# chayanchatterjee/GW-Whisper

Measured on AMD Instinct MI355X. Metric: 1s-strain segments/sec (encoder fwd), higher is better.
Workload: dtype bf16; 1 GPU; whisper-tiny encoder fwd, batch 256 log-mel (80x3000) per GPU, 1500 tokens, random-init weights (BASELINE configs[1]); global_batch=256, parallelism=dp1, encoder=tiny, streams_per_gpu=1

## Files before the change

gw_whisper_amd/_lib.py:

```python

from __future__ import annotations

import ctypes as C
import os

_HERE = os.path.dirname(os.path.abspath(__file__))
LIB_PATH = os.environ.get("GWW_LIB") or os.path.join(_HERE, "libgww.so")

PREC_BF16 = 0
PREC_F32 = 1

EPI_BIAS, EPI_GELU, EPI_RESID = 0, 1, 2
EPI_DGELU = 5


class EncCfg(C.Structure):
    _fields_ = [("d_model", C.c_int), ("n_layers", C.c_int), ("n_heads", C.c_int),
                ("ffn", C.c_int), ("n_mels", C.c_int), ("t_in", C.c_int)]


class EncGlobals(C.Structure):
    _fields_ = [(n, C.c_void_p) for n in
                ("conv1_w", "conv1_b", "conv2_w", "conv2_b", "pos", "ln_w", "ln_b")]


class EncLayer(C.Structure):
    _fields_ = [(n, C.c_void_p) for n in
                ("ln1_w", "ln1_b", "q_w", "q_b", "k_w", "v_w", "v_b", "o_w", "o_b",
                 "ln2_w", "ln2_b", "fc1_w", "fc1_b", "fc2_w", "fc2_b")]


class DoraTarget(C.Structure):
    _fields_ = [("layer", C.c_int), ("proj", C.c_int), ("r", C.c_int), ("scaling", C.c_float),
                ("A", C.c_void_p), ("B", C.c_void_p), ("mag", C.c_void_p), ("nrm", C.c_void_p),
                ("dA", C.c_void_p), ("dB", C.c_void_p), ("dm", C.c_void_p)]


class EncLayerGrads(C.Structure):
    _fields_ = [(f[0], C.c_void_p) for f in EncLayer._fields_]


class EncGrads(C.Structure):
    _fields_ = [(n, C.c_void_p) for n in
                ("conv1_w", "conv1_b", "conv2_w", "conv2_b", "pos", "ln_w", "ln_b")] + \
               [("layers", C.POINTER(EncLayerGrads))]


class DoraMergeItem(C.Structure):
    _fields_ = [("w0", C.c_void_p), ("a", C.c_void_p), ("b", C.c_void_p), ("m", C.c_void_p), ("w_eff", C.c_void_p),
                ("norm_out", C.c_void_p), ("scaling", C.c_float), ("d_out", C.c_int), ("d_in", C.c_int), ("r", C.c_int)]


SIGNATURES = {
    "gww_version": (C.c_int, []),
    "gww_last_error": (C.c_char_p, []),
    "gww_frontend_create": (C.c_int, [C.POINTER(C.c_void_p)]),
    "gww_frontend_create_nmel": (C.c_int, [C.c_int, C.POINTER(C.c_void_p)]),
    "gww_frontend_destroy": (None, [C.c_void_p]),
    "gww_logmel_f32": (C.c_int, [C.c_void_p, C.c_void_p, C.c_int, C.c_int, C.c_long, C.c_void_p,
                                 C.c_void_p, C.c_void_p]),
    "gww_logmel_host_f32": (C.c_int, [C.c_void_p, C.c_int, C.c_int, C.c_long, C.c_void_p]),
    "gww_logmel_host_nmel_f32": (C.c_int, [C.c_void_p, C.c_int, C.c_int, C.c_long, C.c_int, C.c_void_p]),
    "gww_encoder_create": (C.c_int, [C.POINTER(EncCfg), C.POINTER(C.c_void_p)]),
    "gww_encoder_destroy": (None, [C.c_void_p]),
    "gww_encoder_set_weights": (C.c_int, [C.c_void_p, C.POINTER(EncGlobals), C.POINTER(EncLayer),
                                          C.c_int, C.c_void_p]),
    "gww_encoder_update_weights": (C.c_int, [C.c_void_p, C.POINTER(EncGlobals), C.POINTER(EncLayer), C.c_int,
                                             C.POINTER(C.c_uint), C.c_void_p]),
    "gww_encoder_workspace_bytes": (C.c_size_t, [C.c_void_p, C.c_int, C.c_int]),
    "gww_encoder_forward": (C.c_int, [C.c_void_p, C.c_void_p, C.c_int, C.c_int, C.c_void_p, C.c_size_t,
                                      C.c_void_p, C.c_void_p, C.c_void_p]),
    "gww_encoder_forward_outputs": (C.c_int, [C.c_void_p, C.c_void_p, C.c_int, C.c_int, C.c_void_p, C.c_size_t,
                                              C.c_void_p, C.c_void_p, C.c_void_p, C.c_void_p]),
    "gww_encoder_set_split": (C.c_int, [C.c_void_p, C.c_int]),
    "gww_encoder_set_stem_shortcut": (C.c_int, [C.c_void_p, C.c_int]),
    "gww_encoder_stem_shortcut_flags": (C.c_int, [C.c_void_p, C.c_int, C.c_int, C.c_void_p, C.POINTER(C.c_int)]),
    "gww_encoder_trace_enable": (C.c_int, [C.c_void_p, C.c_int]),
    "gww_encoder_trace_read": (C.c_int, [C.c_void_p, C.POINTER(C.c_float), C.POINTER(C.c_int)]),
    "gww_encoder_trace_classes": (C.c_int, []),
    "gww_encoder_trace_class_name": (C.c_char_p, [C.c_int]),
    "gww_train_saved_bytes": (C.c_size_t, [C.c_void_p, C.c_int]),
    "gww_train_workspace_bytes": (C.c_size_t, [C.c_void_p, C.c_int]),
    "gww_encoder_train_forward": (C.c_int, [C.c_void_p, C.c_void_p, C.c_int, C.c_void_p, C.c_size_t, C.c_void_p,
                                            C.c_size_t, C.c_void_p, C.c_int, C.c_void_p]),
    "gww_encoder_train_backward": (C.c_int, [C.c_void_p, C.c_int, C.c_void_p, C.c_size_t, C.c_void_p, C.c_size_t,
                                             C.c_void_p, C.POINTER(DoraTarget), C.c_int, C.c_void_p, C.c_void_p,
                                             C.c_int, C.c_void_p]),
    "gww_train_workspace_bytes_full": (C.c_size_t, [C.c_void_p, C.c_int]),
    "gww_train_workspace_bytes_adapters": (C.c_size_t, [C.c_void_p, C.c_int, C.c_int]),
    "gww_encoder_train_backward_full": (C.c_int, [C.c_void_p, C.c_int, C.c_void_p, C.c_size_t, C.c_void_p, C.c_size_t,
                                                  C.c_void_p, C.POINTER(DoraTarget), C.c_int, C.c_void_p, C.c_void_p,
                                                  C.c_int, C.POINTER(EncGrads), C.c_void_p]),
    "gww_train_saved_bytes_f32": (C.c_size_t, [C.c_void_p, C.c_int]),
    "gww_train_workspace_bytes_f32": (C.c_size_t, [C.c_void_p, C.c_int]),
    "gww_encoder_train_forward_f32": (C.c_int, [C.c_void_p, C.c_void_p, C.c_int, C.c_void_p, C.c_size_t, C.c_void_p,
                                                C.c_size_t, C.c_void_p, C.c_int, C.c_void_p]),
    "gww_encoder_train_backward_f32": (C.c_int, [C.c_void_p, C.c_int, C.c_void_p, C.c_size_t, C.c_void_p, C.c_size_t,
                                                 C.c_void_p, C.POINTER(DoraTarget), C.c_int, C.c_void_p, C.c_void_p,
                                                 C.c_int, C.c_void_p]),
    "gww_attention_lse_f32": (C.c_int, [C.c_void_p, C.c_void_p, C.c_void_p, C.c_int, C.c_int, C.c_int, C.c_void_p]),
    "gww_attention_bwd_f32_scratch_bytes": (C.c_size_t, [C.c_int, C.c_int, C.c_int]),
    "gww_attention_bwd_f32": (C.c_int, [C.c_void_p, C.c_void_p, C.c_void_p, C.c_void_p, C.c_void_p, C.c_void_p,
                                        C.c_int, C.c_int, C.c_int, C.c_void_p]),
    "gww_adapter_grads_f32_scratch_bytes": (C.c_size_t, [C.c_long, C.c_int, C.c_int, C.c_int]),
    "gww_adapter_grads_f32": (C.c_int, [C.c_void_p, C.c_long, C.c_void_p, C.c_void_p, C.c_long, C.c_void_p, C.c_float,
                                        C.c_float, C.c_void_p, C.c_void_p, C.c_void_p, C.c_void_p, C.c_void_p,
                                        C.c_void_p, C.c_void_p, C.c_long, C.c_int, C.c_int, C.c_int, C.c_void_p,
                                        C.c_size_t, C.c_void_p]),
    "gww_gemm_wgrad_workspace_bytes": (C.c_size_t, [C.c_long, C.c_int, C.c_int]),
    "gww_gemm_wgrad_bf16": (C.c_int, [C.c_void_p, C.c_long, C.c_void_p, C.c_long, C.c_long, C.c_int, C.c_int, C.c_float,
                                      C.c_void_p, C.c_void_p, C.c_void_p, C.c_size_t, C.c_void_p]),
    "gww_layernorm_param_grads_workspace_bytes": (C.c_size_t, [C.c_long, C.c_int]),
    "gww_layernorm_param_grads": (C.c_int, [C.c_void_p, C.c_void_p, C.c_int, C.c_long, C.c_int, C.c_void_p, C.c_void_p,
                                            C.c_void_p, C.c_size_t, C.c_void_p]),
    "gww_attention_bwd_bf16": (C.c_int, [C.c_void_p, C.c_void_p, C.c_void_p, C.c_void_p, C.c_void_p, C.c_void_p,
                                         C.c_int, C.c_int, C.c_int, C.c_void_p]),
    "gww_attention_bwd_log2q_bf16": (C.c_int, [C.c_void_p, C.c_void_p, C.c_void_p, C.c_void_p, C.c_void_p, C.c_void_p,
                                         C.c_int, C.c_int, C.c_int, C.c_void_p]),
    "gww_attention_log2q_bf16": (C.c_int, [C.c_void_p, C.c_void_p, C.c_void_p, C.c_int, C.c_int, C.c_int, C.c_void_p]),
    "gww_attention_lse_bf16": (C.c_int, [C.c_void_p, C.c_void_p, C.c_void_p, C.c_int, C.c_int, C.c_int, C.c_void_p]),
    "gww_layernorm_bwd": (C.c_int, [C.c_void_p, C.c_void_p, C.c_void_p, C.c_int, C.c_void_p, C.c_int, C.c_void_p,
                                    C.c_long, C.c_int, C.c_void_p]),
    "gww_gelu_bf16": (C.c_int, [C.c_void_p, C.c_void_p, C.c_void_p, C.c_long, C.c_void_p]),
    "gww_dora_grads": (C.c_int, [C.c_void_p, C.c_long, C.c_void_p, C.c_void_p, C.c_long, C.c_void_p, C.c_float,
                                 C.c_float, C.c_void_p, C.c_void_p, C.c_void_p, C.c_void_p, C.c_void_p, C.c_void_p,
                                 C.c_void_p, C.c_long, C.c_int, C.c_int, C.c_void_p]),
    "gww_adapter_grads_scratch_bytes": (C.c_size_t, [C.c_long, C.c_int, C.c_int, C.c_int]),
    "gww_adapter_grads": (C.c_int, [C.c_void_p, C.c_long, C.c_void_p, C.c_void_p, C.c_long, C.c_void_p, C.c_float,
                                    C.c_float, C.c_void_p, C.c_void_p, C.c_void_p, C.c_void_p, C.c_void_p, C.c_void_p,
                                    C.c_void_p, C.c_long, C.c_int, C.c_int, C.c_int, C.c_void_p, C.c_size_t,
                                    C.c_void_p]),
    "gww_dora_grads_multi": (C.c_int, [C.c_void_p, C.c_long, C.c_void_p, C.c_void_p, C.c_long, C.c_int,
                                       C.POINTER(C.c_long), C.POINTER(C.c_void_p), C.POINTER(C.c_float),
                                       C.POINTER(C.c_float), C.POINTER(C.c_void_p), C.POINTER(C.c_void_p),
                                       C.POINTER(C.c_void_p), C.POINTER(C.c_void_p), C.POINTER(C.c_void_p),
                                       C.POINTER(C.c_void_p), C.POINTER(C.c_void_p), C.c_long, C.c_int, C.c_void_p]),
    "gww_dora_merge_f32": (C.c_int, [C.c_void_p, C.c_void_p, C.c_void_p, C.c_void_p, C.c_float,
                                     C.c_int, C.c_int, C.c_int, C.c_void_p, C.c_void_p, C.c_void_p]),
    "gww_conv1_gelu_bf16": (C.c_int, [C.c_void_p, C.c_void_p, C.c_void_p, C.c_void_p, C.c_void_p, C.c_int, C.c_int, C.c_int,
                                      C.c_void_p]),
    "gww_dora_merge_batch_f32": (C.c_int, [C.POINTER(DoraMergeItem), C.c_int, C.c_void_p]),
    "gww_layernorm": (C.c_int, [C.c_void_p, C.c_void_p, C.c_void_p, C.c_void_p, C.c_int, C.c_long,
                                C.c_int, C.c_void_p]),
    "gww_gemm_bf16": (C.c_int, [C.c_void_p, C.c_void_p, C.c_void_p, C.c_void_p, C.c_void_p, C.c_long,
                                C.c_int, C.c_int, C.c_int, C.c_void_p]),
    "gww_gemm_bf16_v4_split": (C.c_int, [C.c_void_p, C.c_void_p, C.c_void_p, C.c_void_p, C.c_void_p, C.c_long,
                                         C.c_int, C.c_int, C.c_int, C.c_int, C.c_void_p]),
    "gww_gemm_astat_bf16": (C.c_int, [C.c_void_p, C.c_void_p, C.c_void_p, C.c_void_p, C.c_void_p, C.c_void_p,
                                      C.c_void_p, C.c_void_p, C.c_long, C.c_int, C.c_int, C.c_int, C.c_void_p]),
    "gww_ln_fold_weights": (C.c_int, [C.c_void_p, C.c_void_p, C.c_void_p, C.c_void_p, C.c_float, C.c_int, C.c_int,
                                      C.c_void_p, C.c_void_p, C.c_void_p, C.c_void_p]),
    "gww_gemm_fulln_bf16": (C.c_int, [C.c_void_p, C.c_void_p, C.c_void_p, C.c_void_p, C.c_long, C.c_int, C.c_int,
                                      C.c_int, C.c_void_p]),
    "gww_mlp_fused_bf16": (C.c_int, [C.c_void_p] * 8 + [C.c_long, C.c_int, C.c_int, C.c_void_p, C.c_void_p, C.c_void_p,
                                     C.c_int, C.c_void_p]),
    "gww_mlp_pack_bf16": (C.c_int, [C.c_void_p, C.c_void_p, C.c_void_p, C.c_void_p, C.c_int, C.c_int, C.c_int, C.c_void_p]),
    "gww_attn_out_mlp_fused_bf16": (C.c_int, [C.c_void_p] * 9 + [C.c_long, C.c_int, C.c_int, C.c_void_p, C.c_void_p, C.c_void_p,
                                              C.c_int, C.c_void_p]),
    "gww_attn_out_mlp_final_bf16": (C.c_int, [C.c_void_p] * 11 + [C.c_long, C.c_int, C.c_int, C.c_void_p]),
    "gww_mlp_pack_op_bf16": (C.c_int, [C.c_void_p] * 5 + [C.c_int, C.c_int, C.c_int, C.c_void_p]),
    "gww_lnqkv_fused_bf16": (C.c_int, [C.c_void_p, C.c_void_p, C.c_void_p, C.c_void_p, C.c_void_p, C.c_long, C.c_int, C.c_int,
                                       C.c_void_p]),
    "gww_stem_fill_f32": (C.c_int, [C.c_void_p] * 5 + [C.c_int, C.c_int, C.c_int, C.c_int, C.c_void_p]),
    "gww_lnqkv_fused_x0_bf16": (C.c_int, [C.c_void_p] * 5 + [C.c_int, C.c_int] + [C.c_void_p] * 4 + [C.c_long, C.c_int, C.c_int,
                                          C.c_void_p]),
    "gww_attn_out_mlp_fused_x0_bf16": (C.c_int, [C.c_void_p] * 5 + [C.c_int, C.c_int] + [C.c_void_p] * 6 + [C.c_long, C.c_int, C.c_int,
                                                 C.c_void_p, C.c_void_p, C.c_void_p, C.c_int, C.c_void_p]),
    "gww_qscan_energy_f32": (C.c_int, [C.c_void_p, C.c_int, C.c_int, C.c_void_p, C.c_void_p, C.POINTER(C.c_int), C.c_void_p,
                                       C.c_void_p, C.c_long, C.c_void_p, C.c_int, C.c_void_p]),
    "gww_qscan_interp_f32": (C.c_int, [C.c_void_p, C.c_long, C.c_void_p, C.c_void_p, C.c_int, C.c_void_p, C.c_int, C.c_int,
                                       C.c_int, C.c_void_p, C.c_void_p, C.c_void_p]),
    "gww_qadapter_tail_f32": (C.c_int, [C.c_void_p, C.c_int, C.c_int, C.c_int, C.c_void_p, C.c_void_p, C.c_void_p,
                                        C.c_void_p, C.c_void_p, C.c_long, C.c_int, C.c_int, C.c_void_p]),
    "gww_qadapter_cnn_packed_bytes": (C.c_size_t, [C.c_int, C.c_int, C.c_int]),
    "gww_qadapter_cnn_workspace_bytes": (C.c_size_t, [C.c_int, C.c_int, C.c_int, C.c_int, C.c_int]),
    "gww_qadapter_cnn_backward_workspace_bytes": (C.c_size_t, [C.c_int, C.c_int, C.c_int, C.c_int, C.c_int, C.c_int]),
    "gww_qadapter_cnn_backward_f32": (C.c_int, [C.c_void_p, C.c_void_p, C.c_int, C.c_int, C.c_int, C.c_void_p, C.c_void_p,
                                                C.c_void_p, C.c_int, C.c_int, C.c_int, C.c_void_p, C.c_size_t] + [C.c_void_p] * 9),
    "gww_qadapter_cnn_pack_f32": (C.c_int, [C.c_void_p] * 8 + [C.c_int, C.c_int, C.c_int, C.c_void_p, C.c_void_p]),
    "gww_qadapter_cnn_forward_f32": (C.c_int, [C.c_void_p, C.c_int, C.c_int, C.c_int, C.c_void_p, C.c_int, C.c_int, C.c_int,
                                              C.c_void_p, C.c_size_t, C.c_void_p, C.c_void_p]),
    "gww_welch_power_f32": (C.c_int, [C.c_void_p, C.c_long, C.c_long, C.c_int, C.c_float, C.c_void_p, C.c_void_p]),
    "gww_column_median_f32": (C.c_int, [C.c_void_p, C.c_long, C.c_int, C.c_void_p, C.c_void_p]),
    "gww_fir_f32": (C.c_int, [C.c_void_p, C.c_long, C.c_void_p, C.c_int, C.c_int, C.c_void_p, C.c_long, C.c_long, C.c_void_p]),
    "gww_fir_f64": (C.c_int, [C.c_void_p, C.c_long, C.c_void_p, C.c_int, C.c_int, C.c_void_p, C.c_long, C.c_long, C.c_void_p]),
    "gww_cluster_triggers_f64": (C.c_int, [C.c_void_p, C.c_void_p, C.c_long, C.c_float, C.c_double, C.c_void_p, C.c_void_p,
                                          C.c_void_p, C.c_int, C.c_void_p]),
    "gww_gemm_f32": (C.c_int, [C.c_void_p, C.c_void_p, C.c_void_p, C.c_void_p, C.c_void_p, C.c_long,
                               C.c_int, C.c_int, C.c_int, C.c_void_p]),
    "gww_attention_bf16": (C.c_int, [C.c_void_p, C.c_void_p, C.c_int, C.c_int, C.c_int, C.c_void_p]),
    "gww_attention_f32": (C.c_int, [C.c_void_p, C.c_void_p, C.c_int, C.c_int, C.c_int, C.c_void_p]),
    "gww_attention_probs_bf16": (C.c_int, [C.c_void_p, C.c_int, C.c_void_p, C.c_int, C.c_int, C.c_int, C.c_void_p]),
    "gww_attention_probs_f32": (C.c_int, [C.c_void_p, C.c_void_p, C.c_int, C.c_int, C.c_int, C.c_void_p]),
    "gww_cast_f32_bf16": (C.c_int, [C.c_void_p, C.c_void_p, C.c_long, C.c_void_p]),
    "gww_info_nce_forward_f32": (C.c_int, [C.c_void_p, C.c_void_p, C.c_int, C.c_int, C.c_float] + [C.c_void_p] * 6),
    "gww_info_nce_backward_f32": (C.c_int, [C.c_void_p] * 4 + [C.c_int, C.c_int, C.c_float] + [C.c_void_p] * 4),
    "gww_qadapter_tail_backward_workspace_bytes": (C.c_size_t, [C.c_int, C.c_int]),
    "gww_qadapter_tail_backward_f32": (C.c_int, [C.c_void_p, C.c_long, C.c_void_p, C.c_int, C.c_int, C.c_int, C.c_int, C.c_int,
                                                 C.c_void_p, C.c_void_p, C.c_void_p, C.c_void_p, C.c_void_p, C.c_size_t]
                                                + [C.c_void_p] * 5),
    "gww_assemble_batch_f32": (C.c_int, [C.c_void_p, C.c_long, C.c_void_p, C.c_long, C.c_long, C.c_void_p, C.c_void_p,
                                         C.c_void_p, C.c_int, C.c_void_p, C.c_void_p]),
    "gww_head_forward_f32": (C.c_int, [C.c_void_p] * 10 + [C.c_int, C.c_int, C.c_int, C.c_float, C.c_int, C.c_ulonglong,
                                       C.c_ulonglong] + [C.c_void_p] * 9),
    "gww_head_workspace_bytes": (C.c_size_t, [C.c_int, C.c_int]),
    "gww_head_backward_f32": (C.c_int, [C.c_void_p] * 10 + [C.c_int, C.c_int, C.c_int, C.c_float, C.c_int]
                              + [C.c_void_p] * 11),
    "gww_head_dropout_mask_f32": (C.c_int, [C.c_ulonglong, C.c_ulonglong, C.c_int, C.c_int, C.c_int, C.c_float, C.c_void_p,
                                            C.c_void_p]),
    "gww_eval_accumulate": (C.c_int, [C.c_void_p, C.c_void_p, C.c_void_p, C.c_int, C.c_int, C.c_void_p, C.c_void_p,
                                      C.c_void_p, C.c_void_p]),
    "gww_det_head_forward_f32": (C.c_int, [C.c_void_p] * 12 + [C.c_int, C.c_int, C.c_int, C.c_float] + [C.c_void_p] * 10),
    "gww_det_head_workspace_bytes": (C.c_size_t, [C.c_int, C.c_int]),
    "gww_det_head_backward_f32": (C.c_int, [C.c_void_p] * 12 + [C.c_int, C.c_int, C.c_int, C.c_void_p, C.c_size_t]
                                  + [C.c_void_p] * 12),
    "gww_det_head_scores_f32": (C.c_int, [C.c_void_p] * 11 + [C.c_int, C.c_int, C.c_int, C.c_int, C.c_void_p, C.c_long,
                                          C.c_void_p]),
    "gww_det_eval_accumulate": (C.c_int, [C.c_void_p, C.c_void_p, C.c_void_p, C.c_int, C.c_int] + [C.c_void_p] * 5),
    "gww_score_thresholds_workspace_bytes": (C.c_size_t, []),
    "gww_score_thresholds_f32": (C.c_int, [C.c_void_p, C.c_long, C.c_void_p, C.c_int, C.c_void_p, C.c_void_p, C.c_size_t,
                                           C.c_void_p]),
    "gww_detection_counts_f32": (C.c_int, [C.c_void_p, C.c_long, C.c_void_p, C.c_int, C.c_void_p, C.c_void_p]),
    "gww_roc_tile": (C.c_int, []),
    "gww_roc_sort_workspace_bytes": (C.c_size_t, [C.c_long]),
    "gww_roc_sort_f32": (C.c_int, [C.c_void_p, C.c_void_p, C.c_long] + [C.c_void_p] * 7 + [C.c_size_t, C.c_void_p]),
    "gww_roc_curve_workspace_bytes": (C.c_size_t, [C.c_long]),
    "gww_roc_curve_f64": (C.c_int, [C.c_void_p, C.c_void_p, C.c_void_p, C.c_long] + [C.c_void_p] * 7 + [C.c_size_t, C.c_void_p]),
    "gww_roc_bootstrap_workspace_bytes": (C.c_size_t, [C.c_long, C.c_long]),
    "gww_roc_bootstrap_tpr_f64": (C.c_int, [C.c_void_p] * 5 + [C.c_long, C.c_long, C.c_void_p, C.c_int, C.c_void_p, C.c_void_p,
# ... 41 lines not shown
```

gw_whisper_amd/csrc/common.h:

```cpp
#pragma once

#include <hip/hip_runtime.h>
#include <stdarg.h>
#include <stdint.h>
#include <stdio.h>
#include <string.h>

#include "../../include/gww.h"
#include <vector>

namespace gww {

extern thread_local char g_err[512];
int fail(int code, const char* fmt, ...);

#define GWW_HIP(expr)                                                                 \
  do {                                                                                \
    hipError_t _e = (expr);                                                           \
    if (_e != hipSuccess)                                                             \
      return ::gww::fail(GWW_ERR_HIP, "%s failed: %s (%s:%d)", #expr, hipGetErrorString(_e), \
                         __FILE__, __LINE__);                                         \
  } while (0)

#define GWW_LAUNCH_CHECK() GWW_HIP(hipGetLastError())

#define GWW_REQUIRE(cond, ...)                       \
  do {                                               \
    if (!(cond)) return ::gww::fail(GWW_ERR_ARG, __VA_ARGS__); \
  } while (0)

#define GWW_TRY(expr)          \
  do {                         \
    int _rc = (expr);          \
    if (_rc != GWW_OK) return _rc; \
  } while (0)

typedef __attribute__((ext_vector_type(8))) __bf16 bf16x8;
typedef __attribute__((ext_vector_type(4))) __bf16 bf16x4;
typedef __attribute__((ext_vector_type(4))) float f32x4;
typedef __attribute__((ext_vector_type(16))) float f32x16;
typedef __attribute__((ext_vector_type(4))) unsigned int u32x4;
typedef __attribute__((ext_vector_type(2))) unsigned int u32x2;

constexpr int kWave = 64;

__device__ __forceinline__ unsigned short f2bf(float f) {
  __bf16 h = (__bf16)f;
  return __builtin_bit_cast(unsigned short, h);
}
__device__ __forceinline__ float bf2f(unsigned short u) {
  return __builtin_bit_cast(float, ((unsigned int)u) << 16);
}
__device__ __forceinline__ unsigned int pack2bf(float lo, float hi) {
  typedef __bf16 bf16x2_t __attribute__((ext_vector_type(2)));
  typedef float f32x2_t __attribute__((ext_vector_type(2)));
  const f32x2_t v = {lo, hi};
  return __builtin_bit_cast(unsigned int, __builtin_convertvector(v, bf16x2_t));
}

__device__ __forceinline__ float wave_sum(float v) {
#pragma unroll
  for (int o = 32; o > 0; o >>= 1) v += __shfl_xor(v, o, 64);
  return v;
}
__device__ __forceinline__ float wave_max(float v) {
#pragma unroll
  for (int o = 32; o > 0; o >>= 1) v = fmaxf(v, __shfl_xor(v, o, 64));
  return v;
}

__device__ __forceinline__ double wave_sum_f64(double v) {
#pragma unroll
  for (int o = 32; o > 0; o >>= 1) v += __shfl_xor(v, o, 64);
  return v;
}
__device__ __forceinline__ double block_sum_f64(double s) {
  __shared__ double part[256];
  part[threadIdx.x] = s;
  __syncthreads();
  for (int o = 128; o > 0; o >>= 1) {
    if ((int)threadIdx.x < o) part[threadIdx.x] += part[threadIdx.x + o];
    __syncthreads();
  }
  return part[0];
}
__device__ __forceinline__ double block_sum_f64(const float* __restrict__ v, int n) {
  double s = 0.0;
  for (int i = threadIdx.x; i < n; i += 256) s += (double)v[i];
  return block_sum_f64(s);
}

__device__ __forceinline__ float gelu_erf(float x) {
  return 0.5f * x * (1.0f + erff(x * 0.70710678118654752440f));
}

__device__ __forceinline__ float gelu_fast(float x) {
  const float z = fabsf(x) * 0.70710678118654752440f;
  const float t = __builtin_amdgcn_rcpf(fmaf(0.3275911f, z, 1.0f));
  float p = fmaf(1.061405429f, t, -1.453152027f);
  p = fmaf(p, t, 1.421413741f);
  p = fmaf(p, t, -0.284496736f);
  p = fmaf(p, t, 0.254829592f);
  p *= t;
  const float e = __builtin_amdgcn_exp2f(-z * z * 1.44269504088896340736f);
  const float erf_abs = fmaf(-p, e, 1.0f);
  const float h = 0.5f * x;
  return fmaf(h, copysignf(erf_abs, x), h);
}

__device__ __forceinline__ float gelu_sig4(float x) {
  const float s = fminf(x * x, 64.0f);
  float q = fmaf(s, 0.0010148164f, -0.1067791331f);
  q = fmaf(s, q, -2.3011178f);
  const float e = __builtin_amdgcn_exp2f(x * q);
  return x * __builtin_amdgcn_rcpf(1.0f + e);
}
__device__ __forceinline__ float gelu_sig4_sigma(float x) {
  const float s = fminf(x * x, 64.0f);
  float q = fmaf(s, 0.0010148164f, -0.1067791331f);
  q = fmaf(s, q, -2.3011178f);
  const float e = __builtin_amdgcn_exp2f(x * q);
  return __builtin_amdgcn_rcpf(1.0f + e);
}

__device__ __forceinline__ float dgelu_fast(float z) {
  const float az = fabsf(z) * 0.70710678118654752440f;
  const float t = __builtin_amdgcn_rcpf(fmaf(0.3275911f, az, 1.0f));
  float p = fmaf(1.061405429f, t, -1.453152027f);
  p = fmaf(p, t, 1.421413741f);
  p = fmaf(p, t, -0.284496736f);
  p = fmaf(p, t, 0.254829592f);
  p *= t;
  const float e = __builtin_amdgcn_exp2f(-az * az * 1.44269504088896340736f);
  const float erf_abs = fmaf(-p, e, 1.0f);
  return fmaf(0.5f, copysignf(erf_abs, z), fmaf(z * 0.3989422804f, e, 0.5f));
}

static inline long cdiv(long a, long b) { return (a + b - 1) / b; }

struct Arena {
  size_t off = 0;
  size_t take(size_t bytes) { const size_t o = off; off += (bytes + 255) / 256 * 256; return o; }
  size_t total() const { return off; }
};

#ifdef GWW_LAB
long lab_int(const char* name, long dflt);
#else
constexpr long lab_int(const char*, long dflt) { return dflt; }
#endif

constexpr int kStemTc = 256, kStemTt = kStemTc / 2;

enum { PREP_PACK16, PREP_PACK32, PREP_COPY, PREP_LNFOLD, PREP_TRANSPOSE, PREP_DORA };
constexpr int kPrepMaxOps = 40;
constexpr int kPrepMaxRank = 1024;
struct PrepOp {
  const void *a, *b, *c, *d;
  void *o0, *o1, *o2;
  int kind, blocks, N, K;
  int C, taps;
  float scale;
  int pad_;
};
struct PrepArgs {
  int n;
  int first[kPrepMaxOps + 1];
  PrepOp op[kPrepMaxOps];
};
struct PrepBatch {
  std::vector<PrepArgs> args;
  hipStream_t s;
  explicit PrepBatch(hipStream_t st) : s(st) {}
  int add(const PrepOp& o);
  int flush();
  int pack(const float* w, void* out, int out_bf16, int N, int C, int taps, int Kpad, float scale);
  int copy(const float* in, float* out, int n, float scale);
  int ln_fold(const float* w, const float* g, const float* bl, const float* bias, float scale, int N, int K, void* wp,
              float* u, float* cb);
  int transpose(const void* in, void* out, int R, int Cn);
  int dora(const float* w0, const float* a, const float* b, const float* m, float scaling, int d_out, int d_in, int r,
           float* w_eff, float* norm_out);
};

enum : int {
  EPI_BIAS = 0,
  EPI_GELU = 1,
  EPI_RESID = 2,
  EPI_CONV2 = 3,
};

}

#include "launchers.h"
```

gw_whisper_amd/csrc/encoder.hip:

```cpp
#include "encoder_impl.h"

namespace gww {
#ifdef GWW_LAB
long lab_int(const char* name, long dflt) {
  const char* e = getenv(name);
  return e ? atol(e) : dflt;
}
#endif
}

using namespace gww;

static size_t carve_blob(gww_encoder* e, char* blob) {
  const size_t d = e->cfg.d_model, F = e->cfg.ffn, T = e->cfg.t_in / 2, Kc1 = conv1_kpad(e->cfg.n_mels);
  const uintptr_t base = (uintptr_t)blob;
  Arena a;
  auto put = [&](auto*& p, size_t bytes) { p = (decltype(+p))(base + a.take(bytes)); };
  put(e->c1w, d * Kc1 * 2);
  put(e->c2w, (d + 255) / 256 * 256 * 3 * d * 2);
  put(e->c1w32, d * Kc1 * 4);
  put(e->c2w32, d * 3 * d * 4);
  put(e->c1wT, d * Kc1 * 2);
  put(e->c2wT, d * 3 * d * 2);
  put(e->c1b, d * 4);
// ... 127 lines not shown
    GWW_HIP(hipMemcpyAsync(e->pos, g->pos, (size_t)T * d * 4, hipMemcpyDeviceToDevice, s));
    if (T > kStemTt) {
      GWW_HIP(hipMemcpyAsync(e->pos_c, g->pos, (size_t)(kStemTt - 2) * d * 4, hipMemcpyDeviceToDevice, s));
      GWW_HIP(hipMemsetAsync(e->pos_c + (size_t)(kStemTt - 2) * d, 0, (size_t)d * 4, s));
      GWW_HIP(hipMemcpyAsync(e->pos_c + (size_t)(kStemTt - 1) * d, g->pos + (size_t)(T - 1) * d, (size_t)d * 4,
                             hipMemcpyDeviceToDevice, s));
    }
    GWW_TRY(pb.copy(g->ln_w, e->lnw, d, 1.f));
    GWW_TRY(pb.copy(g->ln_b, e->lnb, d, 1.f));
  }
  for (int i = 0; i < n_layers; ++i) {
    const unsigned m = dirty ? dirty[i] : 15u;
    if (!m) continue;
    const gww_enc_layer& L = layers[i];
    LayerW& w = e->layers[i];
    const size_t dd = (size_t)d * d;
    if (m & 1u) {
      GWW_REQUIRE(L.ln1_w && L.ln1_b && L.q_w && L.q_b && L.k_w && L.v_w && L.v_b,
                  "gww_encoder_set_weights: NULL attention weight in layer %d", i);
      const float qs16 = attention_log2q_enabled() ? qs * 1.44269504088896340736f : qs;
      GWW_TRY(pb.pack(L.q_w, w.wqkv, 1, d, d, 1, d, qs16));
      GWW_TRY(pb.pack(L.q_w, w.wqkv32, 0, d, d, 1, d, qs));
      GWW_TRY(pack(L.k_w, w.wqkv + dd, w.wqkv32 + dd, d, d, 1, d, 1.f));
      GWW_TRY(pack(L.v_w, w.wqkv + 2 * dd, w.wqkv32 + 2 * dd, d, d, 1, d, 1.f));
      GWW_TRY(pb.copy(L.q_b, w.bqkv, d, qs));
      GWW_TRY(pb.copy(nullptr, w.bqkv + d, d, 0.f));
      GWW_TRY(pb.copy(L.v_b, w.bqkv + 2 * d, d, 1.f));
      GWW_TRY(pb.copy(L.q_b, w.bqkv16, d, qs16));
      GWW_TRY(pb.copy(nullptr, w.bqkv16 + d, d, 0.f));
      GWW_TRY(pb.copy(L.v_b, w.bqkv16 + 2 * d, d, 1.f));
      GWW_TRY(pb.copy(L.ln1_w, w.ln1w, d, 1.f));
      GWW_TRY(pb.copy(L.ln1_b, w.ln1b, d, 1.f));
      GWW_TRY(pb.ln_fold(L.q_w, L.ln1_w, L.ln1_b, L.q_b, qs16, d, d, w.wqkv_ln, w.uqkv, w.cbqkv));
      GWW_TRY(pb.ln_fold(L.k_w, L.ln1_w, L.ln1_b, nullptr, 1.f, d, d, w.wqkv_ln + dd, w.uqkv + d, w.cbqkv + d));
      GWW_TRY(pb.ln_fold(L.v_w, L.ln1_w, L.ln1_b, L.v_b, 1.f, d, d, w.wqkv_ln + 2 * dd, w.uqkv + 2 * d,
                             w.cbqkv + 2 * d));
      GWW_TRY(pt.transpose(w.wqkv, w.wqkvT, 3 * d, d));
    }
    if (m & 2u) {
      GWW_REQUIRE(L.o_w && L.o_b, "gww_encoder_set_weights: NULL out_proj weight in layer %d", i);
      GWW_TRY(pack(L.o_w, w.wo, w.wo32, d, d, 1, d, 1.f));
      GWW_TRY(pb.copy(L.o_b, w.bo, d, 1.f));
      GWW_TRY(pt.transpose(w.wo, w.woT, d, d));
    }
    if (m & 4u) {
      GWW_REQUIRE(L.ln2_w && L.ln2_b && L.fc1_w && L.fc1_b, "gww_encoder_set_weights: NULL fc1 weight in layer %d", i);
      GWW_TRY(pack(L.fc1_w, w.w1, w.w132, F, d, 1, d, 1.f));
      GWW_TRY(pb.copy(L.fc1_b, w.b1, F, 1.f));
      GWW_TRY(pb.copy(L.ln2_w, w.ln2w, d, 1.f));
      GWW_TRY(pb.copy(L.ln2_b, w.ln2b, d, 1.f));
      GWW_TRY(pb.ln_fold(L.fc1_w, L.ln2_w, L.ln2_b, L.fc1_b, 1.f, F, d, w.w1_ln, w.u1, w.cb1));
      GWW_TRY(pt.transpose(w.w1, w.w1T, F, d));
    }
    if (m & 8u) {
      GWW_REQUIRE(L.fc2_w && L.fc2_b, "gww_encoder_set_weights: NULL fc2 weight in layer %d", i);
      GWW_TRY(pack(L.fc2_w, w.w2, w.w232, d, F, 1, F, 1.f));
      GWW_TRY(pb.copy(L.fc2_b, w.b2, d, 1.f));
      GWW_TRY(pt.transpose(w.w2, w.w2T, d, F));
    }
  }
  GWW_TRY(pb.flush());
  GWW_TRY(pt.flush());
  if (mlp_fused_supported(d, F)) {
    for (int i = 0; i < n_layers; ++i) {
      const unsigned m = dirty ? dirty[i] : 15u, mn = i + 1 < n_layers ? (dirty ? dirty[i + 1] : 15u) : 0u;
      if (!(m & 14u) && !(mn & 1u)) continue;
      LayerW& w = e->layers[i];
      const void* wq_next = i + 1 < n_layers ? e->layers[i + 1].wqkv_ln : nullptr;
      const bool plain_stream = (generic_path_mask() & (GP_QKV | GP_OUT_PROJ)) != 0;
      if (plain_stream && ((m & 12u) || (mn & 1u))) GWW_TRY(launch_mlp_pack(w.w1_ln, w.w2, wq_next, w.wmlp, d, F, 3 * d, s));
      GWW_TRY(launch_mlp_pack(w.w1_ln, w.w2, wq_next, w.wmlp_op, d, F, 3 * d, s, w.wo));
    }
    if (!dirty || (dirty[0] & 1u))
      GWW_TRY(launch_mlp_pack(nullptr, nullptr, e->layers[0].wqkv_ln, e->layers[0].wqkv_st, d, 0, 3 * d, s));
  }
  return GWW_OK;
}

extern "C" int gww_encoder_set_weights(gww_encoder* e, const gww_enc_globals* g, const gww_enc_layer* layers,
                                       int n_layers, void* stream) {
  GWW_REQUIRE(e && g && layers, "gww_encoder_set_weights: NULL argument");
  GWW_REQUIRE(n_layers == e->cfg.n_layers, "gww_encoder_set_weights: got %d layers, handle has %d", n_layers,
              e->cfg.n_layers);
  GWW_TRY(pack_weights(e, g, layers, n_layers, nullptr, (hipStream_t)stream));
  e->ready = true;
  return GWW_OK;
}

extern "C" int gww_encoder_update_weights(gww_encoder* e, const gww_enc_globals* globals_or_null,
                                          const gww_enc_layer* layers, int n_layers, const unsigned* layer_dirty,
                                          void* stream) {
  GWW_REQUIRE(e && layers && layer_dirty, "gww_encoder_update_weights: NULL argument");
  GWW_REQUIRE(n_layers == e->cfg.n_layers, "gww_encoder_update_weights: got %d layers, handle has %d", n_layers,
              e->cfg.n_layers);
  if (!e->ready) return fail(GWW_ERR_STATE, "gww_encoder_update_weights: call gww_encoder_set_weights first");
  return pack_weights(e, globals_or_null, layers, n_layers, layer_dirty, (hipStream_t)stream);
}

namespace {
struct WsLayout {
  size_t melT, c1, x, x2, h, d2, qkv, ctx, f1, total;
};
WsLayout ws_layout(const gww_enc_cfg& c, int B, int precision) {
  const size_t es = precision == GWW_PREC_BF16 ? 2 : 4;
  const size_t d = c.d_model, F = c.ffn, Tin = c.t_in, T = c.t_in / 2, C = c.n_mels, Kc1 = conv1_kpad(c.n_mels);
  WsLayout w{};
  Arena a;
  const size_t Mp = padded_rows((size_t)B * T);
  w.melT = a.take(((size_t)B * (Tin + 2) * C + Kc1) * es);
  w.c1 = a.take((((size_t)B * (Tin + 2) + 255) / 256 * 256 + 520) * d * es);
  w.x = a.take(Mp * d * 4);
  w.x2 = a.take(Mp * d * 4);
  w.h = a.take(Mp * d * es);
  w.d2 = a.take(Mp * d * es);
  w.qkv = a.take(Mp * 3 * d * es);
  w.ctx = a.take(Mp * d * es);
  w.f1 = a.take(Mp * F * es);
  w.total = a.total();
  return w;
}

struct StemTailLayout {
  size_t c1s, xs, tr, dump, total;
};
StemTailLayout stem_tail_layout(int B, int d) {
  StemTailLayout t{};
  Arena a;
  t.c1s = a.take((((size_t)B * (kStemTc + 2) + 255) / 256 * 256 + 520) * d * 2);
  t.xs = a.take((size_t)B * kStemTt * d * 4);
  t.tr = a.take((size_t)B * d * 4);
  t.dump = a.take((size_t)d * 4);
  t.total = a.total();
  return t;
}

enum Conv1Kind { CONV1_DIRECT, CONV1_ASTAT, CONV1_GENERIC };
enum Conv2Kind { CONV2_V4, CONV2_FULLN, CONV2_GENERIC };
struct FwdWants {
  bool last_hidden, last_token, hidden_slab, attn_slab;
};
struct FwdPlan {
  Conv1Kind conv1;
  Conv2Kind conv2;
  bool shortcut;
  bool x0_layer0;
  bool astat;
  bool mlp_fused;
  bool fuse_qkv;
  bool lnqkv0;
  bool op;
  bool fuse_final;
  bool pooled;
  bool q_log2;
};
FwdPlan plan_forward(const gww_encoder* e, int batch, int precision, FwdWants want) {
  const gww_enc_cfg& c = e->cfg;
  const int m = generic_path_mask(), d = c.d_model, F = c.ffn, T = c.t_in / 2;
  const bool bf = precision == GWW_PREC_BF16;
  FwdPlan p{};
  p.conv1 = !bf || (m & GP_CONV1) ? CONV1_GENERIC
            : conv1_mel_supported(c.n_mels, d, conv1_kpad(c.n_mels)) ? CONV1_DIRECT : d % 128 == 0 ? CONV1_ASTAT : CONV1_GENERIC;
  p.conv2 = bf && d % 128 == 0 && d <= 3072 && !(m & GP_CONV2) ? CONV2_V4
            : bf && (d == 384 || d == 512) && !(m & GP_CONV2_FULLN) ? CONV2_FULLN : CONV2_GENERIC;
  const auto x2_bytes = [&] { const WsLayout w = ws_layout(c, batch, precision); return w.h - w.x2; };
  p.shortcut = p.conv1 == CONV1_DIRECT && p.conv2 == CONV2_V4 && e->stem_shortcut && batch > 0 && !(m & GP_STEM_SHORTCUT) &&
               stem_tail_supported(c.t_in, d) && stem_tail_layout(batch, d).total <= x2_bytes();
  p.astat = bf && (d == 384 || (d == 512 && (m & GP_ASTAT_512))) && F % 128 == 0 && !(m & GP_LAYER_GEMMS);
  p.mlp_fused = p.astat && mlp_fused_supported(d, F) && !(m & GP_MLP);
  p.fuse_qkv = p.mlp_fused && !(m & GP_QKV);
  p.lnqkv0 = p.fuse_qkv && !(m & GP_LNQKV0);
  p.op = p.fuse_qkv && !(m & GP_OUT_PROJ);
  p.fuse_final = p.op && want.last_hidden && !(m & GP_FINAL_LN);
  p.pooled = bf && !want.last_hidden && want.last_token && T >= 3 && !(m & GP_POOLED) && !want.hidden_slab && !want.attn_slab;
  p.x0_layer0 = p.shortcut && p.lnqkv0 && p.op && !want.hidden_slab && c.n_layers > 1;
  p.q_log2 = attention_log2q_enabled();
  return p;
}
}

constexpr int kSplitMin = 32;

static bool use_split(const gww_encoder* e, int batch) { return e->split && batch >= 2 * kSplitMin; }

extern "C" size_t gww_encoder_workspace_bytes(const gww_encoder* e, int batch, int precision) {
  if (!e || batch <= 0) return 0;
  if (use_split(e, batch)) {
    const int b0 = batch / 2;
    return ws_layout(e->cfg, b0, precision).total + ws_layout(e->cfg, batch - b0, precision).total;
  }
  return ws_layout(e->cfg, batch, precision).total;
}

extern "C" int gww_encoder_set_stem_shortcut(gww_encoder* e, int on) {
  GWW_REQUIRE(e != nullptr, "gww_encoder_set_stem_shortcut: NULL handle");
  e->stem_shortcut = on != 0;
  return GWW_OK;
}

extern "C" int gww_encoder_stem_shortcut_flags(const gww_encoder* e, int batch, int precision, const void* workspace,
                                               int* flags) {
  GWW_REQUIRE(e && workspace && flags, "gww_encoder_stem_shortcut_flags: NULL argument");
  GWW_REQUIRE(batch > 0 && (precision == GWW_PREC_BF16 || precision == GWW_PREC_F32),
              "gww_encoder_stem_shortcut_flags: bad batch %d / precision %d", batch, precision);
  flags[0] = flags[1] = -1;
  const bool split = use_split(e, batch);
  const int b[2] = {split ? batch / 2 : batch, split ? batch - batch / 2 : 0};
  size_t off = 0;
  for (int i = 0; i < 2 && b[i] > 0; ++i) {
    const WsLayout w = ws_layout(e->cfg, b[i], precision);
    if (plan_forward(e, b[i], precision, FwdWants{}).shortcut)
      GWW_HIP(hipMemcpy(&flags[i], (const char*)workspace + off + w.melT, sizeof(int), hipMemcpyDeviceToHost));
    off += w.total;
  }
  return GWW_OK;
}

extern "C" int gww_encoder_set_split(gww_encoder* e, int on) {
  GWW_REQUIRE(e != nullptr, "gww_encoder_set_split: NULL handle");
  if (on && !e->s2[0]) {
    for (int i = 0; i < 2; ++i) {
      GWW_HIP(hipStreamCreateWithFlags(&e->s2[i], hipStreamNonBlocking));
      GWW_HIP(hipEventCreateWithFlags(&e->ev_join[i], hipEventDisableTiming));
    }
    GWW_HIP(hipEventCreateWithFlags(&e->ev_fork, hipEventDisableTiming));
    GWW_HIP(hipEventCreateWithFlags(&e->ev_skew, hipEventDisableTiming));
  }
  e->split = on ? 1 : 0;
  return GWW_OK;
}

struct Tracer {
  gww_encoder* e;
  hipStream_t s;
  int begin(int cls) {
    if (!e->trace) return GWW_OK;
    TraceSpan sp{cls, nullptr, nullptr};
    for (hipEvent_t* ev : {&sp.a, &sp.b}) {
      if (!e->pool.empty()) { *ev = e->pool.back(); e->pool.pop_back(); }
      else GWW_HIP(hipEventCreate(ev));
    }
    GWW_HIP(hipEventRecord(sp.a, s));
    e->spans.push_back(sp);
    return GWW_OK;
  }
  int end() {
    if (!e->trace) return GWW_OK;
    GWW_HIP(hipEventRecord(e->spans.back().b, s));
    return GWW_OK;
  }
};
#define TR(cls, expr)        \
  do {                       \
    GWW_TRY(tr.begin(cls));  \
    GWW_TRY(expr);           \
    GWW_TRY(tr.end());       \
  } while (0)

struct Fwd {
  gww_encoder* e;
  FwdPlan p;
  Tracer tr;
  hipStream_t s;
  bool bf;
  int B, d, F, T, H, n_layers;
  long M;
  void *melT, *c1, *h, *d2, *qkv, *ctx, *f1;
  float *x, *x2;
  int* st_flag;
  void* c1s;
  float *xs, *st_tr, *st_dump;
  MfX0 x0;
  float *last_hidden, *last_token, *hidden_slab, *attn_slab;
  size_t hs_stride, as_stride;
  hipEvent_t skew_event;

  int gemm(const void* A, long lda, const void* W16, const float* W32, const float* bias, const float* resid, const float* pos,
           void* Cout, long Mr, int N, int K, int epi, int rpb) const {
    return bf ? launch_gemm_bf16(A, lda, W16, bias, resid, pos, Cout, Mr, N, K, epi, rpb, s, 1)
              : launch_gemm_f32((const float*)A, lda, W32, bias, resid, pos, (float*)Cout, Mr, N, K, epi, rpb, s);
  }
  int tap_hidden(int l, const float* src) const {
    if (hidden_slab)
      GWW_HIP(hipMemcpyAsync(hidden_slab + (size_t)l * hs_stride, src, (size_t)M * d * 4, hipMemcpyDeviceToDevice, s));
    return GWW_OK;
  }
  int tap_attn(int l) const {
    if (attn_slab) GWW_TRY(launch_attention_probs(qkv, bf, bf && p.q_log2, attn_slab + (size_t)l * as_stride, B, T, H, s));
    return GWW_OK;
  }
  int tap_final() const {
    float* dst = hidden_slab ? hidden_slab + (size_t)n_layers * hs_stride : nullptr;
    if (dst && dst != last_hidden)
      GWW_HIP(hipMemcpyAsync(dst, last_hidden, (size_t)M * d * 4, hipMemcpyDeviceToDevice, s));
    return GWW_OK;
  }
  int stem(const float* mel);
  int walk_astat();
  int walk_generic();
  int pooled_last_layer(const LayerW& L, const float* x, float* rows, void* hb);
  int final_layernorm(const float* xc, const void* pending);
};

int Fwd::stem(const float* mel) {
  const int Tin = e->cfg.t_in, C = e->cfg.n_mels, Kc1 = conv1_kpad(C);
  const size_t es = bf ? 2 : 4;
  auto conv1_direct = [&]() -> int {
    if (p.shortcut) {
      GWW_TRY(launch_stem_detect(mel, st_flag, (long)B * C, Tin, s));
      GWW_TRY(launch_conv1_mel(mel, e->c1w, e->c1b, c1s, B, kStemTc, d, s, Tin, st_flag, 1));
    }
    return launch_conv1_mel(mel, e->c1w, e->c1b, c1, B, Tin, d, s, 0, p.shortcut ? st_flag : nullptr, 0);
  };
  auto conv2_v4 = [&]() -> int {
    const int Np = (d + 255) / 256 * 256;
    if (p.shortcut) {
      GWW_TRY(launch_gemm_bf16_v4(c1s, 2L * d, e->c2w, e->c2b, nullptr, xs, (long)B * (kStemTt + 1), Np, 3 * d, EPI_CONV2, s, 0,
                                  e->pos_c, kStemTt + 1, d, st_dump, st_flag, 1, st_tr, kStemTt - 2));
      if (!p.x0_layer0) GWW_TRY(launch_stem_fill(xs, st_tr, e->pos, x, st_flag, B, T, d, s));
    }
    return launch_gemm_bf16_v4(c1, 2L * d, e->c2w, e->c2b, nullptr, x, (long)B * (T + 1), Np, 3 * d, EPI_CONV2, s, 0, e->pos,
                               T + 1, d, x + (((size_t)B * T + 255) / 256 * 256) * d, p.shortcut ? st_flag : nullptr, 0);
  };
  if (p.conv1 != CONV1_DIRECT) {
    TR(TR_MEL, launch_mel_to_tokens(mel, melT, bf ? 1 : 0, B, C, Tin, s));
    GWW_HIP(hipMemsetAsync((char*)melT + (size_t)B * (Tin + 2) * C * es, 0, Kc1 * es, s));
    GWW_HIP(hipMemsetAsync(c1, 0, (size_t)d * es, s));
  }
  if (p.conv1 == CONV1_DIRECT)
    TR(TR_CONV1, conv1_direct());
  else if (p.conv1 == CONV1_ASTAT)
    TR(TR_CONV1, launch_gemm_astat(melT, C, nullptr, nullptr, nullptr, nullptr, e->c1w, e->c1b, c1,
                                   (long)B * (Tin + 2), d, Kc1, EPI_CONV1, Tin + 2, s));
  else
    TR(TR_CONV1, gemm(melT, C, e->c1w, e->c1w32, e->c1b, nullptr, nullptr, c1, (long)B * (Tin + 2), d, Kc1,
                      EPI_CONV1, Tin + 2));
  if (p.conv2 == CONV2_V4)
    TR(TR_CONV2, conv2_v4());
  else if (p.conv2 == CONV2_FULLN)
    TR(TR_CONV2, launch_gemm_fulln(c1, 2L * d, e->c2w, e->c2b, e->pos, x, (long)B * (T + 1), d, 3 * d, EPI_CONV2, T + 1, s));
  else
    TR(TR_CONV2, gemm(c1, 2L * d, e->c2w, e->c2w32, e->c2b, nullptr, e->pos, x, (long)B * (T + 1), d, 3 * d, EPI_CONV2,
                      T + 1));
  return GWW_OK;
}

int Fwd::pooled_last_layer(const LayerW& L, const float* x, float* rows, void* hb) {
  TR(TR_ATTN, launch_attention_bf16(qkv, ctx, B, T, H, s, nullptr, true, p.q_log2));
  float* xl = rows;
  float* xm = rows + (size_t)B * d;
  float* xf = rows + 2 * (size_t)B * d;
  GWW_HIP(hipMemcpy2DAsync(xl, (size_t)d * 4, x + (size_t)(T - 1) * d, (size_t)T * d * 4, (size_t)d * 4, B,
                           hipMemcpyDeviceToDevice, s));
  TR(TR_OUT, launch_gemm_bf16((const unsigned short*)ctx + (size_t)(T - 1) * d, (long)T * d, L.wo, L.bo, xl, nullptr,
                              xm, B, d, d, EPI_RESID, 0, s, 0));
  TR(TR_LNROWS, launch_layernorm(xm, L.ln2w, L.ln2b, hb, 1, B, d, s));
  TR(TR_FC1, launch_gemm_bf16(hb, d, L.w1, L.b1, nullptr, nullptr, f1, B, F, d, EPI_GELU, 0, s, 0));
  TR(TR_FC2, launch_gemm_bf16(f1, F, L.w2, L.b2, xm, nullptr, xf, B, d, F, EPI_RESID, 0, s, 0));
  TR(TR_LNROWS, launch_layernorm_rows(xf, d, e->lnw, e->lnb, last_token, B, d, s, nullptr));
  return GWW_OK;
}

int Fwd::final_layernorm(const float* xc, const void* pending) {
  if (last_hidden) TR(TR_LN, launch_layernorm(xc, e->lnw, e->lnb, last_hidden, 0, M, d, s, pending));
  if (last_token)
    TR(TR_LNROWS, launch_layernorm_rows(xc + (long)(T - 1) * d, (long)T * d, e->lnw, e->lnb, last_token, B, d, s,
                                        pending ? (const char*)pending + (size_t)(T - 1) * d * 2 : nullptr));
  if (last_hidden) GWW_TRY(tap_final());
  return GWW_OK;
}

struct AstatState {
  float* xc;
  float* xn;
  const void* pending;
  bool qkv_ready;
  void swap() { std::swap(xc, xn); }
};

int Fwd::walk_astat() {
  AstatState st{x, x2, nullptr, false};
  void* const d1 = h;
  auto args = [&]() { MlpFusedArgs a; a.who = "gww_encoder_forward"; a.M = M; a.d = d; return a; };
  auto with_qkv = [&](MlpFusedArgs& a, const LayerW& W) { a.qkv_u = W.uqkv; a.qkv_cb = W.cbqkv; a.qkv_out = qkv; a.NQ = 3 * d; };
  for (int i = 0; i < n_layers; ++i) {
    const LayerW& L = e->layers[i];
    const bool last = i == n_layers - 1, from_x0 = i == 0 && p.x0_layer0;
    if (!st.qkv_ready) {
      if (i == 0 && p.lnqkv0) {
        MlpFusedArgs a = args();
        a.x = st.xc; a.Wt = L.wqkv_st;
        with_qkv(a, L);
        if (from_x0) a.x0 = &x0;
        TR(TR_QKV, launch_mlp_fused(a, s));
      } else {
        TR(TR_QKV, launch_gemm_astat(st.xc, d, st.pending, st.pending ? st.xn : nullptr, L.uqkv, L.cbqkv, L.wqkv_ln, nullptr, qkv,
                                     M, 3 * d, d, EPI_BIAS, 0, s));
        if (st.pending) st.swap();
        st.pending = nullptr;
      }
    }
    st.qkv_ready = false;
    GWW_TRY(tap_hidden(i, st.xc));
    if (i == 0 && skew_event) GWW_HIP(hipEventRecord(skew_event, s));
    if (p.pooled && last) return pooled_last_layer(L, st.xc, st.xn, d1);
    TR(TR_ATTN, launch_attention_bf16(qkv, ctx, B, T, H, s, nullptr, false, p.q_log2));
    GWW_TRY(tap_attn(i));
    if (!p.op)
      TR(TR_OUT, launch_gemm_astat(ctx, d, nullptr, nullptr, nullptr, nullptr, L.wo, L.bo, d1, M, d, d, EPI_BIAS, 0, s));
    MlpFusedArgs a = args();
    a.x = st.xc; a.x_new = from_x0 ? nullptr : st.xn; a.ln_u = L.u1; a.ln_cb = L.cb1; a.b2 = L.b2; a.F = F;
    if (p.op) { a.ctx = ctx; a.bo = L.bo; a.Wt = L.wmlp_op; }
    else { a.delta = d1; a.Wt = L.wmlp; }
    if (p.fuse_qkv && !last) {
      with_qkv(a, e->layers[i + 1]);
      if (from_x0) a.x0 = &x0;
      TR(TR_MLPQKV, launch_mlp_fused(a, s));
      st.qkv_ready = true;
    } else if (p.fuse_final) {
      a.lnf_w = e->lnw; a.lnf_b = e->lnb; a.y = last_hidden;
      TR(TR_MLPFIN, launch_mlp_fused(a, s));
      if (last_token)
        GWW_HIP(hipMemcpy2DAsync(last_token, (size_t)d * 4, last_hidden + (size_t)(T - 1) * d, (size_t)T * d * 4, (size_t)d * 4,
                                 B, hipMemcpyDeviceToDevice, s));
      return tap_final();
    } else if (p.mlp_fused) {
      a.C = d2; a.keep_x_new = true;
      TR(TR_MLP, launch_mlp_fused(a, s));
      st.swap();
      st.pending = d2;
    } else {
      TR(TR_FC1, launch_gemm_astat(st.xc, d, d1, st.xn, L.u1, L.cb1, L.w1_ln, nullptr, f1, M, F, d, EPI_GELU, 0, s));
      st.swap();
      TR(TR_FC2, launch_gemm_fulln(f1, F, L.w2, L.b2, nullptr, d2, M, d, F, EPI_BIAS, 0, s));
      st.pending = d2;
    }
  }
  return final_layernorm(st.xc, st.pending);
}

int Fwd::walk_generic() {
  for (int i = 0; i < n_layers; ++i) {
    const LayerW& L = e->layers[i];
    GWW_TRY(tap_hidden(i, x));
    TR(TR_LN, launch_layernorm(x, L.ln1w, L.ln1b, h, bf ? 1 : 0, M, d, s));
    TR(TR_QKV, gemm(h, d, L.wqkv, L.wqkv32, bf ? L.bqkv16 : L.bqkv, nullptr, nullptr, qkv, M, 3 * d, d, EPI_BIAS, 0));
    if (p.pooled && i == n_layers - 1) return pooled_last_layer(L, x, x2, h);
    if (bf) TR(TR_ATTN, launch_attention_bf16(qkv, ctx, B, T, H, s, nullptr, false, p.q_log2));
    else TR(TR_ATTN, launch_attention_f32((const float*)qkv, (float*)ctx, B, T, H, s));
    GWW_TRY(tap_attn(i));
    TR(TR_OUT, gemm(ctx, d, L.wo, L.wo32, L.bo, x, nullptr, x, M, d, d, EPI_RESID, 0));
    TR(TR_LN, launch_layernorm(x, L.ln2w, L.ln2b, h, bf ? 1 : 0, M, d, s));
    TR(TR_FC1, gemm(h, d, L.w1, L.w132, L.b1, nullptr, nullptr, f1, M, F, d, EPI_GELU, 0));
    TR(TR_FC2, gemm(f1, F, L.w2, L.w232, L.b2, x, nullptr, x, M, d, F, EPI_RESID, 0));
  }
  return final_layernorm(x, nullptr);
}
#undef TR

static int forward_impl(gww_encoder* e, const float* mel, int batch, int precision, void* workspace,
                        size_t workspace_bytes, float* last_hidden, float* last_token, void* stream,
                        hipEvent_t skew_event = nullptr, float* hidden_slab = nullptr, float* attn_slab = nullptr,
                        size_t hs_stride = 0, size_t as_stride = 0) {
  GWW_REQUIRE(e && mel, "gww_encoder_forward: NULL argument");
  if (!e->ready) return fail(GWW_ERR_STATE, "gww_encoder_forward: weights not set");
  GWW_REQUIRE(precision == GWW_PREC_BF16 || precision == GWW_PREC_F32, "gww_encoder_forward: bad precision %d",
              precision);
  GWW_REQUIRE(batch >= 0, "gww_encoder_forward: batch < 0");
  GWW_REQUIRE(last_hidden || last_token, "gww_encoder_forward: no output requested");
  if (batch == 0) return GWW_OK;
  GWW_REQUIRE((((uintptr_t)mel) & 15) == 0 && (((uintptr_t)workspace) & 255) == 0,
              "gww_encoder_forward: mel must be 16-byte and workspace 256-byte aligned");
  const WsLayout w = ws_layout(e->cfg, batch, precision);
  if (!workspace || workspace_bytes < w.total)
    return fail(GWW_ERR_WORKSPACE, "gww_encoder_forward: workspace %zu bytes < required %zu", workspace_bytes,
                w.total);
  const gww_enc_cfg& c = e->cfg;
  char* base = (char*)workspace;
  const StemTailLayout st = stem_tail_layout(batch, c.d_model);
  char* const st_base = base + w.x2;
  Fwd f{};
  f.e = e;
  f.p = plan_forward(e, batch, precision, {last_hidden != nullptr, last_token != nullptr, hidden_slab != nullptr, attn_slab != nullptr});
  f.s = (hipStream_t)stream;
  f.tr = Tracer{e, f.s};
  f.bf = precision == GWW_PREC_BF16;
  f.B = batch; f.d = c.d_model; f.F = c.ffn; f.T = c.t_in / 2; f.H = c.n_heads; f.n_layers = c.n_layers;
  f.M = (long)batch * f.T;
  f.melT = base + w.melT; f.c1 = base + w.c1; f.h = base + w.h; f.d2 = base + w.d2; f.qkv = base + w.qkv; f.ctx = base + w.ctx;
  f.f1 = base + w.f1; f.x = (float*)(base + w.x); f.x2 = (float*)(base + w.x2);
  f.st_flag = (int*)f.melT; f.c1s = st_base + st.c1s; f.xs = (float*)(st_base + st.xs); f.st_tr = (float*)(st_base + st.tr);
  f.st_dump = (float*)(st_base + st.dump);
  f.x0 = MfX0{f.xs, f.st_tr, e->pos, f.st_flag, f.T, kStemTt};
  f.last_hidden = last_hidden; f.last_token = last_token; f.hidden_slab = hidden_slab; f.attn_slab = attn_slab;
  f.hs_stride = hs_stride; f.as_stride = as_stride; f.skew_event = skew_event;
  GWW_TRY(f.stem(mel));
  return f.p.astat ? f.walk_astat() : f.walk_generic();
}

static int forward_split(gww_encoder* e, const float* mel, int batch, int precision, void* workspace,
                         size_t workspace_bytes, float* last_hidden, float* last_token, float* hidden_slab,
                         float* attn_slab, void* stream) {
  GWW_REQUIRE(e && mel, "gww_encoder_forward: NULL argument");
  const size_t T_ = (size_t)(e->cfg.t_in / 2);
  const size_t hs_stride = (size_t)(batch > 0 ? batch : 0) * T_ * e->cfg.d_model;
  const size_t as_stride = (size_t)(batch > 0 ? batch : 0) * e->cfg.n_heads * T_ * T_;
  if (batch <= 0 || !use_split(e, batch))
    return forward_impl(e, mel, batch, precision, workspace, workspace_bytes, last_hidden, last_token, stream, nullptr,
                        hidden_slab, attn_slab, hs_stride, as_stride);
  hipStream_t s = (hipStream_t)stream;
  const int d = e->cfg.d_model, T = e->cfg.t_in / 2;
  const int b[2] = {batch / 2, batch - batch / 2};
  const size_t w0 = ws_layout(e->cfg, b[0], precision).total, w1 = ws_layout(e->cfg, b[1], precision).total;
  if (!workspace || workspace_bytes < w0 + w1)
    return fail(GWW_ERR_WORKSPACE, "gww_encoder_forward: workspace %zu bytes < required %zu", workspace_bytes, w0 + w1);
  GWW_HIP(hipEventRecord(e->ev_fork, s));
  int off = 0;
  static const int skew = (int)lab_int("GWW_SPLIT_SKEW", 0);
  for (int i = 0; i < 2; ++i) {
    GWW_HIP(hipStreamWaitEvent(e->s2[i], e->ev_fork, 0));
    if (i == 1 && skew) GWW_HIP(hipStreamWaitEvent(e->s2[1], e->ev_skew, 0));
    const int rc = forward_impl(e, mel + (size_t)off * e->cfg.n_mels * e->cfg.t_in, b[i], precision,
                                (char*)workspace + (i ? w0 : 0), i ? w1 : w0,
                                last_hidden ? last_hidden + (size_t)off * T * d : nullptr,
                                last_token ? last_token + (size_t)off * d : nullptr, e->s2[i],
                                (i == 0 && skew) ? e->ev_skew : nullptr,
                                hidden_slab ? hidden_slab + (size_t)off * T * d : nullptr,
                                attn_slab ? attn_slab + (size_t)off * e->cfg.n_heads * T_ * T_ : nullptr, hs_stride, as_stride);
    if (rc != GWW_OK) return rc;
    GWW_HIP(hipEventRecord(e->ev_join[i], e->s2[i]));
    GWW_HIP(hipStreamWaitEvent(s, e->ev_join[i], 0));
    off += b[i];
  }
  return GWW_OK;
}

extern "C" int gww_encoder_forward(gww_encoder* e, const float* mel, int batch, int precision, void* workspace,
                                   size_t workspace_bytes, float* last_hidden, float* last_token,
                                   void* stream) {
  return forward_split(e, mel, batch, precision, workspace, workspace_bytes, last_hidden, last_token, nullptr, nullptr,
                       stream);
}

extern "C" int gww_encoder_forward_outputs(gww_encoder* e, const float* mel, int batch, int precision, void* workspace,
                                           size_t workspace_bytes, float* last_hidden, float* hidden_slab,
                                           float* attn_slab, void* stream) {
  GWW_REQUIRE(e && mel, "gww_encoder_forward_outputs: NULL argument");
  if (!last_hidden && hidden_slab && batch > 0)
    last_hidden = hidden_slab + (size_t)e->cfg.n_layers * batch * (e->cfg.t_in / 2) * e->cfg.d_model;
  GWW_REQUIRE(last_hidden != nullptr, "gww_encoder_forward_outputs: no last_hidden and no hidden_slab");
  return forward_split(e, mel, batch, precision, workspace, workspace_bytes, last_hidden, nullptr, hidden_slab, attn_slab,
                       stream);
}
```

gw_whisper_amd/csrc/encoder_impl.h:

```cpp
#pragma once

#include "common.h"
#include "epilogue.h"

#include <stdlib.h>
#include <algorithm>
#include <vector>

namespace gww {

struct LayerW {
  unsigned short *wqkv, *wo, *w1, *w2;
  float *wqkv32, *wo32, *w132, *w232;
  float *bqkv, *bo, *b1, *b2, *ln1w, *ln1b, *ln2w, *ln2b;
  float* bqkv16;
  unsigned short *wqkv_ln, *w1_ln;
  unsigned short* wmlp;
  unsigned short* wqkv_st;
  unsigned short* wmlp_op;
  float *uqkv, *cbqkv, *u1, *cb1;
  unsigned short *wqkvT, *woT, *w1T, *w2T;
};

constexpr int conv1_kpad(int n_mels) { return (3 * n_mels + 63) / 64 * 64; }

inline size_t align_up(size_t x, size_t a = 256) { return (x + a - 1) / a * a; }

inline size_t padded_rows(size_t M) { return (M + 255) / 256 * 256 + 512; }

struct SavedArena {
  size_t layer_stride, x_in, total;
  int n_layers;
  float* x_in_at(void* saved, int l) const {
    return (float*)((char*)saved + (l < n_layers ? (size_t)l * layer_stride + x_in : (size_t)n_layers * layer_stride));
  }
  const float* x_in_at(const void* saved, int l) const { return x_in_at(const_cast<void*>(saved), l); }
};

enum : int {
  GP_LAYER_GEMMS = 1,
  GP_CONV1 = 2,
  GP_CONV2 = 4,
  GP_MLP = 8,
  GP_QKV = 16,
  GP_POOLED = 32,
  GP_LNQKV0 = 64,
  GP_OUT_PROJ = 128,
  GP_FINAL_LN = 256,
  GP_ASTAT_512 = 512,
  GP_CONV2_FULLN = 1024,
  GP_STEM_SHORTCUT = 2048,
};
inline int generic_path_mask() {
  static const int mask = (int)lab_int("GWW_GENERIC_PATH", 0);
  return mask;
}

inline int check_targets(const char* who, const gww_dora_target* t, int n) {
  for (int i = 0; i < n; ++i) {
    GWW_REQUIRE(t[i].r >= 1 && t[i].r <= 64, "%s: target %d has rank %d: adapter gradients support ranks 1..64", who, i, t[i].r);
    GWW_REQUIRE(t[i].A && t[i].B && t[i].mag && t[i].nrm && t[i].dA && t[i].dB && t[i].dm, "%s: NULL pointer in target %d", who, i);
  }
  for (int i = 1; i < n; ++i)
    for (int j = 0; j < i; ++j)
      GWW_REQUIRE(t[i].layer != t[j].layer || t[i].proj != t[j].proj, "%s: duplicate target: %d and %d both name layer %d proj %d",
                  who, j, i, t[i].layer, t[i].proj);
  return GWW_OK;
}
inline int check_target_range(const char* who, const gww_dora_target* t, int n, int L) {
  for (int i = 0; i < n; ++i)
    GWW_REQUIRE(t[i].layer >= 0 && t[i].layer < L && t[i].proj >= 0 && t[i].proj <= 5, "%s: bad target %d", who, i);
  return GWW_OK;
}
struct TargetTable {
  std::vector<const gww_dora_target*> slot;
  TargetTable() = default;
  TargetTable(const gww_dora_target* t, int n, int L) : slot(n > 0 ? (size_t)L * 6 : 0, nullptr) {
    for (int i = 0; i < n; ++i) slot[(size_t)t[i].layer * 6 + t[i].proj] = &t[i];
  }
  const gww_dora_target* at(int layer, int proj) const { return slot.empty() ? nullptr : slot[(size_t)layer * 6 + proj]; }
};

}

enum : int { TR_MEL = 0, TR_CONV1, TR_CONV2, TR_QKV, TR_ATTN, TR_OUT, TR_FC1, TR_FC2, TR_LN, TR_MLP, TR_MLPQKV, TR_LNROWS, TR_MLPFIN, TR_COUNT };

struct TraceSpan { int cls; hipEvent_t a, b; };

struct gww_encoder {
  gww_enc_cfg cfg{};
  bool ready = false;
  bool trace = false;
  bool stem_shortcut = true;
  std::vector<TraceSpan> spans;
  std::vector<hipEvent_t> pool;
  int split = 0;
  hipStream_t s2[2] = {nullptr, nullptr};
  hipEvent_t ev_fork = nullptr, ev_skew = nullptr, ev_join[2] = {nullptr, nullptr};
  char* blob = nullptr;
  size_t blob_bytes = 0;
  unsigned short *c1w = nullptr, *c2w = nullptr;
  unsigned short *c1wT = nullptr, *c2wT = nullptr;
  float *c1w32 = nullptr, *c2w32 = nullptr;
  float *c1b = nullptr, *c2b = nullptr, *pos = nullptr, *lnw = nullptr, *lnb = nullptr;
  float* pos_c = nullptr;
  std::vector<gww::LayerW> layers;
};
```

gw_whisper_amd/csrc/launchers.h:

```cpp
#pragma once

namespace gww {

int launch_layernorm(const float* x, const float* w, const float* b, void* y, int out_bf16,
                     long M, int d, hipStream_t s, const void* delta_bf16 = nullptr);
int launch_layernorm_rows(const float* x, long row_stride, const float* w, const float* b, float* y,
                          long M, int d, hipStream_t s, const void* delta_bf16 = nullptr);
int launch_pack_weight(const float* w, void* out, int out_bf16, int N, int C, int taps, int Kpad,
                       float scale, hipStream_t s);

bool conv1_mel_supported(int n_mels, int d, int kpad);
int launch_conv1_mel(const float* mel, const void* W, const float* bias, void* c1, int B, int T, int d, hipStream_t s,
                     int t_stride = 0, const int* run_flag = nullptr, int run_if = 0);
bool stem_tail_supported(int t_in, int d);
int launch_stem_detect(const float* mel, int* flag, long rows, int t_in, hipStream_t s);
int launch_stem_fill(const float* xs, const float* tr, const float* pos, float* x, const int* flag, int B, int T, int d,
                     hipStream_t s, int Tt = kStemTt);
int launch_mel_to_tokens(const float* mel, void* out, int out_bf16, int B, int C, int T, hipStream_t s);

int launch_gemm_astat(const void* A, long lda, const void* delta, float* x_out, const float* ln_u,
                      const float* ln_cb, const void* W, const float* bias, void* C, long M, int N, int K,
                      int epi, int rows_per_batch, hipStream_t s, long c_panel_rows = 0);
int launch_gemm_bf16(const void* A, long lda, const void* W, const float* bias, const float* resid,
                     const float* pos, void* C, long M, int N, int K, int epi, int rows_per_batch,
                     hipStream_t s, int rows_padded_256 = 0);
int launch_gemm_bf16_v4(const void* A, long lda, const void* W, const float* bias, const float* resid, void* C, long M,
                        int N, int K, int epi, hipStream_t s, int force_split = 0, const float* pos = nullptr,
                        int rows_per_batch = 0, int n_real = 0, float* dump = nullptr, const int* run_flag = nullptr,
                        int run_if = 0, float* tmpl_r = nullptr, int tmpl_t = 0);
int launch_gemm_fulln(const void* A, long lda, const void* W, const float* bias, const float* pos, void* C,
                      long M, int N, int K, int epi, int rows_per_batch, hipStream_t s);
int launch_gemm_f32(const float* A, long lda, const float* W, const float* bias, const float* resid,
                    const float* pos, float* C, long M, int N, int K, int epi, int rows_per_batch,
                    hipStream_t s);

int launch_attention_bf16(const void* qkv, void* ctx, int B, int T, int H, hipStream_t s, float* lse = nullptr,
                          bool last_tile_only = false, bool q_log2 = false);
int launch_attention_w64_bf16(const void* qkv, void* ctx, int B, int T, int H, hipStream_t s, float* lse);
bool attention_log2q_enabled();
int launch_attention_f32(const float* qkv, float* ctx, int B, int T, int H, hipStream_t s);
int launch_attention_probs(const void* qkv, bool bf16, bool q_log2, float* probs, int B, int T, int H, hipStream_t s);
int launch_attention_bwd_bf16(const void* qkv, const void* ctx, const void* dctx, const float* lse, float* D,
                              void* dqkv, int B, int T, int H, hipStream_t s, bool q_log2);

int launch_mlp_pack(const void* w1_folded, const void* w2, const void* wqkv_folded, void* out, int d, int F, int NQ,
                    hipStream_t s, const void* wo = nullptr);
bool mlp_fused_supported(int d, int F);
struct MfX0 {
  const float *xs, *tr, *pos;
  const int* flag;
  int T, Tt;
};
struct MlpFusedArgs {
  const char* who = "mlp_fused";
  const float* x = nullptr;
  const void* delta = nullptr;
  const void* ctx = nullptr;
  const float* bo = nullptr;
  float* x_new = nullptr;
  bool keep_x_new = false;
  const float *ln_u = nullptr, *ln_cb = nullptr;
  const void* Wt = nullptr;
  const float* b2 = nullptr;
  void* C = nullptr;
  const float *qkv_u = nullptr, *qkv_cb = nullptr;
  void* qkv_out = nullptr;
  int NQ = 0;
  float* x_next = nullptr;
  const float *lnf_w = nullptr, *lnf_b = nullptr;
  float* y = nullptr;
  const MfX0* x0 = nullptr;
  long M = 0;
  int d = 0, F = 0;
};
int launch_mlp_fused(const MlpFusedArgs& a, hipStream_t s);

int launch_ln_bwd(const float* x, const float* gamma, const void* dy, int dy_f32, float* dx, int accumulate,
                  void* dx_bf16, long M, int d, hipStream_t s);
int launch_gelu_bf16(const void* z, const void* df, void* out, long n, hipStream_t s);
int launch_sub_f32_bf16(const float* a, const float* b, void* out, long n, hipStream_t s);
int launch_add_delta_f32(const float* x, const void* delta_bf16, float* out, long n, hipStream_t s);
int launch_stem_dz2(const void* dxb, const void* z2, void* out, int B, int T, int d, hipStream_t s);
int launch_stem_dz1(const void* col, const void* z1, void* out, int B, int T, int Tin, int d, hipStream_t s);
int launch_stem_dmel(const void* col1, float* dmel, int B, int Tin, int C, int Kp, hipStream_t s);
int launch_ln_param_grads(const float* x, const void* dy, int dy_f32, long M, int d, float* dgamma, float* dbeta,
                          void* workspace, size_t ws_bytes, hipStream_t s);
size_t ln_param_grads_workspace_bytes(long M, int d);
int launch_pos_grad(const float* dx0, float* dpos, int B, int T, int d, hipStream_t s);
int launch_dora_grads(const void* X, long ldx, const void* dY, const void* Y, long ldy, const float* bias_st,
                      float yscale, float scaling, const float* A, const float* Bm, const float* mag,
                      const float* nrm, float* dA, float* dB, float* dm, long M, int d, int r, hipStream_t s,
                      void* scratch = nullptr, size_t scratch_bytes = 0);
int launch_dora_grads_multi(const void* X, long ldx, const void* dY, const void* Y, long ldy, int np,
                            const long* col_off, const float* const* bias_st, const float* yscale,
                            const float* scaling, const float* const* A, const float* const* Bm,
                            const float* const* mag, const float* const* nrm, float* const* dA, float* const* dB,
                            float* const* dm, long M, int d, hipStream_t s, void* scratch, size_t scratch_bytes);
size_t dora_grads_scratch_bytes(int np, int d);
int launch_adapter_grads(const void* X, long ldx, const void* dY, const void* Y, long ldy, const float* bias_st,
                         float yscale, float scaling, const float* A, const float* Bm, const float* mag,
                         const float* nrm, float* dA, float* dB, float* dm, long M, int d_in, int d_out, int r,
                         hipStream_t s, void* scratch, size_t scratch_bytes);
size_t adapter_grads_scratch_bytes(long M, int d_in, int d_out, int r);
int launch_wgrad(const void* dY, long ldy, const void* X, long ldx, long M, int N, int K, float alpha, float* dW,
                 float* db, int conv_cin, void* workspace, size_t ws_bytes, hipStream_t s);
size_t wgrad_workspace_bytes(long M, int N, int K);

int launch_attention_lse_f32(const float* qkv, float* ctx, float* lse, int B, int T, int H, bool last_tile_only,
                             hipStream_t s);
int launch_attention_bwd_f32(const float* qkv, const float* ctx, const float* dctx, const float* lse, float* scratch,
                             float* dqkv, int B, int T, int H, hipStream_t s);
size_t attention_bwd_f32_scratch_words(int B, int T, int H);
int launch_gemm_f32_dx(const float* A, long lda, const float* W, float* C, long ldc, long M, int N, int K, hipStream_t s);
int launch_adapter_grads_f32(const float* X, long ldx, const float* dY, const float* Y, long ldy, const float* bias,
                             float yscale, float scaling, const float* A, const float* Bm, const float* mag,
                             const float* nrm, float* dA, float* dB, float* dm, long M, int d_in, int d_out, int r,
                             hipStream_t s, void* scratch, size_t scratch_bytes);
size_t adapter_grads_f32_scratch_bytes(long M, int d_in, int d_out, int r);
int launch_gelu_f32(const float* z, const float* g, float* out, long n, hipStream_t s);
int launch_sub_f32(const float* a, const float* b, float* out, long n, hipStream_t s);
int launch_stem_dz2_f32(const float* dx0, const float* z2, float* out, int B, int T, int d, hipStream_t s);
int launch_stem_dz1_f32(const float* col, const float* z1, float* out, int B, int T, int Tin, int d, hipStream_t s);
int launch_stem_dmel_f32(const float* col1, float* dmel, int B, int Tin, int C, int Kp, hipStream_t s);

}
```

gw_whisper_amd/csrc/mlp_fused.hip:

```cpp
#include "common.h"

#include <stdlib.h>

#include <type_traits>

namespace gww {

namespace {
constexpr int MF_D = 384;
constexpr int MF_KT = MF_D / 64;
constexpr int MF_OT = MF_D / 32;
constexpr int MF_WAVES = 4, MF_THREADS = 256, MF_BM = 128;
#ifndef GWW_MF_EXP
#define GWW_MF_EXP 0
#endif
#ifndef GWW_MF_ABL
#define GWW_MF_ABL 0
#endif
#ifndef GWW_MF_OLDDMA
#define GWW_MF_OLDDMA 0
#endif
#ifndef GWW_MF_AHEAD
#define GWW_MF_AHEAD 3
#endif
#ifndef GWW_MF_SCHED
#define GWW_MF_SCHED 1
#endif
#ifndef GWW_MF_VACC
#define GWW_MF_VACC 1
#endif
#ifndef GWW_MF_NTSTORE
#define GWW_MF_NTSTORE 1
#endif
#ifndef GWW_MF_NTLOAD
#define GWW_MF_NTLOAD 1
#endif
#if GWW_MF_NTLOAD
#define MF_NT " nt"
#else
#define MF_NT ""
#endif
#ifndef GWW_MF_PADNOP
#define GWW_MF_PADNOP 0
#endif
#if GWW_MF_PADNOP
#define MF_PADNOP "s_nop 1\n\t"
#else
#define MF_PADNOP ""
#endif
#ifndef GWW_MF_XLDS
#define GWW_MF_XLDS 0
#endif
#ifndef GWW_MF_XSTNT
#define GWW_MF_XSTNT 0
#endif
#ifndef GWW_MF_XNT
#define GWW_MF_XNT 0
#endif
#if GWW_MF_XNT
#define MF_XNT MF_NT
#else
#define MF_XNT ""
#endif
#ifndef GWW_MF_DMAGAP
#define GWW_MF_DMAGAP 1
#endif
#ifndef GWW_MF_TAIL2
#define GWW_MF_TAIL2 0
#endif
#ifndef GWW_MF_NORM
#define GWW_MF_NORM 1
#endif
#ifndef GWW_MF_XACC
#define GWW_MF_XACC 1
#endif
constexpr int MF_AHEAD = GWW_MF_AHEAD;
constexpr int MF_NST_MAX = MF_AHEAD + 1;
constexpr int MF_TILE = 128 * 64 * 2;
constexpr int MF_GL = 16 / MF_WAVES;
constexpr int MF_FMAX = 1536;
constexpr int MF_SLICE_STRIDE = 144, MF_SLICE_BYTES = 32 * MF_SLICE_STRIDE;
constexpr int MF_OFF_CB = MF_NST_MAX * MF_TILE;
constexpr int MF_OFF_U = MF_OFF_CB + MF_FMAX * 4;
constexpr int MF_OFF_B2 = MF_OFF_U + MF_FMAX * 4;
constexpr int MF_OFF_BO = MF_OFF_B2 + MF_D * 4;
constexpr int MF_OFF_QCB = MF_OFF_BO + MF_D * 4;
constexpr int MF_OFF_SLICE = MF_OFF_QCB + MF_FMAX * 4;
constexpr int MF_LDS = MF_OFF_SLICE + 2 * MF_WAVES * MF_SLICE_BYTES;
static_assert(MF_LDS <= 160 * 1024, "LDS budget");

template <int N>
using MF_FL = std::integral_constant<int, N>;

__device__ __forceinline__ float mf_sum8(float v) {
  v += __builtin_bit_cast(float, __builtin_amdgcn_update_dpp(0, __builtin_bit_cast(int, v), 0xB1, 0xF, 0xF, true));
  v += __builtin_bit_cast(float, __builtin_amdgcn_update_dpp(0, __builtin_bit_cast(int, v), 0x4E, 0xF, 0xF, true));
  v += __builtin_bit_cast(float, __builtin_amdgcn_update_dpp(0, __builtin_bit_cast(int, v), 0x141, 0xF, 0xF, true));
  return v;
}

template <int N>
__device__ __forceinline__ void mf_wait_vmcnt() {
  asm volatile("s_waitcnt vmcnt(%0)" ::"n"(N) : "memory");
}

__device__ __forceinline__ float gelu_sig(float x) {
  const float s = fminf(x * x, 64.0f);
  float q = fmaf(s, 0.0010148164f, -0.1067791331f);
  q = fmaf(s, q, -2.3011178f);
#if GWW_MF_EXP & 32
  const float e = (x * q) * 0.37f;
  return x * ((1.0f + e) * 0.91f);
#else
  const float e = __builtin_amdgcn_exp2f(x * q);
  return x * __builtin_amdgcn_rcpf(1.0f + e);
#endif
}

#ifdef GWW_STAMP
__device__ unsigned long long g_stamp_mlp[24];
#define MSTAMP_DECL unsigned long long _t0 = __builtin_amdgcn_s_memtime(); unsigned long long _acc[20] = {0}; \
  const unsigned long long _tb = _t0, _rb = __builtin_amdgcn_s_memrealtime();
#define MSTAMP(i)                                                  \
  do {                                                             \
    if (GWW_STAMP >= 2 && (i) != 0 && (i) != 3 && (i) != 4 && (i) != 5 && !((i) >= 100)) break; \
    __builtin_amdgcn_sched_barrier(0);                             \
    const unsigned long long _t1 = __builtin_amdgcn_s_memtime();   \
    _acc[(i) >= 100 ? (i) - 100 : (i)] += _t1 - _t0;               \
    _t0 = _t1;                                                     \
    __builtin_amdgcn_sched_barrier(0);                             \
  } while (0)
#define TSTAMP(i) do { if (GWW_STAMP == 3) MSTAMP(100 + (i)); } while (0)
#define MSTAMP_FLUSH                                                                 \
  if (lane == 0) {                                                                   \
    for (int _q = 0; _q < 20; ++_q) atomicAdd(&g_stamp_mlp[_q], _acc[_q]);           \
    atomicAdd(&g_stamp_mlp[21], __builtin_amdgcn_s_memrealtime() - _rb);             \
    atomicAdd(&g_stamp_mlp[22], __builtin_amdgcn_s_memtime() - _tb);                 \
    atomicAdd(&g_stamp_mlp[23], 1ull);                                                \
  }
#else
#define MSTAMP_DECL
#define MSTAMP(i)
#define TSTAMP(i)
#define MSTAMP_FLUSH
#endif
}

__device__ __forceinline__ const float* mf_x0_row(const MfX0& z, const float* X, long g, bool x0, bool& tail, int& seg) {
  tail = false; seg = 0;
  if (!x0) return X + g * MF_D;
  const unsigned b = (unsigned)g / (unsigned)z.T, j = (unsigned)g - b * (unsigned)z.T;
  seg = (int)b;
  tail = (int)j >= z.Tt - 2 && (int)j <= z.T - 2;
  if (tail) return z.pos + (long)j * MF_D;
  return z.xs + ((long)b * z.Tt + ((int)j == z.T - 1 ? z.Tt - 1 : (int)j)) * MF_D;
}

struct MfNoX0 {};
template <int MODE, bool OP, bool X0 = false>
__global__ __launch_bounds__(MF_THREADS, 1) void k_mlp_fused(const float* X, const unsigned short* delta, float* x_out,
                                                            const float* __restrict__ ln_u,
                                                            const float* __restrict__ ln_cb,
                                                            const unsigned short* __restrict__ Wt,
                                                            const float* __restrict__ b2,
                                                            unsigned short* __restrict__ C, long M, int F,
                                                            int stagger_ticks, const float* __restrict__ q_u,
                                                            const float* __restrict__ q_cb,
                                                            unsigned short* __restrict__ q_out, int NQ,
                                                            float* x_next, const float* __restrict__ bo, int keep_x_new,
                                                            const std::conditional_t<X0, MfX0, MfNoX0> z) {
  __shared__ __attribute__((aligned(16))) unsigned char lds[MF_LDS];
  constexpr bool QKV = MODE == 1 || MODE == 2, LNQ = MODE == 2, FIN = MODE == 3;
  static_assert(!X0 || (GWW_MF_NORM && GWW_MF_XACC && (MODE == 2 || (MODE == 1 && OP))), "X0: layer 0's two launches; stages in the u table");
  constexpr bool XACC = GWW_MF_XACC && GWW_MF_NORM && GWW_MF_SCHED && OP && (MODE == 1 || MODE == 3);
  constexpr int MF_NST = MF_AHEAD + 1;
  float* lds_cb = reinterpret_cast<float*>(lds + MF_OFF_CB);
  float* lds_u = reinterpret_cast<float*>(lds + MF_OFF_U);
  float* lds_b2 = reinterpret_cast<float*>(lds + MF_OFF_B2);
  float* lds_bo = reinterpret_cast<float*>(lds + MF_OFF_BO);
  float* lds_qcb = reinterpret_cast<float*>(lds + MF_OFF_QCB);
  constexpr int OP_TILES = OP ? 3 * MF_KT : 0;
  typedef __attribute__((address_space(3))) void* lds_ptr;

  const int tid = threadIdx.x, lane = tid & 63, wave = tid >> 6;
  const int r = lane & 31, hh = lane >> 5;
  const long m_base = (long)blockIdx.x * MF_BM + wave * 32;
  unsigned char* slice = lds + MF_OFF_SLICE + wave * MF_SLICE_BYTES;
  unsigned char* const slice0 = slice;
  const int crow = lane >> 3, cchunk = lane & 7;

  const int wave_u = __builtin_amdgcn_readfirstlane(wave);
  const unsigned lane_off = (unsigned)lane * 16u;
  const unsigned lds_base = (unsigned)(unsigned long long)(lds_ptr)lds;
  auto issue_piece_c = [&](int tile, int stage, auto j_c) {
    constexpr int J = decltype(j_c)::value;
    const unsigned dst = lds_base + (unsigned)(stage * MF_TILE + MF_GL * wave_u * 1024);
    if (GWW_MF_EXP & 8) tile &= 7;
    const unsigned short* src = Wt + ((long)tile * (MF_TILE / 2) + MF_GL * wave_u * 512);
    const unsigned lo = lane_off;
    asm volatile("s_mov_b32 m0, %2\n\ts_nop 0\n\tglobal_load_lds_dwordx4 %0, %1 offset:%3"
                 :
                 : "v"(lo), "s"(src), "s"(dst), "n"(J * 1024)
                 : "memory");
  };
  auto issue_piece = [&](int tile, int stage, int j) {
#if GWW_MF_OLDDMA
    const unsigned dst = lds_base + (unsigned)(stage * MF_TILE + (MF_GL * wave_u + j) * 1024);
    const unsigned short* src = Wt + ((long)tile * (MF_TILE / 2) + (MF_GL * wave_u + j) * 512);
    unsigned keep;
    asm volatile("s_mov_b32 %0, m0\n\ts_mov_b32 m0, %3\n\ts_nop 0\n\tglobal_load_lds_dwordx4 %1, %2\n\ts_mov_b32 m0, %0"
                 : "=&s"(keep) : "v"(lane_off), "s"(src), "s"(dst) : "memory");
#else
    if (j == 0) issue_piece_c(tile, stage, std::integral_constant<int, 0>{});
    else if (j == 1) issue_piece_c(tile, stage, std::integral_constant<int, 1>{});
    else if (j == 2) issue_piece_c(tile, stage, std::integral_constant<int, 2>{});
    else issue_piece_c(tile, stage, std::integral_constant<int, 3>{});
#endif
  };
  auto issue = [&](int tile, int stage) {
#pragma unroll
    for (int j = 0; j < MF_GL; ++j) issue_piece(tile, stage, j);
  };

  MSTAMP_DECL
  auto stage_tables = [&]() {
    for (int i = tid; i < F; i += MF_THREADS) {
      lds_cb[i] = GWW_MF_SCHED ? ln_cb[i] * 0.125f : ln_cb[i];
      if (!GWW_MF_NORM) lds_u[i] = ln_u[i];
    }
    if (!GWW_MF_NORM && FIN) __syncthreads();
    if (!LNQ)
      for (int i = tid; i < MF_D; i += MF_THREADS) lds_b2[i] = XACC ? b2[i] + bo[i] : b2[i];
    if (OP)
      for (int i = tid; i < MF_D; i += MF_THREADS) lds_bo[i] = bo[i];
    if (FIN)
      for (int i = tid; i < MF_D; i += MF_THREADS) { lds_u[i] = q_u[i]; lds_u[MF_D + i] = q_cb[i]; }
    if (QKV && GWW_MF_NORM)
      for (int i = tid; i < NQ; i += MF_THREADS) lds_qcb[i] = q_cb[i];
  };
  if constexpr (!XACC) stage_tables();
  if (stagger_ticks > 0 && blockIdx.x < 256) {
    const unsigned long long t0 = __builtin_amdgcn_s_memrealtime();
    const unsigned long long wait = (unsigned long long)((blockIdx.x >> 3) & 15) * stagger_ticks;
    while (__builtin_amdgcn_s_memrealtime() - t0 < wait) __builtin_amdgcn_s_sleep(8);
  }

#pragma unroll
  for (int p = 0; p < MF_AHEAD; ++p) issue(p, p);
  const long xrow_l = m_base + r < M ? m_base + r : M - 1;
  const unsigned xoff = (unsigned)xrow_l * (unsigned)(MF_D * 4) + 16u * (unsigned)hh;
  f32x4 xp[XACC ? MF_OT : 1][4];
  bool x0 = false;
  int x0_seg0 = 0;
  f32x4* const lds_x0 = reinterpret_cast<f32x4*>(lds + MF_OFF_U);
  const float* x0_stage[2] = {nullptr, nullptr};
  f32x4 x0_sg[2];
  bool x0_tail = false;
  int x0_seg = 0;
  if constexpr (X0) {
    x0 = __builtin_amdgcn_readfirstlane(*z.flag) != 0;
    const unsigned g0 = (unsigned)blockIdx.x * (unsigned)MF_BM;
    x0_seg0 = (int)(g0 / (unsigned)z.T);
    const int seg_last = (int)((unsigned)(M - 1) / (unsigned)z.T);
#pragma unroll
    for (int k = 0; k < 2; ++k) {
      const int q = tid + 256 * k < 4 * (MF_D / 4) ? tid + 256 * k : tid;
      const int sg = q / (2 * (MF_D / 4)), wh = (q / (MF_D / 4)) & 1, c = q % (MF_D / 4);
      const long b = x0_seg0 + sg < seg_last ? x0_seg0 + sg : seg_last;
      x0_stage[k] = (wh ? z.tr + b * MF_D : z.xs + (b * z.Tt + (z.Tt - 2)) * MF_D) + 4 * c;
    }
  }
  auto x0_publish = [&](f32x4 (&sg)[2]) {
    lds_x0[tid] = sg[0];
    if (tid + 256 < 4 * (MF_D / 4)) lds_x0[tid + 256] = sg[1];
    asm volatile("s_waitcnt lgkmcnt(0)" ::: "memory");
    __builtin_amdgcn_s_barrier();
    asm volatile("" ::: "memory");
  };
  if constexpr (XACC && X0) {
    const float* xsrc = mf_x0_row(z, X, xrow_l, x0, x0_tail, x0_seg) + 4 * hh;
#pragma unroll
    for (int t = 0; t < MF_OT; ++t)
#pragma unroll
      for (int cc = 0; cc < 4; ++cc)
        asm volatile("global_load_dwordx4 %0, %1, off offset:%2" MF_XNT : "=a"(xp[t][cc]) : "v"(xsrc), "n"((32 * t + 8 * cc) * 4) : "memory");
#pragma unroll
    for (int k = 0; k < 2; ++k) asm volatile("global_load_dwordx4 %0, %1, off" : "=v"(x0_sg[k]) : "v"(x0_stage[k]) : "memory");
  } else if constexpr (XACC) {
#pragma unroll
    for (int t = 0; t < MF_OT; ++t)
#pragma unroll
      for (int cc = 0; cc < 4; ++cc)
        if (GWW_MF_ABL & 32) asm volatile("v_accvgpr_write_b32 %0, 0" : "=a"(xp[t][cc][0]));
        else asm volatile("global_load_dwordx4 %0, %1, %2 offset:%3" MF_XNT : "=a"(xp[t][cc]) : "v"(xoff), "s"(X), "n"((32 * t + 8 * cc) * 4) : "memory");
  }
  bf16x8 af[MF_KT * 4];
  float row_rstd, row_mean;
  long grow[4];
#pragma unroll
  for (int i = 0; i < 4; ++i) {
    const long g = m_base + 8 * i + crow;
    grow[i] = g < M ? g : M - 1;
  }
  if constexpr (XACC) {
    const unsigned coff = (unsigned)xrow_l * (unsigned)(MF_D * 2) + 64u * (unsigned)hh;
#pragma unroll
    for (int S = 0; S < MF_KT; ++S)
#pragma unroll
      for (int j = 0; j < 4; ++j)
        asm volatile("global_load_dwordx4 %0, %1, %2 offset:%3" : "=v"(af[4 * S + j]) : "v"(coff), "s"(delta), "n"((64 * S + 8 * j) * 2) : "memory");
    if constexpr (X0) {
      if (x0) {
        asm volatile("s_waitcnt vmcnt(24)" : "+v"(x0_sg[0]), "+v"(x0_sg[1]) : : "memory");
#pragma unroll
        for (int t = 0; t < MF_OT; ++t) asm volatile("" : "+a"(xp[t][0]), "+a"(xp[t][1]), "+a"(xp[t][2]), "+a"(xp[t][3]));
        x0_publish(x0_sg);
        if (x0_tail) {
          const f32x4* const st = lds_x0 + (x0_seg - x0_seg0) * (2 * (MF_D / 4)) + hh;
#pragma unroll
          for (int t = 0; t < MF_OT; ++t)
#pragma unroll
            for (int cc = 0; cc < 4; ++cc) {
              const f32x4 xt = st[8 * t + 2 * cc], rt = st[MF_D / 4 + 8 * t + 2 * cc];
#pragma unroll
              for (int k = 0; k < 4; ++k) xp[t][cc][k] = __builtin_fmaf(xt[k], rt[k], xp[t][cc][k]);
            }
        }
      }
    }
    stage_tables();
    asm volatile("s_waitcnt vmcnt(0)" ::: "memory");
#pragma unroll
    for (int i = 0; i < MF_KT * 4; ++i) asm volatile("" : "+v"(af[i]));
    row_rstd = 1.f; row_mean = 0.f;
  } else if constexpr (OP) {
    const unsigned short* crow_p[4];
#pragma unroll
    for (int i = 0; i < 4; ++i) crow_p[i] = delta + grow[i] * MF_D + 8 * cchunk;
    u32x4 cv[MF_KT][4];
#pragma unroll
    for (int S = 0; S < MF_KT; ++S)
#pragma unroll
      for (int i = 0; i < 4; ++i) {
        if (GWW_MF_ABL & 64) { cv[S][i] = u32x4{0x3f803f80u, 0x3f803f80u, 0x3f803f80u, 0x3f803f80u}; continue; }
        asm volatile("global_load_dwordx4 %0, %1, off offset:%2" MF_NT : "=v"(cv[S][i]) : "v"(crow_p[i]), "n"(64 * S * 2) : "memory");
      }
#pragma unroll
    for (int S = 0; S < MF_KT; ++S) {
#pragma unroll
      for (int i = 0; i < 4; ++i) {
        if (!(GWW_MF_ABL & 64)) asm volatile("s_waitcnt vmcnt(%1)" : "+v"(cv[S][i]) : "n"(23 - (4 * S + i)));
        *reinterpret_cast<u32x4*>(slice + (8 * i + crow) * MF_SLICE_STRIDE + cchunk * 16) = cv[S][i];
      }
#pragma unroll
      for (int j = 0; j < 4; ++j) {
        u32x4 u = *reinterpret_cast<const u32x4*>(slice + r * MF_SLICE_STRIDE + (4 * hh + j) * 16);
        asm volatile("" : "+v"(u)::"memory");
        af[4 * S + j] = __builtin_bit_cast(bf16x8, u);
      }
    }
    row_rstd = 1.f; row_mean = 0.f;
  } else
  {
    float s1[4] = {0.f, 0.f, 0.f, 0.f}, s2[4] = {0.f, 0.f, 0.f, 0.f}, cshift[4];
    const float* xrow[4];
    const unsigned short* drow[4];
#pragma unroll
    for (int i = 0; i < 4; ++i) {
      xrow[i] = X + grow[i] * MF_D + 4 * cchunk;
      drow[i] = LNQ ? nullptr : delta + grow[i] * MF_D + 4 * cchunk;
    }
    bool tl[4] = {false, false, false, false};
    const f32x4* st_row[4] = {lds_x0, lds_x0, lds_x0, lds_x0};
    if constexpr (X0) {
#pragma unroll
      for (int i = 0; i < 4; ++i) {
        int seg;
        xrow[i] = mf_x0_row(z, X, grow[i], x0, tl[i], seg) + 4 * cchunk;
        st_row[i] = lds_x0 + (seg - x0_seg0) * (2 * (MF_D / 4)) + cchunk;
      }
#pragma unroll
      for (int k = 0; k < 2; ++k) asm volatile("global_load_dwordx4 %0, %1, off" : "=v"(x0_sg[k]) : "v"(x0_stage[k]) : "memory");
    }
#pragma unroll
    for (int S3 = 0; S3 < MF_KT; S3 += 3) {
      f32x4 xv[3][2][4];
      u32x2 dv[3][2][4];
#pragma unroll
      for (int S = 0; S < 3; ++S)
#pragma unroll
        for (int h2 = 0; h2 < 2; ++h2)
#pragma unroll
          for (int i = 0; i < 4; ++i) {
            if constexpr (X0)
              asm volatile("global_load_dwordx4 %0, %1, off offset:%2"
                           : "=v"(xv[S][h2][i]) : "v"(xrow[i]), "n"((64 * (S3 + S) + 32 * h2) * 4) : "memory");
            else
            asm volatile("global_load_dwordx4 %0, %1, off offset:%2" MF_NT
                         : "=v"(xv[S][h2][i]) : "v"(xrow[i]), "n"((64 * (S3 + S) + 32 * h2) * 4) : "memory");
            if (!LNQ)
              asm volatile("global_load_dwordx2 %0, %1, off offset:%2" MF_NT
                           : "=v"(dv[S][h2][i]) : "v"(drow[i]), "n"((64 * (S3 + S) + 32 * h2) * 2) : "memory");
          }
      if constexpr (X0) {
        if (S3 == 0 && x0) {
          asm volatile("s_waitcnt vmcnt(24)" : "+v"(x0_sg[0]), "+v"(x0_sg[1]) : : "memory");
          x0_publish(x0_sg);
        }
      }
#pragma unroll
      for (int Sl = 0; Sl < 3; ++Sl) {
        const int S = S3 + Sl;
#pragma unroll
        for (int h2 = 0; h2 < 2; ++h2)
#pragma unroll
          for (int i = 0; i < 4; ++i) {
            f32x4 v;
            if (LNQ) {
              asm volatile("s_waitcnt vmcnt(%1)" : "+v"(xv[Sl][h2][i]) : "n"(23 - (8 * Sl + 4 * h2 + i)));
              v = xv[Sl][h2][i];
              if constexpr (X0) {
                if (tl[i]) {
                  const f32x4 xt = st_row[i][16 * S + 8 * h2], rt = st_row[i][MF_D / 4 + 16 * S + 8 * h2];
#pragma unroll
                  for (int k = 0; k < 4; ++k) v[k] = __builtin_fmaf(xt[k], rt[k], v[k]);
                }
              }
            } else {
              asm volatile("s_waitcnt vmcnt(%2)" : "+v"(xv[Sl][h2][i]), "+v"(dv[Sl][h2][i]) : "n"(46 - (8 * Sl + 4 * h2 + i)));
              v = xv[Sl][h2][i];
              v[0] += bf2f((unsigned short)(dv[Sl][h2][i][0] & 0xffff));
              v[1] += bf2f((unsigned short)(dv[Sl][h2][i][0] >> 16));
              v[2] += bf2f((unsigned short)(dv[Sl][h2][i][1] & 0xffff));
              v[3] += bf2f((unsigned short)(dv[Sl][h2][i][1] >> 16));
              *reinterpret_cast<f32x4*>(x_out + grow[i] * MF_D + 64 * S + 32 * h2 + 4 * cchunk) = v;
              asm volatile("" ::: "memory");
            }
            if (S == 0 && h2 == 0) {
              float t = (v[0] + v[1]) + (v[2] + v[3]);
              t = mf_sum8(t);
              cshift[i] = t * (1.0f / 32.0f);
            }
            v[0] -= cshift[i]; v[1] -= cshift[i]; v[2] -= cshift[i]; v[3] -= cshift[i];
            s1[i] += (v[0] + v[1]) + (v[2] + v[3]);
            s2[i] += (v[0] * v[0] + v[1] * v[1]) + (v[2] * v[2] + v[3] * v[3]);
            u32x2 o = {pack2bf(v[0], v[1]), pack2bf(v[2], v[3])};
// ... 241 lines not shown
        }
        if (GWW_MF_SCHED && RIDE_T >= 0) {
          if (u < 3) asm volatile("" : "+v"(cur[u + 1]));
          else if (sub < 3) asm volatile("" : "+v"(nxt[0]));
        }
        if (!(GWW_MF_EXP & 4)) {
          int off;
          if (sub == 3) off = first_off(next_kind, u);
          else off = KIND == 0 ? (u & 1) * 8192 + off1[2 * (sub + 1) + (u >> 1)] : u * 4096 + off2[sub + 1];
          nxt[u] = *reinterpret_cast<const bf16x8*>(Wn + off);
        }
        if (GWW_MF_SCHED && RIDE_T >= 0) {
          if (PRE >= 0 && 4 * sub + u < 8) preload_bias(2 * PRE + ((4 * sub + u) >> 2), pre_chunk, (4 * sub + u) & 3);
          gelu_slice(RIDE_T, 16 * IDX3 + 4 * sub + u);
          if (DMA_IN_GAPS && !(GWW_MF_EXP & 1)) {
            const int piece = 4 * sub + u - (9 - 4 * IDX3);
            if (piece >= 0 && piece < 4) issue_piece(dma_tile, dma_stage, piece);
          }
          MF_FENCE();
        }
      }
      if (GWW_MF_SCHED) continue;
      __builtin_amdgcn_sched_group_barrier(0x008, 1, 0);
      __builtin_amdgcn_sched_group_barrier(0x100, 2, 0);
      __builtin_amdgcn_sched_group_barrier(0x002, 8, 0);
      __builtin_amdgcn_sched_group_barrier(0x008, 1, 0);
      __builtin_amdgcn_sched_group_barrier(0x100, 1, 0);
      __builtin_amdgcn_sched_group_barrier(0x002, 8, 0);
      __builtin_amdgcn_sched_group_barrier(0x008, 1, 0);
      __builtin_amdgcn_sched_group_barrier(0x100, 1, 0);
      __builtin_amdgcn_sched_group_barrier(0x002, 8, 0);
      __builtin_amdgcn_sched_group_barrier(0x008, 1, 0);
      __builtin_amdgcn_sched_group_barrier(0x100, 1, 0);
      __builtin_amdgcn_sched_group_barrier(0x002, 8, 0);
      __builtin_amdgcn_sched_barrier(0);
    }
    stage = stage_next;
    ++it;
    MSTAMP(8 + (KIND == 0 ? IDX3 : 3 + IDX3) + 6 * PAR);
  };
  using I0 = std::integral_constant<int, 0>;
  using I1 = std::integral_constant<int, 1>;
  using I2 = std::integral_constant<int, 2>;
  using I3 = std::integral_constant<int, 3>;
  using IM = std::integral_constant<int, -1>;

  auto seam = [&](const float* seam_src, float* seam_dst, const float* seam_bias, auto&& after_request) {
      unsigned roff[4];
#pragma unroll
      for (int i = 0; i < 4; ++i) roff[i] = (unsigned)grow[i] * (unsigned)(MF_D * 4) + 16u * (unsigned)cchunk;

      float s1[4] = {0.f, 0.f, 0.f, 0.f}, s2[4] = {0.f, 0.f, 0.f, 0.f}, cshift[4];
      f32x4 xn4[3][2][4], xa4[3][2][4];
      auto request = [&](int np0) {
#pragma unroll
        for (int q = 0; q < 3; ++q)
#pragma unroll
          for (int h2 = 0; h2 < 2; ++h2)
#pragma unroll
            for (int i = 0; i < 4; ++i) {
              if (GWW_MF_ABL & 32) { xn4[q][h2][i] = f32x4{0.5f, -0.25f, 1.f, 0.f}; xa4[q][h2][i] = f32x4{0.5f, -0.25f, 1.f, 0.f}; continue; }
              if (np0 == 0)
                asm volatile("global_load_dwordx4 %0, %1, %2 offset:%3" MF_NT
                             : "=v"(xn4[q][h2][i]) : "v"(roff[i]), "s"(seam_src), "n"((64 * q + 32 * h2) * 4) : "memory");
              else
                asm volatile("global_load_dwordx4 %0, %1, %2 offset:%3" MF_NT
                             : "=a"(xa4[q][h2][i]) : "v"(roff[i]), "s"(seam_src), "n"((64 * (3 + q) + 32 * h2) * 4) : "memory");
            }
      };
      auto store_chunk = [&](int np) {
#pragma unroll
        for (int h2 = 0; h2 < 2; ++h2)
#pragma unroll
          for (int i = 0; i < 4; ++i) {
            if (GWW_MF_ABL & 16) asm volatile("" :: "v"(xn4[np % 3][h2][i]));
            else asm volatile("global_store_dwordx4 %0, %1, %2 offset:%3\n\ts_nop 1"
                              : : "v"(roff[i]), "v"(xn4[np % 3][h2][i]), "s"(seam_dst), "n"((64 * np + 32 * h2) * 4) : "memory");
          }
      };
#pragma unroll
      for (int np = 0; np < MF_KT; ++np) {
        unsigned char* const slice = slice0 + (np & 1) * (MF_WAVES * MF_SLICE_BYTES);
        if (np == 0) {
          request(0);
          after_request();
        }
#pragma unroll
        for (int tt = 0; tt < 2; ++tt) {
          const int t = 2 * np + tt;
#pragma unroll
          for (int cc = 0; cc < 4; ++cc) {
            const int nl = 32 * t + 8 * cc + 4 * hh;
            const float4 bv = *reinterpret_cast<const float4*>(seam_bias + nl);
            u32x2 o = {pack2bf(oacc[t][4 * cc] + bv.x, oacc[t][4 * cc + 1] + bv.y),
                       pack2bf(oacc[t][4 * cc + 2] + bv.z, oacc[t][4 * cc + 3] + bv.w)};
            *reinterpret_cast<u32x2*>(slice + r * MF_SLICE_STRIDE + (32 * tt + 8 * cc + 4 * hh) * 2) = o;
          }
        }
#pragma unroll
        for (int h2 = 0; h2 < 2; ++h2)
#pragma unroll
          for (int i = 0; i < 4; ++i) {
            const int ST_SINCE = 8 * (np % 3) + (np >= 3 ? 8 : 0);
            f32x4 v;
            if (np < 3) {
              if (!(GWW_MF_ABL & 32)) asm volatile("s_waitcnt vmcnt(%1)" : "+v"(xn4[np % 3][h2][i]) : "n"(ST_SINCE + 23 - (8 * (np % 3) + 4 * h2 + i)));
              v = xn4[np % 3][h2][i];
            } else {
              if (!(GWW_MF_ABL & 32)) asm volatile("s_waitcnt vmcnt(%1)" : "+a"(xa4[np % 3][h2][i]) : "n"(ST_SINCE + 23 - (8 * (np % 3) + 4 * h2 + i)));
              v = xa4[np % 3][h2][i];
            }
            const u32x2 dv = *reinterpret_cast<const u32x2*>(slice + (8 * i + crow) * MF_SLICE_STRIDE + h2 * 64 + cchunk * 8);
            v[0] += bf2f((unsigned short)(dv[0] & 0xffff));
            v[1] += bf2f((unsigned short)(dv[0] >> 16));
            v[2] += bf2f((unsigned short)(dv[1] & 0xffff));
            v[3] += bf2f((unsigned short)(dv[1] >> 16));
            xn4[np % 3][h2][i] = v;
            if (np == 0 && h2 == 0) {
              float t = (v[0] + v[1]) + (v[2] + v[3]);
              t = mf_sum8(t);
              cshift[i] = t * (1.0f / 32.0f);
            }
            v[0] -= cshift[i]; v[1] -= cshift[i]; v[2] -= cshift[i]; v[3] -= cshift[i];
            s1[i] += (v[0] + v[1]) + (v[2] + v[3]);
            s2[i] += (v[0] * v[0] + v[1] * v[1]) + (v[2] * v[2] + v[3] * v[3]);
            u32x2 o = {pack2bf(v[0], v[1]), pack2bf(v[2], v[3])};
            *reinterpret_cast<u32x2*>(slice + (8 * i + crow) * MF_SLICE_STRIDE + h2 * 64 + cchunk * 8) = o;
          }
#pragma unroll
        for (int j = 0; j < 4; ++j) {
          u32x4 u = *reinterpret_cast<const u32x4*>(slice + r * MF_SLICE_STRIDE + (4 * hh + j) * 16);
          asm volatile("" : "+v"(u)::"memory");
          af[4 * np + j] = __builtin_bit_cast(bf16x8, u);
        }
        if (np == 2) request(3);
        store_chunk(np);
      }
      float* stat = reinterpret_cast<float*>(slice0);
#pragma unroll
      for (int i = 0; i < 4; ++i) {
        float a = s1[i], b = s2[i];
        a = mf_sum8(a); b = mf_sum8(b);
        const float mean = a * (1.0f / MF_D);
        const float var = fmaxf(b * (1.0f / MF_D) - mean * mean, 0.f);
        if (cchunk == 0) {
          stat[8 * i + crow] = rsqrtf(var + 1e-5f);
          stat[32 + 8 * i + crow] = mean;
        }
      }
      row_rstd = stat[r];
      row_mean = stat[32 + r];
      asm volatile("" : "+v"(row_rstd), "+v"(row_mean)::"memory");
      };
  auto seam_x = [&](const float* sb, float* dst) {
    if constexpr (XACC) {
    float s1 = 0.f, s2 = 0.f, csh = 0.f;
#pragma unroll
    for (int t = 0; t < MF_OT; ++t)
#pragma unroll
      for (int cc = 0; cc < 4; ++cc) {
        const float4 bv = *reinterpret_cast<const float4*>(sb + 32 * t + 8 * cc + 4 * hh);
        f32x4 v = {oacc[t][4 * cc] + bv.x, oacc[t][4 * cc + 1] + bv.y, oacc[t][4 * cc + 2] + bv.z, oacc[t][4 * cc + 3] + bv.w};
        if (dst && !(GWW_MF_ABL & 16)) {
          if (GWW_MF_XLDS) {
            *reinterpret_cast<f32x4*>(slice0 + (t & 1) * (MF_WAVES * MF_SLICE_BYTES) + r * MF_SLICE_STRIDE + (8 * cc + 4 * hh) * 4) = v;
          } else {
            f32x4* const sp = reinterpret_cast<f32x4*>(reinterpret_cast<char*>(dst) + xoff + (32 * t + 8 * cc) * 4);
            if (GWW_MF_XSTNT) __builtin_nontemporal_store(v, sp);
            else *sp = v;
          }
        }
        if (GWW_MF_XLDS && dst && !(GWW_MF_ABL & 16) && cc == 3) {
#pragma unroll
          for (int i = 0; i < 4; ++i) {
            const f32x4 u = *reinterpret_cast<const f32x4*>(slice0 + (t & 1) * (MF_WAVES * MF_SLICE_BYTES) + (8 * i + crow) * MF_SLICE_STRIDE + cchunk * 16);
            *reinterpret_cast<f32x4*>(reinterpret_cast<char*>(dst) + (unsigned)grow[i] * (unsigned)(MF_D * 4) + 16u * (unsigned)cchunk + t * 128) = u;
          }
        }
        if (t == 0 && cc == 0) {
          const auto sw = __builtin_amdgcn_permlane32_swap(__float_as_uint(v[0]), __float_as_uint(v[0]), false, false);
          csh = hh ? __uint_as_float(sw[0]) : v[0];
        }
        v[0] -= csh; v[1] -= csh; v[2] -= csh; v[3] -= csh;
        s1 += (v[0] + v[1]) + (v[2] + v[3]);
        s2 += (v[0] * v[0] + v[1] * v[1]) + (v[2] * v[2] + v[3] * v[3]);
      }
    {
      const auto a = __builtin_amdgcn_permlane32_swap(__float_as_uint(s1), __float_as_uint(s1), false, false);
      const auto b = __builtin_amdgcn_permlane32_swap(__float_as_uint(s2), __float_as_uint(s2), false, false);
      s1 = __uint_as_float(a[0]) + __uint_as_float(a[1]);
      s2 = __uint_as_float(b[0]) + __uint_as_float(b[1]);
    }
    const float mean_s = s1 * (1.0f / MF_D);
    row_rstd = rsqrtf(fmaxf(s2 * (1.0f / MF_D) - mean_s * mean_s, 0.f) + 1e-5f);
    row_mean = csh + mean_s;
    const float nm = -mean_s * row_rstd;
    asm volatile("" : "+a"(oacc[0]), "+a"(oacc[1]), "+a"(oacc[2]), "+a"(oacc[3]), "+a"(oacc[4]), "+a"(oacc[5]), "+a"(oacc[6]),
                      "+a"(oacc[7]), "+a"(oacc[8]), "+a"(oacc[9]), "+a"(oacc[10]), "+a"(oacc[11]));
#pragma unroll
    for (int S = 0; S < MF_KT; ++S)
#pragma unroll
      for (int cc = 0; cc < 4; ++cc) {
        const float4 be = *reinterpret_cast<const float4*>(sb + 64 * S + 8 * cc + 4 * hh);
        const float4 bo_ = *reinterpret_cast<const float4*>(sb + 64 * S + 32 + 8 * cc + 4 * hh);
        const f32x16& E = oacc[2 * S];
        const f32x16& O = oacc[2 * S + 1];
        const unsigned e0 = pack2bf(fmaf(E[4 * cc] + be.x - csh, row_rstd, nm), fmaf(E[4 * cc + 1] + be.y - csh, row_rstd, nm));
        const unsigned e1 = pack2bf(fmaf(E[4 * cc + 2] + be.z - csh, row_rstd, nm), fmaf(E[4 * cc + 3] + be.w - csh, row_rstd, nm));
        const unsigned o0 = pack2bf(fmaf(O[4 * cc] + bo_.x - csh, row_rstd, nm), fmaf(O[4 * cc + 1] + bo_.y - csh, row_rstd, nm));
        const unsigned o1 = pack2bf(fmaf(O[4 * cc + 2] + bo_.z - csh, row_rstd, nm), fmaf(O[4 * cc + 3] + bo_.w - csh, row_rstd, nm));
        const auto w0 = __builtin_amdgcn_permlane32_swap(e0, o0, false, false);
        const auto w1 = __builtin_amdgcn_permlane32_swap(e1, o1, false, false);
        const u32x4 f = {w0[0], w1[0], w0[1], w1[1]};
        af[4 * S + cc] = __builtin_bit_cast(bf16x8, f);
      }
      }
  };
  if constexpr (OP) {
    static_assert(12 % MF_NST == 0, "OP mode relies on a ring whose depth divides the 12-tile body (4 or 6 stages)");
#pragma unroll
    for (int nt = 0; nt < 3; ++nt) {
#pragma unroll
      for (int kt = 0; kt < MF_KT; ++kt) {
        const int itile = nt * MF_KT + kt;
        if (!(GWW_MF_ABL & 128)) mf_wait_vmcnt<MF_GL * (MF_AHEAD - 2)>();
        __builtin_amdgcn_s_barrier();
        const int st = itile % MF_NST, st_next = (itile + 1) % MF_NST, dma_st = (itile + MF_AHEAD) % MF_NST;
        const int dma_tile = itile + MF_AHEAD < total ? itile + MF_AHEAD : total - 1;
        const bool last = itile == OP_TILES - 1;
#pragma unroll
        for (int sub = 0; sub < 4; ++sub) {
          const int q = 4 * kt + sub;
          bf16x8(&cur)[4] = wf[q & 1];
          bf16x8(&nxt)[4] = wf[(q + 1) & 1];
          const unsigned char* Wn = lds + (sub == 3 ? st_next : st) * MF_TILE;
          if (!(GWW_MF_ABL & 128)) issue_piece(dma_tile, dma_st, sub);
#pragma unroll
          for (int u = 0; u < 4; ++u) {
            asm volatile(MF_PADNOP "v_mfma_f32_32x32x16_bf16 %0, %1, %2, %0" : "+a"(oacc[4 * nt + u]) : "v"(cur[u]), "v"(af[4 * kt + sub]));
            const int off = (last && sub == 3) ? (u & 1) * 8192 + off1[u >> 1] : u * 4096 + offq[(sub + 1) & 3];
            nxt[u] = *reinterpret_cast<const bf16x8*>(Wn + off);
          }
        }
      }
    }
    it = OP_TILES;
    stage = OP_TILES % MF_NST;
    TSTAMP(14);
    asm volatile("s_nop 15\n\ts_nop 15"
                 : "+a"(oacc[0]), "+a"(oacc[1]), "+a"(oacc[2]), "+a"(oacc[3]), "+a"(oacc[4]), "+a"(oacc[5]), "+a"(oacc[6]),
                   "+a"(oacc[7]), "+a"(oacc[8]), "+a"(oacc[9]), "+a"(oacc[10]), "+a"(oacc[11]));
    if constexpr (XACC) {
      seam_x(lds_bo, (keep_x_new && !(GWW_MF_ABL & 256)) ? x_out : nullptr);
    } else {
    seam(X, x_out, lds_bo, [] {});
#if GWW_MF_NORM
    normalise_af();
#endif
#pragma unroll
    for (int t = 0; t < MF_OT; ++t)
#pragma unroll
      for (int j = 0; j < 16; ++j) oacc[t][j] = 0.f;
    }
    TSTAMP(15);
  }
  if constexpr (!LNQ) {
  if (GWW_MF_SCHED) {
#pragma unroll
    for (int t = 0; t < 4; ++t)
#pragma unroll
      for (int q = 0; q < 4; ++q) preload_bias(t, t >> 1, q);
  }
  using IW = std::conditional_t<OP && !XACC && !(GWW_MF_ABL & 32), I2, I1>;
  run_tile(MF_FL<0>{}, I0{}, I0{}, I0{}, IM{}, 0, 0, IM{}, 0, IW{});
  run_tile(MF_FL<1>{}, I0{}, I0{}, I1{}, IM{}, 0, 0, IM{}, 0, IW{});
  run_tile(MF_FL<2>{}, I0{}, I0{}, I2{}, IM{}, 0, 0, IM{}, 0, I1{});
  TSTAMP(12);
  if (GWW_MF_SCHED) asm volatile("s_nop 15\n\ts_nop 15" : "+v"(sacc[0]), "+v"(sacc[1]), "+v"(sacc[2]), "+v"(sacc[3]));
  act_piece(0, 0, 0); act_piece(0, 0, 1); act_piece(0, 0, 2); act_piece(0, 0, 3);
  TSTAMP(13);
  int b = 0;
  for (; b + 2 < nck; b += 2) {
    run_tile(MF_FL<3>{}, I0{}, I1{}, I0{}, I1{}, b >> 1, 0, IM{}, 0, I0{});
    run_tile(MF_FL<4>{}, I0{}, I1{}, I1{}, I1{}, b >> 1, 0, IM{}, 0, I0{});
    run_tile(MF_FL<5>{}, I0{}, I1{}, I2{}, I1{}, b >> 1, 1, IM{}, 0, I0{});
    run_tile(MF_FL<6>{}, I1{}, I0{}, I0{}, I2{}, b >> 1, 1, I0{}, b + 2, I0{});
    run_tile(MF_FL<7>{}, I1{}, I0{}, I1{}, I2{}, b >> 1, 1, IM{}, 0, I0{});
    run_tile(MF_FL<8>{}, I1{}, I0{}, I2{}, I2{}, b >> 1, 0, IM{}, 0, I0{});
    run_tile(MF_FL<9>{}, I0{}, I0{}, I0{}, I3{}, b >> 1, 0, IM{}, 0, I0{});
    run_tile(MF_FL<10>{}, I0{}, I0{}, I1{}, I3{}, b >> 1, 0, IM{}, 0, I0{});
    run_tile(MF_FL<11>{}, I0{}, I0{}, I2{}, I3{}, b >> 1, 1, IM{}, 0, I0{});
    run_tile(MF_FL<12>{}, I1{}, I1{}, I0{}, I0{}, (b >> 1) + 1, 1, I1{}, b + 3, I0{});
    run_tile(MF_FL<13>{}, I1{}, I1{}, I1{}, I0{}, (b >> 1) + 1, 1, IM{}, 0, I0{});
    run_tile(MF_FL<14>{}, I1{}, I1{}, I2{}, I0{}, (b >> 1) + 1, 0, IM{}, 0, I0{});
  }
  run_tile(MF_FL<3>{}, I0{}, I1{}, I0{}, I1{}, b >> 1, 0, IM{}, 0, I1{});
  run_tile(MF_FL<4>{}, I0{}, I1{}, I1{}, I1{}, b >> 1, 0, IM{}, 0, I1{});
  run_tile(MF_FL<5>{}, I0{}, I1{}, I2{}, I1{}, b >> 1, 1, IM{}, 0, I1{});
  run_tile(MF_FL<6>{}, I1{}, I0{}, I0{}, I2{}, b >> 1, 1, IM{}, 0, I1{});
  run_tile(MF_FL<7>{}, I1{}, I0{}, I1{}, I2{}, b >> 1, 1, IM{}, 0, I1{});
  run_tile(MF_FL<8>{}, I1{}, I0{}, I2{}, I2{}, b >> 1, 1, IM{}, 0, I1{});
  if (GWW_MF_SCHED) asm volatile("s_nop 15\n\ts_nop 15" : "+v"(sacc[0]), "+v"(sacc[1]), "+v"(sacc[2]), "+v"(sacc[3]));
  act_piece(0, b >> 1, 12); act_piece(0, b >> 1, 13); act_piece(0, b >> 1, 14); act_piece(0, b >> 1, 15);
  run_tile(MF_FL<9>{}, I1{}, I1{}, I0{}, IM{}, 0, 1, IM{}, 0, I1{});
  run_tile(MF_FL<10>{}, I1{}, I1{}, I1{}, IM{}, 0, 1, IM{}, 0, I1{});
  run_tile(MF_FL<11>{}, I1{}, I1{}, I2{}, IM{}, 0, QKV ? (GWW_MF_TAIL2 ? 0 : 2) : 1, IM{}, 0, I1{});

  MSTAMP(4);
  if (GWW_MF_SCHED)
    asm volatile("s_nop 15\n\ts_nop 15"
                 : "+a"(oacc[0]), "+a"(oacc[1]), "+a"(oacc[2]), "+a"(oacc[3]), "+a"(oacc[4]), "+a"(oacc[5]), "+a"(oacc[6]),
                   "+a"(oacc[7]), "+a"(oacc[8]), "+a"(oacc[9]), "+a"(oacc[10]), "+a"(oacc[11]));
  }
  if constexpr (FIN && XACC) {
    mf_wait_vmcnt<0>();
    float* y_out = reinterpret_cast<float*>(C);
    float s1 = 0.f, s2 = 0.f, csh = 0.f;
#pragma unroll
    for (int t = 0; t < MF_OT; ++t)
#pragma unroll
      for (int cc = 0; cc < 4; ++cc) {
        const float4 bv = *reinterpret_cast<const float4*>(lds_b2 + 32 * t + 8 * cc + 4 * hh);
        f32x4 v = {oacc[t][4 * cc] + bv.x, oacc[t][4 * cc + 1] + bv.y, oacc[t][4 * cc + 2] + bv.z, oacc[t][4 * cc + 3] + bv.w};
        if (t == 0 && cc == 0) {
          const auto sw = __builtin_amdgcn_permlane32_swap(__float_as_uint(v[0]), __float_as_uint(v[0]), false, false);
          csh = hh ? __uint_as_float(sw[0]) : v[0];
        }
        v[0] -= csh; v[1] -= csh; v[2] -= csh; v[3] -= csh;
        s1 += (v[0] + v[1]) + (v[2] + v[3]);
        s2 += (v[0] * v[0] + v[1] * v[1]) + (v[2] * v[2] + v[3] * v[3]);
      }
    {
      const auto a = __builtin_amdgcn_permlane32_swap(__float_as_uint(s1), __float_as_uint(s1), false, false);
      const auto b = __builtin_amdgcn_permlane32_swap(__float_as_uint(s2), __float_as_uint(s2), false, false);
      s1 = __uint_as_float(a[0]) + __uint_as_float(a[1]);
      s2 = __uint_as_float(b[0]) + __uint_as_float(b[1]);
    }
    const float mean_s = s1 * (1.0f / MF_D);
    const float rstd = rsqrtf(fmaxf(s2 * (1.0f / MF_D) - mean_s * mean_s, 0.f) + 1e-5f);
    const float mean = csh + mean_s;
    asm volatile("" : "+a"(oacc[0]), "+a"(oacc[1]), "+a"(oacc[2]), "+a"(oacc[3]), "+a"(oacc[4]), "+a"(oacc[5]), "+a"(oacc[6]),
                      "+a"(oacc[7]), "+a"(oacc[8]), "+a"(oacc[9]), "+a"(oacc[10]), "+a"(oacc[11]));
#pragma unroll
    for (int t = 0; t < MF_OT; ++t)
#pragma unroll
      for (int cc = 0; cc < 4; ++cc) {
        const int col = 32 * t + 8 * cc + 4 * hh;
        const float4 bv = *reinterpret_cast<const float4*>(lds_b2 + col);
        const float4 g4 = *reinterpret_cast<const float4*>(lds_u + col);
        const float4 b4 = *reinterpret_cast<const float4*>(lds_u + MF_D + col);
        const f32x4 y = {fmaf((oacc[t][4 * cc] + bv.x - mean) * rstd, g4.x, b4.x), fmaf((oacc[t][4 * cc + 1] + bv.y - mean) * rstd, g4.y, b4.y),
                         fmaf((oacc[t][4 * cc + 2] + bv.z - mean) * rstd, g4.z, b4.z), fmaf((oacc[t][4 * cc + 3] + bv.w - mean) * rstd, g4.w, b4.w)};
        if (GWW_MF_XLDS) {
          *reinterpret_cast<f32x4*>(slice0 + (t & 1) * (MF_WAVES * MF_SLICE_BYTES) + r * MF_SLICE_STRIDE + (8 * cc + 4 * hh) * 4) = y;
          if (cc == 3) {
#pragma unroll
            for (int i = 0; i < 4; ++i) {
              const f32x4 u = *reinterpret_cast<const f32x4*>(slice0 + (t & 1) * (MF_WAVES * MF_SLICE_BYTES) + (8 * i + crow) * MF_SLICE_STRIDE + cchunk * 16);
              *reinterpret_cast<f32x4*>(reinterpret_cast<char*>(y_out) + (unsigned)grow[i] * (unsigned)(MF_D * 4) + 16u * (unsigned)cchunk + t * 128) = u;
            }
          }
        } else if (GWW_MF_XSTNT) __builtin_nontemporal_store(y, reinterpret_cast<f32x4*>(reinterpret_cast<char*>(y_out) + xoff + (32 * t + 8 * cc) * 4));
        else *reinterpret_cast<f32x4*>(reinterpret_cast<char*>(y_out) + xoff + (32 * t + 8 * cc) * 4) = y;
      }
  } else if constexpr (FIN) {
    mf_wait_vmcnt<0>();
    float* y_out = reinterpret_cast<float*>(C);
    unsigned roff[4];
#pragma unroll
    for (int i = 0; i < 4; ++i) roff[i] = (unsigned)grow[i] * (unsigned)(MF_D * 4) + 16u * (unsigned)cchunk;
    f32x4 xh[MF_KT][2][4];
    float s1[4] = {0.f, 0.f, 0.f, 0.f}, s2[4] = {0.f, 0.f, 0.f, 0.f}, cshift[4];
    auto request = [&](int np0) {
#pragma unroll
      for (int q = 0; q < 3; ++q)
#pragma unroll
        for (int h2 = 0; h2 < 2; ++h2)
#pragma unroll
          for (int i = 0; i < 4; ++i) {
            if (np0 == 0)
              asm volatile("global_load_dwordx4 %0, %1, %2 offset:%3" MF_NT
                           : "=v"(xh[q][h2][i]) : "v"(roff[i]), "s"(x_out), "n"((64 * q + 32 * h2) * 4) : "memory");
            else
              asm volatile("global_load_dwordx4 %0, %1, %2 offset:%3" MF_NT
                           : "=a"(xh[3 + q][h2][i]) : "v"(roff[i]), "s"(x_out), "n"((64 * (3 + q) + 32 * h2) * 4) : "memory");
          }
    };
    request(0);
#pragma unroll
    for (int np = 0; np < MF_KT; ++np) {
#pragma unroll
      for (int tt = 0; tt < 2; ++tt) {
        const int t = 2 * np + tt;
#pragma unroll
        for (int cc = 0; cc < 4; ++cc) {
          const int nl = 32 * t + 8 * cc + 4 * hh;
          const float4 bv = *reinterpret_cast<const float4*>(lds_b2 + nl);
          u32x2 o = {pack2bf(oacc[t][4 * cc] + bv.x, oacc[t][4 * cc + 1] + bv.y),
                     pack2bf(oacc[t][4 * cc + 2] + bv.z, oacc[t][4 * cc + 3] + bv.w)};
          *reinterpret_cast<u32x2*>(slice + r * MF_SLICE_STRIDE + (32 * tt + 8 * cc + 4 * hh) * 2) = o;
        }
      }
      if (np == 2) request(3);
#pragma unroll
      for (int h2 = 0; h2 < 2; ++h2)
#pragma unroll
        for (int i = 0; i < 4; ++i) {
          if (np < 2) asm volatile("s_waitcnt vmcnt(%1)" : "+v"(xh[np][h2][i]) : "n"(23 - (8 * np + 4 * h2 + i)));
          else if (np == 2) asm volatile("s_waitcnt vmcnt(%1)" : "+v"(xh[np][h2][i]) : "n"(24 + 23 - (16 + 4 * h2 + i)));
          else asm volatile("s_waitcnt vmcnt(%1)" : "+a"(xh[np][h2][i]) : "n"(23 - (8 * (np - 3) + 4 * h2 + i)));
          f32x4 v = xh[np][h2][i];
          const u32x2 dv = *reinterpret_cast<const u32x2*>(slice + (8 * i + crow) * MF_SLICE_STRIDE + h2 * 64 + cchunk * 8);
          v[0] += bf2f((unsigned short)(dv[0] & 0xffff));
          v[1] += bf2f((unsigned short)(dv[0] >> 16));
          v[2] += bf2f((unsigned short)(dv[1] & 0xffff));
          v[3] += bf2f((unsigned short)(dv[1] >> 16));
          if (np == 0 && h2 == 0) {
            float t = (v[0] + v[1]) + (v[2] + v[3]);
            t = mf_sum8(t);
            cshift[i] = t * (1.0f / 32.0f);
          }
          v[0] -= cshift[i]; v[1] -= cshift[i]; v[2] -= cshift[i]; v[3] -= cshift[i];
          s1[i] += (v[0] + v[1]) + (v[2] + v[3]);
          s2[i] += (v[0] * v[0] + v[1] * v[1]) + (v[2] * v[2] + v[3] * v[3]);
          xh[np][h2][i] = v;
        }
    }
    float rstd[4], mean_s[4];
#pragma unroll
    for (int i = 0; i < 4; ++i) {
      float a = s1[i], b = s2[i];
      a = mf_sum8(a); b = mf_sum8(b);
      mean_s[i] = a * (1.0f / MF_D);
      rstd[i] = rsqrtf(fmaxf(b * (1.0f / MF_D) - mean_s[i] * mean_s[i], 0.f) + 1e-5f);
    }
#pragma unroll
    for (int np = 0; np < MF_KT; ++np)
#pragma unroll
      for (int h2 = 0; h2 < 2; ++h2) {
        const int col = 64 * np + 32 * h2 + 4 * cchunk;
        const float4 g4 = *reinterpret_cast<const float4*>(lds_u + col);
        const float4 b4 = *reinterpret_cast<const float4*>(lds_u + MF_D + col);
#pragma unroll
        for (int i = 0; i < 4; ++i) {
          const f32x4 v = xh[np][h2][i];
          const f32x4 y = {fmaf((v[0] - mean_s[i]) * rstd[i], g4.x, b4.x), fmaf((v[1] - mean_s[i]) * rstd[i], g4.y, b4.y),
                           fmaf((v[2] - mean_s[i]) * rstd[i], g4.z, b4.z), fmaf((v[3] - mean_s[i]) * rstd[i], g4.w, b4.w)};
          *reinterpret_cast<f32x4*>(reinterpret_cast<char*>(y_out) + roff[i] + (64 * np + 32 * h2) * 4) = y;
        }
      }
  } else if constexpr (!QKV) {
    mf_wait_vmcnt<0>();
#pragma unroll
    for (int np = 0; np < MF_OT / 2; ++np) {
#pragma unroll
      for (int tt = 0; tt < 2; ++tt) {
        const int t = 2 * np + tt;
#pragma unroll
        for (int cc = 0; cc < 4; ++cc) {
          const int nl = 32 * t + 8 * cc + 4 * hh;
          const float4 bv = *reinterpret_cast<const float4*>(lds_b2 + nl);
          u32x2 o = {pack2bf(oacc[t][4 * cc] + bv.x, oacc[t][4 * cc + 1] + bv.y),
                     pack2bf(oacc[t][4 * cc + 2] + bv.z, oacc[t][4 * cc + 3] + bv.w)};
          *reinterpret_cast<u32x2*>(slice + r * MF_SLICE_STRIDE + (32 * tt + 8 * cc + 4 * hh) * 2) = o;
        }
      }
#pragma unroll
      for (int i = 0; i < 4; ++i) {
        const u32x4 u = *reinterpret_cast<const u32x4*>(slice + (8 * i + crow) * MF_SLICE_STRIDE + cchunk * 16);
        const long orow = m_base + 8 * i + crow;
        *reinterpret_cast<u32x4*>(C + orow * MF_D + np * 64 + 8 * cchunk) = u;
      }
    }
  } else {
    if constexpr (XACC) {
      seam_x(lds_b2, x_next);
    } else if constexpr (!LNQ) {
      seam(x_out, x_next, lds_b2, [] {});
#if GWW_MF_NORM
    normalise_af();
#else
      for (int i = tid; i < NQ; i += MF_THREADS) { lds_qcb[i] = q_cb[i]; lds_u[i] = q_u[i]; }
      mf_wait_vmcnt<0>();
#endif
    } else {
      mf_wait_vmcnt<0>();
    }
    __builtin_amdgcn_s_barrier();

    MSTAMP(5);
#if GWW_MF_TAIL2
    {
    const int nchunks = NQ / 64;
    u32x4 tq[4];
#pragma unroll
    for (int i = 0; i < 4; ++i) tq[i] = u32x4{0u, 0u, 0u, 0u};
    auto q_preload = [&](int t, int chunk, int q) {
      const float4 bv = *reinterpret_cast<const float4*>(lds_qcb + 64 * chunk + 32 * (t & 1) + 8 * q + 4 * hh);
      sacc[t][4 * q] = bv.x; sacc[t][4 * q + 1] = bv.y; sacc[t][4 * q + 2] = bv.z; sacc[t][4 * q + 3] = bv.w;
    };
    auto q_ride = [&](auto q_c, auto g_c, int chunk, auto mode_c) {
      constexpr int Q = decltype(q_c)::value, G = decltype(g_c)::value, RM = decltype(mode_c)::value;
      if constexpr (RM == 1 && G >= 4 && G < 12) {
        constexpr int tt = (G - 4) >> 2, cc = (G - 4) & 3;
        const f32x16& a = sacc[2 * Q + tt];
        u32x2 o = {pack2bf(a[4 * cc], a[4 * cc + 1]), pack2bf(a[4 * cc + 2], a[4 * cc + 3])};
        *reinterpret_cast<u32x2*>(slice + r * MF_SLICE_STRIDE + (32 * tt + 8 * cc + 4 * hh) * 2) = o;
      }
      if constexpr (RM >= 1 && G >= 12 && G < 20) {
        if (chunk + 1 < nchunks) q_preload(2 * Q + ((G - 12) >> 2), chunk + 1, (G - 12) & 3);
      }
      if constexpr (RM == 1 && G >= 22 && G < 26) {
        tq[G - 22] = *reinterpret_cast<const u32x4*>(slice + (8 * (G - 22) + crow) * MF_SLICE_STRIDE + cchunk * 16);
        asm volatile("" : "+v"(tq[G - 22]));
      }
      if constexpr (RM == 1 && G >= 37 && G < 41) {
        const long orow = m_base + 8 * (G - 37) + crow;
        if (!(GWW_MF_ABL & 1))
          __builtin_nontemporal_store(tq[G - 37], reinterpret_cast<u32x4*>(q_out + orow * NQ + (chunk - 1) * 64 + 8 * cchunk));
      }
    };
    auto run_qtile = [&](auto flat_c, auto par_c, auto idx3_c, auto mode_c, int chunk, auto extra_c, auto nowait_c) {
      constexpr int FLAT = decltype(flat_c)::value, PAR = decltype(par_c)::value, IDX3 = decltype(idx3_c)::value;
      constexpr int RM = decltype(mode_c)::value, EXTRA = decltype(extra_c)::value;
      constexpr bool NOWAIT = decltype(nowait_c)::value != 0;
      constexpr int ST = (12 % MF_NST == 0) ? ((FLAT + OP_TILES) % MF_NST) : -1;
      if (ST >= 0) stage = ST;
      if (!(GWW_MF_ABL & 4)) {
        if (!NOWAIT) mf_wait_vmcnt<MF_GL*(MF_AHEAD - 2) + ((GWW_MF_ABL & 3) ? 0 : EXTRA)>();
      }
      if (!(GWW_MF_ABL & 8)) __builtin_amdgcn_s_barrier();
      TSTAMP(6);
      const int dma_tile = it + MF_AHEAD < total ? it + MF_AHEAD : total - 1;
      const int dma_stage = stage + MF_AHEAD >= MF_NST ? stage + MF_AHEAD - MF_NST : stage + MF_AHEAD;
      const int stage_next = stage + 1 == MF_NST ? 0 : stage + 1;
#pragma unroll
      for (int sub = 0; sub < 4; ++sub) {
        bf16x8(&cur)[4] = wf[sub & 1];
        bf16x8(&nxt)[4] = wf[(sub + 1) & 1];
        const unsigned char* Wn = lds + (sub == 3 ? stage_next : stage) * MF_TILE;
        __builtin_amdgcn_sched_barrier(0);
#pragma unroll
        for (int u = 0; u < 4; ++u) {
          const int tl = u & 1, ks = 2 * sub + (u >> 1);
          asm volatile("s_nop 1\n\tv_mfma_f32_32x32x16_bf16 %0, %1, %2, %0" : "+v"(sacc[2 * PAR + tl]) : "v"(cur[u]), "v"(af[8 * IDX3 + ks]));
          if (u < 3) asm volatile("" : "+v"(cur[u + 1]));
          else if (sub < 3) asm volatile("" : "+v"(nxt[0]));
          {
            const int off = sub == 3 ? first_off(0, u) : (u & 1) * 8192 + off1[2 * (sub + 1) + (u >> 1)];
            nxt[u] = *reinterpret_cast<const bf16x8*>(Wn + off);
          }
          if constexpr (RM != 0) {
            if (sub == 0 && u == 0) q_ride(MF_FL<1 - PAR>{}, MF_FL<16 * IDX3 + 0>{}, chunk, mode_c);
            else if (sub == 0 && u == 1) q_ride(MF_FL<1 - PAR>{}, MF_FL<16 * IDX3 + 1>{}, chunk, mode_c);
            else if (sub == 0 && u == 2) q_ride(MF_FL<1 - PAR>{}, MF_FL<16 * IDX3 + 2>{}, chunk, mode_c);
            else if (sub == 0 && u == 3) q_ride(MF_FL<1 - PAR>{}, MF_FL<16 * IDX3 + 3>{}, chunk, mode_c);
            else if (sub == 1 && u == 0) q_ride(MF_FL<1 - PAR>{}, MF_FL<16 * IDX3 + 4>{}, chunk, mode_c);
            else if (sub == 1 && u == 1) q_ride(MF_FL<1 - PAR>{}, MF_FL<16 * IDX3 + 5>{}, chunk, mode_c);
            else if (sub == 1 && u == 2) q_ride(MF_FL<1 - PAR>{}, MF_FL<16 * IDX3 + 6>{}, chunk, mode_c);
            else if (sub == 1 && u == 3) q_ride(MF_FL<1 - PAR>{}, MF_FL<16 * IDX3 + 7>{}, chunk, mode_c);
            else if (sub == 2 && u == 0) q_ride(MF_FL<1 - PAR>{}, MF_FL<16 * IDX3 + 8>{}, chunk, mode_c);
            else if (sub == 2 && u == 1) q_ride(MF_FL<1 - PAR>{}, MF_FL<16 * IDX3 + 9>{}, chunk, mode_c);
            else if (sub == 2 && u == 2) q_ride(MF_FL<1 - PAR>{}, MF_FL<16 * IDX3 + 10>{}, chunk, mode_c);
            else if (sub == 2 && u == 3) q_ride(MF_FL<1 - PAR>{}, MF_FL<16 * IDX3 + 11>{}, chunk, mode_c);
            else if (sub == 3 && u == 0) q_ride(MF_FL<1 - PAR>{}, MF_FL<16 * IDX3 + 12>{}, chunk, mode_c);
            else if (sub == 3 && u == 1) q_ride(MF_FL<1 - PAR>{}, MF_FL<16 * IDX3 + 13>{}, chunk, mode_c);
            else if (sub == 3 && u == 2) q_ride(MF_FL<1 - PAR>{}, MF_FL<16 * IDX3 + 14>{}, chunk, mode_c);
            else q_ride(MF_FL<1 - PAR>{}, MF_FL<16 * IDX3 + 15>{}, chunk, mode_c);
          }
          if (!(GWW_MF_ABL & 4)) {
            const int piece = 4 * sub + u - (9 - 4 * IDX3);
            if (piece >= 0 && piece < 4) issue_piece(dma_tile, dma_stage, piece);
          }
        }
        __builtin_amdgcn_sched_barrier(0);
      }
      stage = stage_next;
      ++it;
      TSTAMP(7);
    };
    using NW = std::conditional_t<LNQ || (GWW_MF_ABL & 32), I0, I1>;
    if (LNQ) {
#pragma unroll
      for (int u = 0; u < 4; ++u) wf[0][u] = *reinterpret_cast<const bf16x8*>(lds + stage * MF_TILE + first_off(0, u));
    }
#pragma unroll
    for (int t = 0; t < 2; ++t)
#pragma unroll
      for (int q = 0; q < 4; ++q) q_preload(t, 0, q);
    run_qtile(MF_FL<0>{}, I0{}, I0{}, I2{}, 0, I0{}, NW{});
    run_qtile(MF_FL<1>{}, I0{}, I1{}, I2{}, 0, I0{}, NW{});
    run_qtile(MF_FL<2>{}, I0{}, I2{}, I2{}, 0, I0{}, I0{});
    run_qtile(MF_FL<3>{}, I1{}, I0{}, I1{}, 1, I0{}, I0{});
    run_qtile(MF_FL<4>{}, I1{}, I1{}, I1{}, 1, I0{}, I0{});
    run_qtile(MF_FL<5>{}, I1{}, I2{}, I1{}, 1, I0{}, I0{});
    using I4 = std::integral_constant<int, 4>;
    for (int c = 2; c < nchunks; c += 4) {
      run_qtile(MF_FL<6>{}, I0{}, I0{}, I1{}, c, I4{}, I0{});
      run_qtile(MF_FL<7>{}, I0{}, I1{}, I1{}, c, I4{}, I0{});
      run_qtile(MF_FL<8>{}, I0{}, I2{}, I1{}, c, I0{}, I0{});
      run_qtile(MF_FL<9>{}, I1{}, I0{}, I1{}, c + 1, I4{}, I0{});
      run_qtile(MF_FL<10>{}, I1{}, I1{}, I1{}, c + 1, I4{}, I0{});
      run_qtile(MF_FL<11>{}, I1{}, I2{}, I1{}, c + 1, I0{}, I0{});
      run_qtile(MF_FL<12>{}, I0{}, I0{}, I1{}, c + 2, I4{}, I0{});
      run_qtile(MF_FL<13>{}, I0{}, I1{}, I1{}, c + 2, I4{}, I0{});
      run_qtile(MF_FL<14>{}, I0{}, I2{}, I1{}, c + 2, I0{}, I0{});
      run_qtile(MF_FL<15>{}, I1{}, I0{}, I1{}, c + 3, I4{}, I0{});
      run_qtile(MF_FL<16>{}, I1{}, I1{}, I1{}, c + 3, I4{}, I0{});
      run_qtile(MF_FL<17>{}, I1{}, I2{}, I1{}, c + 3, I0{}, I0{});
    }
    asm volatile("s_nop 15\n\ts_nop 15" : "+v"(sacc[2]), "+v"(sacc[3]));
    if (!(GWW_MF_ABL & 2)) {
#pragma unroll
      for (int tt = 0; tt < 2; ++tt)
#pragma unroll
        for (int cc = 0; cc < 4; ++cc) {
          const f32x16& a = sacc[2 + tt];
          u32x2 o = {pack2bf(a[4 * cc], a[4 * cc + 1]), pack2bf(a[4 * cc + 2], a[4 * cc + 3])};
          *reinterpret_cast<u32x2*>(slice + r * MF_SLICE_STRIDE + (32 * tt + 8 * cc + 4 * hh) * 2) = o;
        }
#pragma unroll
      for (int i = 0; i < 4; ++i) {
        const u32x4 u = *reinterpret_cast<const u32x4*>(slice + (8 * i + crow) * MF_SLICE_STRIDE + cchunk * 16);
        const long orow = m_base + 8 * i + crow;
        if (GWW_MF_ABL & 1) { asm volatile("" :: "v"(u)); continue; }
        __builtin_nontemporal_store(u, reinterpret_cast<u32x4*>(q_out + orow * NQ + (nchunks - 1) * 64 + 8 * cchunk));
      }
    }
    mf_wait_vmcnt<(GWW_MF_ABL & 3) ? 0 : 8>();
// ... 50 lines not shown
            } else {
              acc[u] = __builtin_amdgcn_mfma_f32_32x32x16_bf16(cur[u], af[4 * kt + sub], acc[u], 0, 0, 0);
            }
#endif
            nxt[u] = *reinterpret_cast<const bf16x8*>(Wn + u * 4096);
          }
#if !GWW_MF_SCHED
          __builtin_amdgcn_sched_group_barrier(0x008, 1, 0);
          __builtin_amdgcn_sched_group_barrier(0x100, 1, 0);
          __builtin_amdgcn_sched_group_barrier(0x002, 2, 0);
          __builtin_amdgcn_sched_group_barrier(0x008, 1, 0);
          __builtin_amdgcn_sched_group_barrier(0x100, 1, 0);
          __builtin_amdgcn_sched_group_barrier(0x002, 2, 0);
          __builtin_amdgcn_sched_group_barrier(0x008, 1, 0);
          __builtin_amdgcn_sched_group_barrier(0x100, 1, 0);
          __builtin_amdgcn_sched_group_barrier(0x002, 2, 0);
          __builtin_amdgcn_sched_group_barrier(0x008, 1, 0);
          __builtin_amdgcn_sched_group_barrier(0x100, 1, 0);
          __builtin_amdgcn_sched_group_barrier(0x002, 2, 0);
#endif
          __builtin_amdgcn_sched_barrier(0);
        }
        stage = stage_next;
        TSTAMP(7);
      }
#if GWW_MF_SCHED
      asm volatile("s_nop 15\n\ts_nop 15" : "+v"(acc[0]), "+v"(acc[1]), "+v"(acc[2]), "+v"(acc[3]));
#endif
#pragma unroll
      for (int half = 0; half < 2; ++half) {
        if (GWW_MF_ABL & 2) break;
#pragma unroll
        for (int tt = 0; tt < 2; ++tt) {
          const int t = 2 * half + tt;
#pragma unroll
          for (int cc = 0; cc < 4; ++cc) {
            const int nl = 128 * nt + 32 * t + 8 * cc + 4 * hh;
#if GWW_MF_SCHED
            const float v0 = acc[t][4 * cc], v1 = acc[t][4 * cc + 1], v2 = acc[t][4 * cc + 2], v3 = acc[t][4 * cc + 3];
            (void)nl;
#elif GWW_MF_NORM
            const float4 bv = *reinterpret_cast<const float4*>(lds_qcb + nl);
            const float v0 = acc[t][4 * cc] + bv.x, v1 = acc[t][4 * cc + 1] + bv.y;
            const float v2 = acc[t][4 * cc + 2] + bv.z, v3 = acc[t][4 * cc + 3] + bv.w;
#else
            const float4 bv = *reinterpret_cast<const float4*>(lds_qcb + nl);
            const float4 uv = *reinterpret_cast<const float4*>(lds_u + nl);
            const float v0 = fmaf(row_rstd, fmaf(-row_mean, uv.x, acc[t][4 * cc]), bv.x);
            const float v1 = fmaf(row_rstd, fmaf(-row_mean, uv.y, acc[t][4 * cc + 1]), bv.y);
            const float v2 = fmaf(row_rstd, fmaf(-row_mean, uv.z, acc[t][4 * cc + 2]), bv.z);
            const float v3 = fmaf(row_rstd, fmaf(-row_mean, uv.w, acc[t][4 * cc + 3]), bv.w);
#endif
            u32x2 o = {pack2bf(v0, v1), pack2bf(v2, v3)};
            *reinterpret_cast<u32x2*>(slice + r * MF_SLICE_STRIDE + (32 * tt + 8 * cc + 4 * hh) * 2) = o;
          }
        }
#pragma unroll
        for (int i = 0; i < 4; ++i) {
          const u32x4 u = *reinterpret_cast<const u32x4*>(slice + (8 * i + crow) * MF_SLICE_STRIDE + cchunk * 16);
          const long orow = m_base + 8 * i + crow;
          if (GWW_MF_ABL & 1) { asm volatile("" :: "v"(u)); continue; }
#if GWW_MF_NTSTORE
          __builtin_nontemporal_store(u, reinterpret_cast<u32x4*>(q_out + orow * NQ + nt * 128 + 64 * half + 8 * cchunk));
#else
          *reinterpret_cast<u32x4*>(q_out + orow * NQ + nt * 128 + 64 * half + 8 * cchunk) = u;
#endif
        }
      }
    }
    mf_wait_vmcnt<(GWW_MF_ABL & 3) ? 0 : 8>();
#endif
  }
  MSTAMP(3);
  MSTAMP_FLUSH
}

__device__ __forceinline__ u32x4 mf_scale_bf16x8(u32x4 v, float f) {
#pragma unroll
  for (int j = 0; j < 4; ++j) {
    const float lo = __uint_as_float(v[j] << 16) * f, hi = __uint_as_float(v[j] & 0xffff0000u) * f;
    v[j] = (__float_as_uint(lo) >> 16) | (__float_as_uint(hi) & 0xffff0000u);
  }
  return v;
}

__global__ __launch_bounds__(256) void k_mlp_pack(const unsigned short* __restrict__ w1,
                                                  const unsigned short* __restrict__ w2,
                                                  const unsigned short* __restrict__ wq,
                                                  unsigned short* __restrict__ out, int F, long n_chunks16,
                                                  const unsigned short* __restrict__ wo) {
  const int nck = F / 64, mlp_tiles = 6 * nck, op_tiles = wo ? 3 * MF_KT : 0;
  for (long g = (long)blockIdx.x * 256 + threadIdx.x; g < n_chunks16; g += (long)gridDim.x * 256) {
    const int tile_all = (int)(g >> 10), within = (int)(g & 1023);
    const int row = within >> 3, chunk = (within & 7) ^ ((row >> 1) & 7);
    const int tile = tile_all - op_tiles;
    u32x4 v;
    if (tile < 0) {
      const int nt = tile_all / MF_KT, kt = tile_all - nt * MF_KT;
      v = *reinterpret_cast<const u32x4*>(wo + (long)(128 * nt + row) * MF_D + 64 * kt + 8 * chunk);
    } else if (tile >= mlp_tiles) {
#if GWW_MF_TAIL2
      const int it2 = tile - mlp_tiles, cq = it2 / 3, k3 = it2 - 3 * cq;
      const int row2 = within >> 4, ch = (within & 15) ^ (row2 & 15);
      v = *reinterpret_cast<const u32x4*>(wq + (long)(64 * cq + row2) * MF_D + 128 * k3 + 8 * ch);
#else
      const int it2 = tile - mlp_tiles, nt = it2 / MF_KT, kt = it2 - nt * MF_KT;
      v = *reinterpret_cast<const u32x4*>(wq + (long)(128 * nt + row) * MF_D + 64 * kt + 8 * chunk);
#endif
    } else {
      int kind, cp, idx3;
      if (tile < 3) { kind = 0; cp = 0; idx3 = tile; }
      else {
        const int k = tile - 3, blk = k / 6, w = k - 6 * blk;
        if (blk == nck - 1) { kind = 1; cp = blk; idx3 = w; }
        else if (w < 3) { kind = 0; cp = blk + 1; idx3 = w; }
        else { kind = 1; cp = blk; idx3 = w - 3; }
      }
      if (kind == 0) {
        const int row2 = within >> 4, ch = (within & 15) ^ (row2 & 15);
        v = *reinterpret_cast<const u32x4*>(w1 + (long)(64 * cp + row2) * MF_D + 128 * idx3 + 8 * ch);
        if (GWW_MF_SCHED) v = mf_scale_bf16x8(v, 0.125f);
      } else {
        const unsigned short* src = w2 + (long)(128 * idx3 + row) * F + 64 * cp;
        unsigned short e[8];
#pragma unroll
        for (int j = 0; j < 8; ++j) {
          const int p = 8 * chunk + j;
          e[j] = src[(p & ~12) | ((p & 4) << 1) | ((p & 8) >> 1)];
        }
        v = u32x4{(unsigned)e[0] | ((unsigned)e[1] << 16), (unsigned)e[2] | ((unsigned)e[3] << 16),
                  (unsigned)e[4] | ((unsigned)e[5] << 16), (unsigned)e[6] | ((unsigned)e[7] << 16)};
        if (GWW_MF_SCHED) v = mf_scale_bf16x8(v, 8.0f);
      }
    }
    reinterpret_cast<u32x4*>(out)[g] = v;
  }
}

int launch_mlp_pack(const void* w1_folded, const void* w2, const void* wqkv_folded, void* out, int d, int F, int NQ,
                    hipStream_t s, const void* wo) {
  GWW_REQUIRE(d == MF_D && F % 128 == 0 && F >= 0 && (F > 0 || wqkv_folded),
              "mlp_pack: d must be 384 and ffn a multiple of 128 (0: only the q / k / v panel, for LayerNorm 1 + q / k / v alone)");
  GWW_REQUIRE(!wqkv_folded || (NQ > 0 && NQ % 128 == 0), "mlp_pack: the q / k / v panel needs NQ %% 128 == 0");
  GWW_REQUIRE(!wo || F > 0, "mlp_pack: an out_proj panel goes in front of an MLP stream");
  const long n16 = ((wo ? (long)MF_D * MF_D : 0) + 2L * MF_D * F + (wqkv_folded ? (long)NQ * MF_D : 0)) / 8;
  hipLaunchKernelGGL(k_mlp_pack, dim3((unsigned)cdiv(n16, 256)), dim3(256), 0, s, (const unsigned short*)w1_folded,
                     (const unsigned short*)w2, (const unsigned short*)wqkv_folded, (unsigned short*)out, F, n16,
                     (const unsigned short*)wo);
  GWW_LAUNCH_CHECK();
  return GWW_OK;
}

bool mlp_fused_supported(int d, int F) { return d == MF_D && F > 0 && F % 128 == 0 && F <= MF_FMAX; }

int launch_mlp_fused(const MlpFusedArgs& a, hipStream_t s) {
  const char* who = a.who;
  const void* const A = a.ctx ? a.ctx : a.delta;
  const bool op = a.ctx != nullptr, lnq = !A, fin = a.y != nullptr, qkv = a.qkv_out != nullptr, x0 = a.x0 != nullptr;
  GWW_REQUIRE(!(a.ctx && a.delta) && op == (a.bo != nullptr), "%s: a pending delta, or ctx with the out_proj bias", who);
  GWW_REQUIRE(!fin || (op && !qkv && !a.C && a.lnf_w && a.lnf_b), "%s: the final LayerNorm takes ctx, bo, lnf_w, lnf_b and no other output", who);
  GWW_REQUIRE(!lnq || (!a.x_new && !a.ln_u && !a.ln_cb && !a.b2 && !a.C && a.F == 0), "%s: LayerNorm 1 + q / k / v alone takes no block operand", who);
  GWW_REQUIRE(fin || qkv || (!lnq && a.C), "%s: no output", who);
  GWW_REQUIRE(!x0 || (!a.x_new && !a.keep_x_new && (lnq || (op && qkv))), "%s: x0 runs LN1 + q / k / v alone or ctx + block + q / k / v, without x_new", who);
  GWW_REQUIRE(a.Wt && (x0 || a.x) && (lnq || (a.ln_u && a.ln_cb && a.b2 && (x0 || a.x_new))) && (!a.keep_x_new || a.x_new), "%s: NULL operand", who);
  GWW_REQUIRE(a.d == MF_D && (lnq || mlp_fused_supported(a.d, a.F)),
              "%s: built for d_model = 384 and ffn a multiple of 128, <= 1536 (got %d, %d)", who, a.d, a.F);
  GWW_REQUIRE(!qkv || (a.qkv_u && a.qkv_cb && a.NQ > 0 && a.NQ % 128 == 0 && a.NQ <= MF_FMAX),
              "%s: the q / k / v projection needs u, cb and NQ %% 128 == 0, NQ <= 1536", who);
  GWW_REQUIRE(x0 || lnq || ((const void*)a.x_new != (const void*)a.x && (const void*)a.y != (const void*)a.x_new),
              "%s: x_new must alias neither x nor y", who);
  GWW_REQUIRE((lnq && !x0) || a.M * (long)(MF_D * 4) < (1L << 32), "%s: M = %ld rows exceed the 32-bit row offsets of the seams", who, a.M);
  GWW_REQUIRE((((x0 ? 0 : (uintptr_t)a.x) | ((uintptr_t)A) | ((uintptr_t)a.x_new) | ((uintptr_t)a.Wt) | ((uintptr_t)a.C) |
                ((uintptr_t)a.qkv_out) | ((uintptr_t)a.y)) & 15) == 0, "%s: operands must be 16-byte aligned", who);
  if (a.M == 0) return GWW_OK;
  if (x0) {
    const MfX0& z = *a.x0;
    GWW_REQUIRE(z.xs && z.tr && z.pos && z.flag && a.x, "%s: NULL operand", who);
    GWW_REQUIRE(z.T >= MF_BM && z.Tt >= 3 && z.Tt < z.T && a.M % z.T == 0, "%s: bad shape M=%ld T=%d Tt=%d", who, a.M, z.T, z.Tt);
    GWW_REQUIRE(((((uintptr_t)z.xs) | ((uintptr_t)z.tr) | ((uintptr_t)z.pos) | ((uintptr_t)a.x)) & 15) == 0 && (((uintptr_t)z.flag) & 3) == 0,
                "%s: operands must be 16-byte aligned", who);
  }
  float* const x_next = !qkv || lnq ? nullptr : a.x_next ? a.x_next : const_cast<float*>(a.x);
  GWW_REQUIRE(!x_next || ((((uintptr_t)x_next) & 15) == 0 && x_next != a.x_new), "%s: x_next must not alias x_new", who);
  const long panels = cdiv(a.M, MF_BM);
  static const int stagger_env = (int)lab_int("GWW_MLP_STAGGER", 0);
  const int stagger = !lnq && !fin && !x0 && panels >= 512 ? stagger_env : 0;
  auto launch = [&](auto kernel, auto z) {
    hipLaunchKernelGGL(kernel, dim3((unsigned)panels), dim3(MF_THREADS), 0, s, a.x, (const unsigned short*)A, a.x_new, a.ln_u, a.ln_cb,
                       (const unsigned short*)a.Wt, a.b2, fin ? reinterpret_cast<unsigned short*>(a.y) : (unsigned short*)a.C, a.M, a.F,
                       stagger, fin ? a.lnf_w : qkv ? a.qkv_u : nullptr, fin ? a.lnf_b : qkv ? a.qkv_cb : nullptr,
                       (unsigned short*)a.qkv_out, qkv ? a.NQ : 0, x_next, a.bo, a.keep_x_new ? 1 : 0, z);
  };
  switch ((lnq ? 2 : fin ? 3 : qkv ? 1 : 0) | (op ? 4 : 0) | (x0 ? 8 : 0)) {
    case 5: launch(k_mlp_fused<1, true>, MfNoX0{}); break;
    case 1: launch(k_mlp_fused<1, false>, MfNoX0{}); break;
    case 4: launch(k_mlp_fused<0, true>, MfNoX0{}); break;
    case 0: launch(k_mlp_fused<0, false>, MfNoX0{}); break;
    case 7: launch(k_mlp_fused<3, true>, MfNoX0{}); break;
    case 2: launch(k_mlp_fused<2, false>, MfNoX0{}); break;
    case 10: launch(k_mlp_fused<2, false, true>, *a.x0); break;
    case 13: launch(k_mlp_fused<1, true, true>, *a.x0); break;
    default: return fail(GWW_ERR_ARG, "%s: no such instantiation of k_mlp_fused", who);
  }
  GWW_LAUNCH_CHECK();
  return GWW_OK;
}

}

using namespace gww;

#ifdef GWW_STAMP
extern "C" int gww_debug_stamps_mlp(unsigned long long* out8, int reset) {
  GWW_HIP(hipMemcpyFromSymbol(out8, HIP_SYMBOL(gww::g_stamp_mlp), sizeof(unsigned long long) * 24));
  if (reset) {
    unsigned long long z[24] = {0};
    GWW_HIP(hipMemcpyToSymbol(HIP_SYMBOL(gww::g_stamp_mlp), z, sizeof(z)));
  }
  return GWW_OK;
}
#endif

extern "C" int gww_mlp_pack_bf16(const void* w1_folded, const void* w2, const void* wqkv_folded_or_null, void* out, int d,
                                 int F, int NQ, void* stream) {
  GWW_REQUIRE(out && ((w1_folded && w2) || (F == 0 && wqkv_folded_or_null)), "gww_mlp_pack_bf16: NULL argument");
  return launch_mlp_pack(w1_folded, w2, wqkv_folded_or_null, out, d, F, NQ, (hipStream_t)stream, nullptr);
}

extern "C" int gww_mlp_pack_op_bf16(const void* wo, const void* w1_folded, const void* w2, const void* wqkv_folded_or_null,
                                    void* out, int d, int F, int NQ, void* stream) {
  GWW_REQUIRE(wo && w1_folded && w2 && out, "gww_mlp_pack_op_bf16: NULL argument");
  return launch_mlp_pack(w1_folded, w2, wqkv_folded_or_null, out, d, F, NQ, (hipStream_t)stream, wo);
}

static MlpFusedArgs mf_block_args(const char* who, const float* x, float* x_new, const float* ln_u, const float* ln_cb, const void* Wt,
                                  const float* b2, long M, int d, int F) {
  MlpFusedArgs a;
  a.who = who; a.x = x; a.x_new = x_new; a.keep_x_new = x_new != nullptr; a.ln_u = ln_u; a.ln_cb = ln_cb; a.Wt = Wt; a.b2 = b2;
  a.M = M; a.d = d; a.F = F;
  return a;
}
static void mf_qkv_args(MlpFusedArgs& a, const float* qkv_u, const float* qkv_cb, void* qkv_out, int NQ) {
  a.qkv_u = qkv_u; a.qkv_cb = qkv_cb; a.qkv_out = qkv_out; a.NQ = NQ;
}

extern "C" int gww_attn_out_mlp_fused_bf16(float* x, const void* ctx, const float* bo, float* x_out, const float* ln_u,
                                           const float* ln_cb, const void* Wt, const float* b2, void* C, long M, int d,
                                           int F, const float* qkv_u, const float* qkv_cb, void* qkv_out, int NQ,
                                           void* stream) {
  GWW_REQUIRE(ctx && bo, "gww_attn_out_mlp_fused_bf16: NULL ctx or out_proj bias");
  MlpFusedArgs a = mf_block_args("gww_attn_out_mlp_fused_bf16", x, x_out, ln_u, ln_cb, Wt, b2, M, d, F);
  a.ctx = ctx; a.bo = bo; a.C = C;
  mf_qkv_args(a, qkv_u, qkv_cb, qkv_out, NQ);
  return launch_mlp_fused(a, (hipStream_t)stream);
}

extern "C" int gww_attn_out_mlp_final_bf16(const float* x, const void* ctx, const float* bo, float* x_mid, const float* ln_u,
                                          const float* ln_cb, const void* Wt, const float* b2, const float* lnf_w,
                                          const float* lnf_b, float* y, long M, int d, int F, void* stream) {
  MlpFusedArgs a = mf_block_args("gww_attn_out_mlp_final_bf16", x, x_mid, ln_u, ln_cb, Wt, b2, M, d, F);
  a.ctx = ctx; a.bo = bo; a.lnf_w = lnf_w; a.lnf_b = lnf_b; a.y = y;
  return launch_mlp_fused(a, (hipStream_t)stream);
}

extern "C" int gww_lnqkv_fused_bf16(const float* x, const float* qkv_u, const float* qkv_cb, const void* Wt, void* qkv_out,
                                    long M, int d, int NQ, void* stream) {
  MlpFusedArgs a;
  a.who = "gww_lnqkv_fused_bf16"; a.x = x; a.Wt = Wt; a.M = M; a.d = d;
  mf_qkv_args(a, qkv_u, qkv_cb, qkv_out, NQ);
  return launch_mlp_fused(a, (hipStream_t)stream);
}

extern "C" int gww_mlp_fused_bf16(float* x, const void* delta, float* x_out, const float* ln_u,
                                  const float* ln_cb, const void* Wt, const float* b2, void* C, long M, int d,
                                  int F, const float* qkv_u, const float* qkv_cb, void* qkv_out, int NQ,
                                  void* stream) {
  GWW_REQUIRE(delta, "gww_mlp_fused_bf16: NULL operand");
  MlpFusedArgs a = mf_block_args("gww_mlp_fused_bf16", x, x_out, ln_u, ln_cb, Wt, b2, M, d, F);
  a.delta = delta; a.C = C;
  mf_qkv_args(a, qkv_u, qkv_cb, qkv_out, NQ);
  return launch_mlp_fused(a, (hipStream_t)stream);
}

extern "C" int gww_lnqkv_fused_x0_bf16(const float* xs, const float* tr, const float* pos, const int* flag, const float* x, int T,
                                       int Tt, const float* qkv_u, const float* qkv_cb, const void* Wt, void* qkv_out, long M,
                                       int d, int NQ, void* stream) {
  const MfX0 z{xs, tr, pos, flag, T, Tt};
  MlpFusedArgs a;
  a.who = "gww_lnqkv_fused_x0_bf16"; a.x = x; a.x0 = &z; a.Wt = Wt; a.M = M; a.d = d;
  mf_qkv_args(a, qkv_u, qkv_cb, qkv_out, NQ);
  return launch_mlp_fused(a, (hipStream_t)stream);
}

extern "C" int gww_attn_out_mlp_fused_x0_bf16(const float* xs, const float* tr, const float* pos, const int* flag, float* x, int T,
                                              int Tt, const void* ctx, const float* bo, const float* ln_u, const float* ln_cb,
                                              const void* Wt, const float* b2, long M, int d, int F, const float* qkv_u,
                                              const float* qkv_cb, void* qkv_out, int NQ, void* stream) {
  GWW_REQUIRE(ctx, "gww_attn_out_mlp_fused_x0_bf16: NULL operand");
  const MfX0 z{xs, tr, pos, flag, T, Tt};
  MlpFusedArgs a = mf_block_args("gww_attn_out_mlp_fused_x0_bf16", x, nullptr, ln_u, ln_cb, Wt, b2, M, d, F);
  a.ctx = ctx; a.bo = bo; a.x0 = &z;
  mf_qkv_args(a, qkv_u, qkv_cb, qkv_out, NQ);
  return launch_mlp_fused(a, (hipStream_t)stream);
}
```

gw_whisper_amd/encoder.py:

```python

from __future__ import annotations

import ctypes as C
import operator
import sys
import weakref
from dataclasses import dataclass

import torch
import torch.nn as nn

from . import _lib, synth
from ._lib import check, lib


@dataclass
class WhisperConfig:
    d_model: int = 384
    encoder_layers: int = 4
    encoder_attention_heads: int = 6
    encoder_ffn_dim: int = 1536
    num_mel_bins: int = 80
    max_source_positions: int = 1500
    dropout: float = 0.0
# ... 227 lines not shown
        enc = WhisperEncoder(config, **kw)
        enc.load_state_dict({k: torch.from_numpy(v) for k, v in sd.items()})
        return enc

    def __del__(self):
        try:
            h = self.__dict__.get("_handle")
            self.__dict__["_handle"] = None
            if h is not None and not sys.is_finalizing():
                lib().gww_encoder_destroy(h)
        except Exception:
            pass

    def _ensure_handle(self):
        if self._handle is None:
            c = self.config
            cfg = _lib.EncCfg(c.d_model, c.encoder_layers, c.encoder_attention_heads, c.encoder_ffn_dim,
                              c.num_mel_bins, 2 * c.max_source_positions)
            h = C.c_void_p()
            check(lib().gww_encoder_create(C.byref(cfg), C.byref(h)), "gww_encoder_create")
            self._handle = h
        return self._handle

    def _param_cache(self) -> _ParamCache:
        c = self.__dict__.get("_pcache")
        if c is None or not c.valid():
            c = self.__dict__["_pcache"] = _ParamCache(self)
        return c

    def _group_keys(self, c=None):
        c = self._param_cache() if c is None else c
        key = lambda ps: tuple((p.data_ptr(), p._version) for p in ps)
        return key(c.globals), [tuple(key(ps) for ps in g) for g in c.layers]

    def _sync_weights(self, c=None):
        c = self._param_cache() if c is None else c
        stream = torch.cuda.current_stream()
        ev = self.__dict__.get("_packed_event")
        if ev is not None and ev[0] != stream.cuda_stream:
            stream.wait_event(ev[1])
        gkey, lkeys = self._group_keys(c)
        old = self._packed_key
        if old == (gkey, lkeys):
            return
        full = old is None
        masks = [15 if full else sum((1 << b) for b in range(4) if old[1][i][b] != lkeys[i][b])
                 for i in range(len(lkeys))]
        keep = []

        def ptr(t):
            t = t.detach().to(torch.float32).contiguous()
            keep.append(t)
            return t.data_ptr()

        wrapped = [x for mods, m in zip(c.modules, masks) for x, r in zip(mods, _LAYER)
                   if m & r[3] and hasattr(x, "effective_weights")]
        merged = {}
        if wrapped:
            merged = {id(x): w for x, w in zip(wrapped, type(wrapped[0]).effective_weights(wrapped))}
        eff = lambda lin: merged[id(lin)] if id(lin) in merged else _effective_weight(lin)

        g = None
        if full or old[0] != gkey:
            g = _lib.EncGlobals(**{f: ptr(getattr(self.get_submodule(path), attr)) for f, path, attr in _fields(_GLOBALS)})
        n = len(lkeys)
        arr = (_lib.EncLayer * n)()
        for lay, mods, m in zip(arr, c.modules, masks):
            for mod, (_, w_field, b_field, bit, _) in zip(mods, _LAYER):
                if m & bit:
                    setattr(lay, w_field, ptr(eff(mod)))
                    if b_field:
                        setattr(lay, b_field, ptr(_bias(mod)))
        if full:
            check(lib().gww_encoder_set_weights(self._ensure_handle(), C.byref(g), arr, n, stream.cuda_stream),
                  "gww_encoder_set_weights")
        else:
            dirty = (C.c_uint * n)(*masks)
            check(lib().gww_encoder_update_weights(self._ensure_handle(), C.byref(g) if g is not None else None, arr, n,
                                                   dirty, stream.cuda_stream), "gww_encoder_update_weights")
        self._packed_key = (gkey, lkeys)
        ev = torch.cuda.Event()
        ev.record(stream)
        self.__dict__["_packed_event"] = (stream.cuda_stream, ev)

    def _workspace(self, batch: int, prec: int, device) -> torch.Tensor:
        need = lib().gww_encoder_workspace_bytes(self._ensure_handle(), batch, prec)
        if self._ws is None or self._ws.numel() < need or self._ws.device != device:
            self._ws = None
            self._ws = torch.empty((need,), dtype=torch.uint8, device=device)
        return self._ws

    @property
    def _prec(self) -> int:
        return {"bf16": _lib.PREC_BF16, "fp32": _lib.PREC_F32}[self.precision]

    def _enter(self, x) -> _ParamCache:
        c = self._param_cache()
        if not x.is_cuda:
            raise _lib.GwwError("WhisperEncoder.forward needs GPU tensors: gw_whisper_amd has no CPU fallback "
                                f"(got input on {x.device})")
        t_in = 2 * self.config.max_source_positions
        if x.dim() != 3 or x.shape[1] != self.config.num_mel_bins or x.shape[-1] != t_in:
            raise ValueError(f"Whisper expects the mel input features to be of length {t_in}, but found "
                             f"{x.shape[-1]}. Make sure to pad the input mel features to {t_in}.")
        if c.named[0][1].device != x.device:
            raise _lib.GwwError("encoder parameters and input are on different devices")
        return c

    def forward_raw(self, input_features: torch.Tensor, want_hidden: bool = True, want_last: bool = False, cache=None):
        c = self._enter(input_features) if cache is None else cache
        x, prec = input_features.to(torch.float32).contiguous(), self._prec
        cfg = self.config
        B = x.shape[0]
        with torch.cuda.device(x.device):
            self._sync_weights(c)
            ws = self._workspace(B, prec, x.device)
            hidden = torch.empty((B, cfg.max_source_positions, cfg.d_model), dtype=torch.float32,
                                 device=x.device) if want_hidden else None
            last = torch.empty((B, cfg.d_model), dtype=torch.float32, device=x.device) if want_last else None
            check(lib().gww_encoder_forward(self._handle, x.data_ptr(), B, prec, ws.data_ptr(), ws.numel(),
                                            hidden.data_ptr() if want_hidden else None,
                                            last.data_ptr() if want_last else None,
                                            torch.cuda.current_stream().cuda_stream), "gww_encoder_forward")
        return hidden, last

    def forward_outputs_raw(self, input_features: torch.Tensor, want_hidden_states: bool, want_attentions: bool,
                            cache=None):
        c = self._enter(input_features) if cache is None else cache
        x, prec = input_features.to(torch.float32).contiguous(), self._prec
        cfg = self.config
        B, T, d, L, H = x.shape[0], cfg.max_source_positions, cfg.d_model, cfg.encoder_layers, cfg.encoder_attention_heads
        f32 = dict(dtype=torch.float32, device=x.device)
        with torch.cuda.device(x.device):
            self._sync_weights(c)
            ws = self._workspace(B, prec, x.device)
            hs = torch.empty((L + 1, B, T, d), **f32) if want_hidden_states else None
            last = hs[L] if want_hidden_states else torch.empty((B, T, d), **f32)
            at = torch.empty((L, B, H, T, T), **f32) if want_attentions else None
            check(lib().gww_encoder_forward_outputs(self._handle, x.data_ptr(), B, prec, ws.data_ptr(), ws.numel(),
                                                    last.data_ptr(), hs.data_ptr() if hs is not None else None,
                                                    at.data_ptr() if at is not None else None,
                                                    torch.cuda.current_stream().cuda_stream), "gww_encoder_forward_outputs")
        hidden_states = tuple(hs[:L].unbind(0)) + (last,) if hs is not None else None
        attentions = tuple(at.unbind(0)) if at is not None else None
        return last, hidden_states, attentions

    def set_split(self, on: bool = True):
        check(lib().gww_encoder_set_split(self._ensure_handle(), int(on)), "gww_encoder_set_split")
        self._ws = None

    def set_stem_shortcut(self, on: bool = True):
        check(lib().gww_encoder_set_stem_shortcut(self._ensure_handle(), int(on)), "gww_encoder_set_stem_shortcut")

    def stem_shortcut_flags(self, batch: int) -> tuple:
        if self._ws is None:
            raise _lib.GwwError("stem_shortcut_flags: no forward has run yet")
        flags = (C.c_int * 2)()
        with torch.cuda.device(self._ws.device):
            torch.cuda.synchronize()
            check(lib().gww_encoder_stem_shortcut_flags(self._ensure_handle(), int(batch), self._prec, self._ws.data_ptr(), flags),
                  "gww_encoder_stem_shortcut_flags")
        return int(flags[0]), int(flags[1])

    def trace_enable(self, on: bool = True):
        check(lib().gww_encoder_trace_enable(self._ensure_handle(), int(on)), "gww_encoder_trace_enable")

    def trace_read(self) -> dict:
        n = lib().gww_encoder_trace_classes()
        ms = (C.c_float * n)()
        cnt = (C.c_int * n)()
        check(lib().gww_encoder_trace_read(self._ensure_handle(), ms, cnt), "gww_encoder_trace_read")
        return {lib().gww_encoder_trace_class_name(i).decode(): (float(ms[i]), int(cnt[i])) for i in range(n)}

    def forward(self, input_features, attention_mask=None, output_hidden_states=None, output_attentions=None,
                return_dict=None, **kwargs):
        c = self.config
        want_h = c.output_hidden_states if output_hidden_states is None else bool(output_hidden_states)
        want_a = c.output_attentions if output_attentions is None else bool(output_attentions)
        as_dict = c.return_dict if return_dict is None else bool(return_dict)
        cache = self._enter(input_features)
        if self._wants_grad(input_features, cache):
            if want_h or want_a:
                raise _lib.GwwError("WhisperEncoder: output_hidden_states / output_attentions are inference only (no "
                                    "gradient flows through them): run under torch.no_grad() or freeze the adapters")
            from .training import encoder_train_forward
            out = BaseModelOutput(last_hidden_state=encoder_train_forward(self, input_features, cache=cache))
        elif want_h or want_a:
            last, hs, at = self.forward_outputs_raw(input_features, want_h, want_a, cache=cache)
            out = BaseModelOutput(last_hidden_state=last, hidden_states=hs, attentions=at)
        else:
            hidden, _ = self.forward_raw(input_features, want_hidden=True, want_last=False, cache=cache)
            out = BaseModelOutput(last_hidden_state=hidden)
        return out if as_dict else out.to_tuple()

    def _wants_grad(self, input_features, c=None) -> bool:
        if not torch.is_grad_enabled():
            return False
        c = self._param_cache() if c is None else c
        input_grad = torch.is_tensor(input_features) and input_features.requires_grad
        base_trainable = [n for n, p in c.base if p.requires_grad]
        if not base_trainable and not any(p.requires_grad for p in c.adapters):
            return input_grad
        if self.full_finetune:
            if c.adapters:
                raise _lib.GwwError("WhisperEncoder: full fine-tuning is enabled and DoRA / LoRA adapters are attached: "
                                    "the two do not combine")
            return True
        if base_trainable:
            raise _lib.GwwError(
                "WhisperEncoder: autograd is on and base parameters require grad (e.g. " + base_trainable[0] + "): only "
                "the frozen-base + DoRA training step (and the input gradient) is implemented -- freeze the encoder "
                "(get_peft_model does) or run under torch.no_grad()")
        return self._has_trainable_adapters(c) or input_grad

    def _has_trainable_adapters(self, c=None) -> bool:
        return any(p.requires_grad for p in (self._param_cache() if c is None else c).lora_A)

    def last_token(self, input_features) -> torch.Tensor:
        cache = self._enter(input_features)
        if self._wants_grad(input_features, cache):
            from .training import encoder_train_forward
            return encoder_train_forward(self, input_features, pooled=True, cache=cache)
        return self.forward_raw(input_features, want_hidden=False, want_last=True, cache=cache)[1]
```

include/gww.h:

```cpp
#ifndef GWW_H
#define GWW_H

#include <stddef.h>
#include <stdint.h>

#ifdef __cplusplus
extern "C" {
#endif

#define GWW_VERSION 107

#define GWW_OK 0
#define GWW_ERR_ARG (-1)
#define GWW_ERR_HIP (-2)
#define GWW_ERR_WORKSPACE (-3)
#define GWW_ERR_STATE (-4)

#define GWW_PREC_BF16 0
#define GWW_PREC_F32 1

int gww_version(void);
const char* gww_last_error(void);

typedef struct gww_frontend gww_frontend;
int gww_frontend_create(gww_frontend** out);
int gww_frontend_create_nmel(int n_mels, gww_frontend** out);
void gww_frontend_destroy(gww_frontend* fe);
int gww_logmel_f32(gww_frontend* fe, const float* wave, int n_seg, int n_samples,
                   long wave_stride, float* out, float* seg_max, void* stream);
int gww_logmel_host_f32(const float* wave, int n_seg, int n_samples, long wave_stride, float* out);
int gww_logmel_host_nmel_f32(const float* wave, int n_seg, int n_samples, long wave_stride, int n_mels, float* out);

typedef struct {
  int d_model;
  int n_layers;
  int n_heads;
  int ffn;
  int n_mels;
  int t_in;
} gww_enc_cfg;

typedef struct {
  const float* conv1_w; const float* conv1_b;
  const float* conv2_w; const float* conv2_b;
  const float* pos;
  const float* ln_w; const float* ln_b;
} gww_enc_globals;

typedef struct {
  const float* ln1_w; const float* ln1_b;
  const float* q_w; const float* q_b;
  const float* k_w;
  const float* v_w; const float* v_b;
  const float* o_w; const float* o_b;
  const float* ln2_w; const float* ln2_b;
  const float* fc1_w; const float* fc1_b;
  const float* fc2_w; const float* fc2_b;
} gww_enc_layer;

typedef struct gww_encoder gww_encoder;

int gww_encoder_create(const gww_enc_cfg* cfg, gww_encoder** out);
void gww_encoder_destroy(gww_encoder* enc);
int gww_encoder_set_weights(gww_encoder* enc, const gww_enc_globals* g,
                            const gww_enc_layer* layers, int n_layers, void* stream);
int gww_encoder_update_weights(gww_encoder* enc, const gww_enc_globals* globals_or_null,
                               const gww_enc_layer* layers, int n_layers, const unsigned* layer_dirty,
                               void* stream);
size_t gww_encoder_workspace_bytes(const gww_encoder* enc, int batch, int precision);
int gww_encoder_forward(gww_encoder* enc, const float* mel, int batch, int precision,
                        void* workspace, size_t workspace_bytes,
                        float* last_hidden, float* last_token, void* stream);
int gww_encoder_forward_outputs(gww_encoder* enc, const float* mel, int batch, int precision,
                                void* workspace, size_t workspace_bytes, float* last_hidden,
                                float* hidden_slab, float* attn_slab, void* stream);

int gww_encoder_set_split(gww_encoder* enc, int on);

int gww_encoder_set_stem_shortcut(gww_encoder* enc, int on);
int gww_encoder_stem_shortcut_flags(const gww_encoder* enc, int batch, int precision, const void* workspace, int* flags);

int gww_encoder_trace_enable(gww_encoder* enc, int on);
int gww_encoder_trace_read(gww_encoder* enc, float* ms, int* counts);
int gww_encoder_trace_classes(void);
const char* gww_encoder_trace_class_name(int i);

int gww_dora_merge_f32(const float* w0, const float* a, const float* b, const float* m,
                       float scaling, int d_out, int d_in, int r,
                       float* w_eff, float* norm_out, void* stream);

int gww_conv1_gelu_bf16(const float* mel, const float* conv1_w, const float* conv1_b, void* w_scratch_bf16,
                        void* c1_out, int B, int T, int d, void* stream);

typedef struct {
  const float* w0;
  const float* a;
  const float* b;
  const float* m;
  float* w_eff;
  float* norm_out;
  float scaling;
  int d_out, d_in, r;
} gww_dora_merge_item;
int gww_dora_merge_batch_f32(const gww_dora_merge_item* items, int n, void* stream);

typedef struct {
  int layer;
  int proj;
  int r;
  float scaling;
  const float* A;
  const float* B;
  const float* mag;
  const float* nrm;
  float* dA;
  float* dB;
  float* dm;
} gww_dora_target;

size_t gww_train_saved_bytes(const gww_encoder* enc, int batch);
size_t gww_train_workspace_bytes(const gww_encoder* enc, int batch);
size_t gww_train_workspace_bytes_adapters(const gww_encoder* enc, int batch, int max_r);
int gww_encoder_train_forward(gww_encoder* enc, const float* mel, int batch, void* workspace,
                              size_t workspace_bytes, void* saved, size_t saved_bytes,
                              float* last_hidden, int pooled, void* stream);
int gww_encoder_train_backward(gww_encoder* enc, int batch, void* workspace, size_t workspace_bytes,
                               const void* saved, size_t saved_bytes, const float* d_last_hidden,
                               const gww_dora_target* targets, int n_targets, float* d_x0, float* d_mel,
                               int pooled, void* stream);

typedef struct {
  float* ln1_w; float* ln1_b;
  float* q_w; float* q_b;
  float* k_w;
  float* v_w; float* v_b;
  float* o_w; float* o_b;
  float* ln2_w; float* ln2_b;
  float* fc1_w; float* fc1_b;
  float* fc2_w; float* fc2_b;
} gww_enc_layer_grads;
typedef struct {
  float* conv1_w; float* conv1_b;
  float* conv2_w; float* conv2_b;
  float* pos;
  float* ln_w; float* ln_b;
  const gww_enc_layer_grads* layers;
} gww_enc_grads;
size_t gww_train_workspace_bytes_full(const gww_encoder* enc, int batch);
int gww_encoder_train_backward_full(gww_encoder* enc, int batch, void* workspace, size_t workspace_bytes,
                                    const void* saved, size_t saved_bytes, const float* d_last_hidden,
                                    const gww_dora_target* targets, int n_targets, float* d_x0, float* d_mel,
                                    int pooled, const gww_enc_grads* grads, void* stream);
size_t gww_train_saved_bytes_f32(const gww_encoder* enc, int batch);
size_t gww_train_workspace_bytes_f32(const gww_encoder* enc, int batch);
int gww_encoder_train_forward_f32(gww_encoder* enc, const float* mel, int batch, void* workspace,
                                  size_t workspace_bytes, void* saved, size_t saved_bytes,
                                  float* last_hidden, int pooled, void* stream);
int gww_encoder_train_backward_f32(gww_encoder* enc, int batch, void* workspace, size_t workspace_bytes,
                                   const void* saved, size_t saved_bytes, const float* d_last_hidden,
                                   const gww_dora_target* targets, int n_targets, float* d_x0, float* d_mel,
                                   int pooled, void* stream);

size_t gww_gemm_wgrad_workspace_bytes(long M, int N, int K);
int gww_gemm_wgrad_bf16(const void* dY, long ldy, const void* X, long ldx, long M, int N, int K, float alpha,
                        float* dW, float* db_or_null, void* workspace, size_t ws_bytes, void* stream);
size_t gww_layernorm_param_grads_workspace_bytes(long M, int d);
int gww_layernorm_param_grads(const float* x, const void* dy, int dy_is_f32, long M, int d, float* dgamma,
                              float* dbeta, void* workspace, size_t ws_bytes, void* stream);

int gww_layernorm(const float* x, const float* w, const float* b, void* y, int out_bf16,
                  long M, int d, void* stream);
int gww_gemm_bf16(const void* A, const void* W, const float* bias, const float* resid, void* C,
                  long M, int N, int K, int epilogue, void* stream);
int gww_gemm_bf16_v4_split(const void* A, const void* W, const float* bias, const float* resid, void* C,
                           long M, int N, int K, int epilogue, int n_split, void* stream);
int gww_gemm_astat_bf16(const void* A, const void* delta, float* x_out, const float* ln_u,
                        const float* ln_cb, const void* W, const float* bias, void* C, long M, int N,
                        int K, int epilogue, void* stream);
int gww_ln_fold_weights(const float* w, const float* ln_w, const float* ln_b, const float* bias, float scale,
                        int N, int K, void* w_folded_bf16, float* u, float* cb, void* stream);
int gww_gemm_fulln_bf16(const void* A, const void* W, const float* bias, void* C, long M, int N, int K,
                        int epilogue, void* stream);
int gww_mlp_fused_bf16(float* x, const void* delta, float* x_out, const float* ln_u, const float* ln_cb,
                       const void* Wt, const float* b2, void* C, long M, int d, int F, const float* qkv_u,
                       const float* qkv_cb, void* qkv_out, int NQ, void* stream);
int gww_mlp_pack_bf16(const void* w1_folded, const void* w2, const void* wqkv_folded_or_null, void* out, int d, int F,
                      int NQ, void* stream);
int gww_attn_out_mlp_fused_bf16(float* x, const void* ctx, const float* bo, float* x_out, const float* ln_u,
                                const float* ln_cb, const void* Wt, const float* b2, void* C, long M, int d, int F,
                                const float* qkv_u, const float* qkv_cb, void* qkv_out, int NQ, void* stream);
int gww_attn_out_mlp_final_bf16(const float* x, const void* ctx, const float* bo, float* x_mid, const float* ln_u,
                                const float* ln_cb, const void* Wt, const float* b2, const float* lnf_w, const float* lnf_b,
                                float* y, long M, int d, int F, void* stream);
int gww_mlp_pack_op_bf16(const void* wo, const void* w1_folded, const void* w2, const void* wqkv_folded_or_null, void* out,
                         int d, int F, int NQ, void* stream);
int gww_lnqkv_fused_bf16(const float* x, const float* qkv_u, const float* qkv_cb, const void* Wt, void* qkv_out, long M,
                         int d, int NQ, void* stream);
int gww_stem_fill_f32(const float* xs, const float* tr, const float* pos, const int* flag, float* x, int B, int T, int Tt, int d,
                      void* stream);
int gww_lnqkv_fused_x0_bf16(const float* xs, const float* tr, const float* pos, const int* flag, const float* x, int T, int Tt,
                            const float* qkv_u, const float* qkv_cb, const void* Wt, void* qkv_out, long M, int d, int NQ,
                            void* stream);
int gww_attn_out_mlp_fused_x0_bf16(const float* xs, const float* tr, const float* pos, const int* flag, float* x, int T, int Tt,
                                   const void* ctx, const float* bo, const float* ln_u, const float* ln_cb, const void* Wt,
                                   const float* b2, long M, int d, int F, const float* qkv_u, const float* qkv_cb, void* qkv_out,
                                   int NQ, void* stream);
int gww_qscan_energy_f32(const float* fseries, int ld, int B, const int* rows, const int* order,
                         const int* class_ranges_host, const float* window, float* energy, long e_total,
                         unsigned int* plane_max, int n_planes, void* stream);
int gww_qscan_interp_f32(const float* energy, long e_total, const int* rows, const int* plane_rows, int n_planes,
                         const unsigned int* plane_max, int B, int F, int T, float* out, int* chosen, void* stream);
int gww_qadapter_tail_f32(const float* y, int B, int Hin, int Win, const float* scale, const float* bias,
                          const float* gamma_i, const float* beta_i, float* out, long out_batch_stride, int F, int T,
                          void* stream);
size_t gww_qadapter_cnn_packed_bytes(int c1, int c2, int c3);
size_t gww_qadapter_cnn_workspace_bytes(int B, int H, int W, int c1, int c2);
int gww_qadapter_cnn_pack_f32(const float* w1, const float* b1, const float* w2, const float* b2, const float* w3,
                              const float* b3, const float* w4, const float* b4, int c1, int c2, int c3, void* packed,
                              void* stream);
int gww_qadapter_cnn_forward_f32(const float* qspec, int B, int H, int W, const void* packed, int c1, int c2, int c3,
                                 void* workspace, size_t workspace_bytes, float* y, void* stream);
size_t gww_qadapter_cnn_backward_workspace_bytes(int B, int H, int W, int c1, int c2, int c3);
int gww_qadapter_cnn_backward_f32(const float* qspec, const float* dy, int B, int H, int W, const void* packed,
                                  const float* w2, const float* w3, int c1, int c2, int c3, void* workspace,
                                  size_t workspace_bytes, float* dw1, float* db1, float* dw2, float* db2, float* dw3,
                                  float* db3, float* dw4, float* db4, void* stream);
int gww_welch_power_f32(const float* spec, long ld, long n_seg, int n_bins, float scale, float* power, void* stream);
int gww_column_median_f32(const float* power, long n_seg, int n_bins, float* median, void* stream);
int gww_fir_f32(const float* xp, long xp_stride, const float* g, int taps4, int D, float* out, long out_stride,
                long n_out, void* stream);
int gww_fir_f64(const double* xp, long xp_stride, const double* g, int taps4, int D, float* out, long out_stride,
                long n_out, void* stream);
int gww_cluster_triggers_f64(const double* times, const float* scores, long n, float trigger_threshold,
// ... 107 lines not shown
```

Measured before the change: 25920 segments/s.

## Stream residual activations between fused MLP kernels in accumulator-native layout

Adds an 'x_native' residual-stream layout in which the fused MLP+QKV kernel stores the updated residual x in the order its accumulators hold it, in 32-row slices. The next layer's fused kernel then loads it back with contiguous dwordx4 non-temporal accesses, which avoids strided row-major stores and loads between layers. The final fused LayerNorm kernel also writes last_token directly, replacing a separate hipMemcpy2DAsync. This adds new template instantiations, 32-bit offset limits and layout coupling between kernels, and the path is on by default.

New measurement: 26250 segments/s (median of 6 runs). 1.01x the previous value.

```diff
diff --git a/gw_whisper_amd/_lib.py b/gw_whisper_amd/_lib.py
--- a/gw_whisper_amd/_lib.py
+++ b/gw_whisper_amd/_lib.py
@@ -75,6 +75,9 @@
     "gww_encoder_set_split": (C.c_int, [C.c_void_p, C.c_int]),
     "gww_encoder_set_stem_shortcut": (C.c_int, [C.c_void_p, C.c_int]),
     "gww_encoder_stem_shortcut_flags": (C.c_int, [C.c_void_p, C.c_int, C.c_int, C.c_void_p, C.POINTER(C.c_int)]),
+    "gww_encoder_set_x_native": (C.c_int, [C.c_void_p, C.c_int]),
+    "gww_x_native_offset": (C.c_size_t, [C.c_long, C.c_int, C.c_long]),
+    "gww_x_native_bytes": (C.c_size_t, [C.c_long]),
     "gww_encoder_trace_enable": (C.c_int, [C.c_void_p, C.c_int]),
     "gww_encoder_trace_read": (C.c_int, [C.c_void_p, C.POINTER(C.c_float), C.POINTER(C.c_int)]),
     "gww_encoder_trace_classes": (C.c_int, []),
diff --git a/gw_whisper_amd/csrc/common.h b/gw_whisper_amd/csrc/common.h
--- a/gw_whisper_amd/csrc/common.h
+++ b/gw_whisper_amd/csrc/common.h
@@ -137,6 +137,14 @@
 }
 
 static inline long cdiv(long a, long b) { return (a + b - 1) / b; }
+
+__host__ __device__ inline size_t x_native_offset(long g, int c, long M) {
+  if (g > M - 1) g = M - 1;
+  const size_t slice = (size_t)(g >> 5);
+  const int r = (int)(g & 31), t = c >> 5, cc = (c >> 3) & 3, hh = (c >> 2) & 1, k = c & 3;
+  return (slice * 48 + (size_t)(4 * t + cc)) * 1024 + (size_t)(r + 32 * hh) * 16 + (size_t)(4 * k);
+}
+inline size_t x_native_bytes(long M) { return (size_t)cdiv(M, 128) * 128 * 384 * 4; }
 
 struct Arena {
   size_t off = 0;
diff --git a/gw_whisper_amd/csrc/encoder.hip b/gw_whisper_amd/csrc/encoder.hip
--- a/gw_whisper_amd/csrc/encoder.hip
+++ b/gw_whisper_amd/csrc/encoder.hip
@@ -303,6 +303,7 @@
   bool fuse_final;
   bool pooled;
   bool q_log2;
+  bool x_native;
 };
 FwdPlan plan_forward(const gww_encoder* e, int batch, int precision, FwdWants want) {
   const gww_enc_cfg& c = e->cfg;
@@ -325,6 +326,9 @@
   p.pooled = bf && !want.last_hidden && want.last_token && T >= 3 && !(m & GP_POOLED) && !want.hidden_slab && !want.attn_slab;
   p.x0_layer0 = p.shortcut && p.lnqkv0 && p.op && !want.hidden_slab && c.n_layers > 1;
   p.q_log2 = attention_log2q_enabled();
+  p.x_native = e->x_native && p.op && p.fuse_final && !p.pooled && !want.hidden_slab && c.n_layers > 1 && d == 384 &&
+               mlp_fused_x_native_supported() && !(m & GP_X_NATIVE) &&
+               x_native_bytes((long)batch * T) <= padded_rows((size_t)batch * T) * d * 4;
   return p;
 }
 }
@@ -347,6 +351,18 @@
   e->stem_shortcut = on != 0;
   return GWW_OK;
 }
+
+extern "C" int gww_encoder_set_x_native(gww_encoder* e, int on) {
+  GWW_REQUIRE(e != nullptr, "gww_encoder_set_x_native: NULL handle");
+  e->x_native = on != 0;
+  return GWW_OK;
+}
+
+extern "C" size_t gww_x_native_offset(long row, int col, long M) {
+  if (row < 0 || col < 0 || col >= 384 || M <= 0) return (size_t)-1;
+  return x_native_offset(row, col, M);
+}
+extern "C" size_t gww_x_native_bytes(long M) { return M > 0 ? x_native_bytes(M) : 0; }
 
 extern "C" int gww_encoder_stem_shortcut_flags(const gww_encoder* e, int batch, int precision, const void* workspace,
                                                int* flags) {
@@ -560,19 +576,18 @@
       TR(TR_OUT, launch_gemm_astat(ctx, d, nullptr, nullptr, nullptr, nullptr, L.wo, L.bo, d1, M, d, d, EPI_BIAS, 0, s));
     MlpFusedArgs a = args();
     a.x = st.xc; a.x_new = from_x0 ? nullptr : st.xn; a.ln_u = L.u1; a.ln_cb = L.cb1; a.b2 = L.b2; a.F = F;
+    a.x_native_in = p.x_native && i > (p.x0_layer0 ? 1 : 0);
     if (p.op) { a.ctx = ctx; a.bo = L.bo; a.Wt = L.wmlp_op; }
     else { a.delta = d1; a.Wt = L.wmlp; }
     if (p.fuse_qkv && !last) {
       with_qkv(a, e->layers[i + 1]);
       if (from_x0) a.x0 = &x0;
+      a.x_native_out = p.x_native && !from_x0;
       TR(TR_MLPQKV, launch_mlp_fused(a, s));
       st.qkv_ready = true;
     } else if (p.fuse_final) {
-      a.lnf_w = e->lnw; a.lnf_b = e->lnb; a.y = last_hidden;
+      a.lnf_w = e->lnw; a.lnf_b = e->lnb; a.y = last_hidden; a.last_token = last_token; a.T = T;
       TR(TR_MLPFIN, launch_mlp_fused(a, s));
-      if (last_token)
-        GWW_HIP(hipMemcpy2DAsync(last_token, (size_t)d * 4, last_hidden + (size_t)(T - 1) * d, (size_t)T * d * 4, (size_t)d * 4,
-                                 B, hipMemcpyDeviceToDevice, s));
       return tap_final();
     } else if (p.mlp_fused) {
       a.C = d2; a.keep_x_new = true;
diff --git a/gw_whisper_amd/csrc/encoder_impl.h b/gw_whisper_amd/csrc/encoder_impl.h
--- a/gw_whisper_amd/csrc/encoder_impl.h
+++ b/gw_whisper_amd/csrc/encoder_impl.h
@@ -50,6 +50,7 @@
   GP_ASTAT_512 = 512,
   GP_CONV2_FULLN = 1024,
   GP_STEM_SHORTCUT = 2048,
+  GP_X_NATIVE = 4096,
 };
 inline int generic_path_mask() {
   static const int mask = (int)lab_int("GWW_GENERIC_PATH", 0);
@@ -92,6 +93,7 @@
   bool ready = false;
   bool trace = false;
   bool stem_shortcut = true;
+  bool x_native = true;
   std::vector<TraceSpan> spans;
   std::vector<hipEvent_t> pool;
   int split = 0;
diff --git a/gw_whisper_amd/csrc/launchers.h b/gw_whisper_amd/csrc/launchers.h
--- a/gw_whisper_amd/csrc/launchers.h
+++ b/gw_whisper_amd/csrc/launchers.h
@@ -46,6 +46,7 @@
 int launch_mlp_pack(const void* w1_folded, const void* w2, const void* wqkv_folded, void* out, int d, int F, int NQ,
                     hipStream_t s, const void* wo = nullptr);
 bool mlp_fused_supported(int d, int F);
+bool mlp_fused_x_native_supported();
 struct MfX0 {
   const float *xs, *tr, *pos;
   const int* flag;
@@ -69,6 +70,10 @@
   float* x_next = nullptr;
   const float *lnf_w = nullptr, *lnf_b = nullptr;
   float* y = nullptr;
+  float* last_token = nullptr;
+  int T = 0;
+  bool x_native_in = false;
+  bool x_native_out = false;
   const MfX0* x0 = nullptr;
   long M = 0;
   int d = 0, F = 0;
diff --git a/gw_whisper_amd/csrc/mlp_fused.hip b/gw_whisper_amd/csrc/mlp_fused.hip
--- a/gw_whisper_amd/csrc/mlp_fused.hip
+++ b/gw_whisper_amd/csrc/mlp_fused.hip
@@ -61,6 +61,22 @@
 #define MF_XNT MF_NT
 #else
 #define MF_XNT ""
+#endif
+#ifndef GWW_MF_XN_LDNT
+#define GWW_MF_XN_LDNT 1
+#endif
+#ifndef GWW_MF_XN_STNT
+#define GWW_MF_XN_STNT 1
+#endif
+#if GWW_MF_XN_LDNT
+#define MF_XN_LDNT " nt"
+#else
+#define MF_XN_LDNT ""
+#endif
+#if GWW_MF_XN_STNT
+#define MF_XN_STNT " nt"
+#else
+#define MF_XN_STNT ""
 #endif
 #ifndef GWW_MF_DMAGAP
 #define GWW_MF_DMAGAP 1
@@ -157,7 +173,7 @@
 }
 
 struct MfNoX0 {};
-template <int MODE, bool OP, bool X0 = false>
+template <int MODE, bool OP, bool X0 = false, int XL = 0>
 __global__ __launch_bounds__(MF_THREADS, 1) void k_mlp_fused(const float* X, const unsigned short* delta, float* x_out,
                                                             const float* __restrict__ ln_u,
                                                             const float* __restrict__ ln_cb,
@@ -173,6 +189,8 @@
   constexpr bool QKV = MODE == 1 || MODE == 2, LNQ = MODE == 2, FIN = MODE == 3;
   static_assert(!X0 || (GWW_MF_NORM && GWW_MF_XACC && (MODE == 2 || (MODE == 1 && OP))), "X0: layer 0's two launches; stages in the u table");
   constexpr bool XACC = GWW_MF_XACC && GWW_MF_NORM && GWW_MF_SCHED && OP && (MODE == 1 || MODE == 3);
+  constexpr bool XIN = (XL & 1) != 0, XOUT = (XL & 2) != 0;
+  static_assert(XL == 0 || (XACC && !GWW_MF_XLDS && !X0 && (!XOUT || MODE == 1) && XL <= 3), "XL: the accumulator-order stream of XACC");
   constexpr int MF_NST = MF_AHEAD + 1;
   float* lds_cb = reinterpret_cast<float*>(lds + MF_OFF_CB);
   float* lds_u = reinterpret_cast<float*>(lds + MF_OFF_U);
@@ -249,6 +267,7 @@
   for (int p = 0; p < MF_AHEAD; ++p) issue(p, p);
   const long xrow_l = m_base + r < M ? m_base + r : M - 1;
   const unsigned xoff = (unsigned)xrow_l * (unsigned)(MF_D * 4) + 16u * (unsigned)hh;
+  const unsigned xoff_n = (unsigned)(xrow_l >> 5) * (unsigned)(32 * MF_D * 4) + 16u * (((unsigned)xrow_l & 31u) + 32u * (unsigned)hh);
   f32x4 xp[XACC ? MF_OT : 1][4];
   bool x0 = false;
   int x0_seg0 = 0;
@@ -292,6 +311,8 @@
 #pragma unroll
       for (int cc = 0; cc < 4; ++cc)
         if (GWW_MF_ABL & 32) asm volatile("v_accvgpr_write_b32 %0, 0" : "=a"(xp[t][cc][0]));
+        else if constexpr (XIN)
+          asm volatile("global_load_dwordx4 %0, %1, %2 offset:%3" MF_XN_LDNT : "=a"(xp[t][cc]) : "v"(xoff_n), "s"(reinterpret_cast<const char*>(X) + 4096 * t), "n"(1024 * cc) : "memory");
         else asm volatile("global_load_dwordx4 %0, %1, %2 offset:%3" MF_XNT : "=a"(xp[t][cc]) : "v"(xoff), "s"(X), "n"((32 * t + 8 * cc) * 4) : "memory");
   }
   bf16x8 af[MF_KT * 4];
@@ -839,7 +860,8 @@
       row_mean = stat[32 + r];
       asm volatile("" : "+v"(row_rstd), "+v"(row_mean)::"memory");
       };
-  auto seam_x = [&](const float* sb, float* dst) {
+  auto seam_x = [&](const float* sb, float* dst, auto native_c, const unsigned xst_n) {
+    constexpr bool NAT = decltype(native_c)::value;
     if constexpr (XACC) {
     float s1 = 0.f, s2 = 0.f, csh = 0.f;
 #pragma unroll
@@ -851,8 +873,10 @@
         if (dst && !(GWW_MF_ABL & 16)) {
           if (GWW_MF_XLDS) {
             *reinterpret_cast<f32x4*>(slice0 + (t & 1) * (MF_WAVES * MF_SLICE_BYTES) + r * MF_SLICE_STRIDE + (8 * cc + 4 * hh) * 4) = v;
+          } else if constexpr (NAT) {
+            asm volatile("global_store_dwordx4 %0, %1, %2 offset:%3" MF_XN_STNT "\n\ts_nop 1" : : "v"(xst_n), "v"(v), "s"(reinterpret_cast<char*>(dst) + 4096 * t), "n"(1024 * cc) : "memory");
           } else {
-            f32x4* const sp = reinterpret_cast<f32x4*>(reinterpret_cast<char*>(dst) + xoff + (32 * t + 8 * cc) * 4);
+            f32x4* const sp = reinterpret_cast<f32x4*>(reinterpret_cast<char*>(dst) + (XL != 0 && MODE == 1 ? xst_n : xoff) + (32 * t + 8 * cc) * 4);
             if (GWW_MF_XSTNT) __builtin_nontemporal_store(v, sp);
             else *sp = v;
           }
@@ -938,7 +962,14 @@
                  : "+a"(oacc[0]), "+a"(oacc[1]), "+a"(oacc[2]), "+a"(oacc[3]), "+a"(oacc[4]), "+a"(oacc[5]), "+a"(oacc[6]),
                    "+a"(oacc[7]), "+a"(oacc[8]), "+a"(oacc[9]), "+a"(oacc[10]), "+a"(oacc[11]));
     if constexpr (XACC) {
-      seam_x(lds_bo, (keep_x_new && !(GWW_MF_ABL & 256)) ? x_out : nullptr);
+      if constexpr (XL != 0 && MODE == 1) {
+        unsigned lo = lane_off;
+        asm volatile("" : "+v"(lo));
+        const long g = m_base + (long)((lo >> 4) & 31u);
+        const unsigned gc = (unsigned)(g < M ? g : M - 1);
+        seam_x(lds_bo, (keep_x_new && !(GWW_MF_ABL & 256)) ? x_out : nullptr, std::false_type{}, gc * (unsigned)(MF_D * 4) + ((lo >> 9) << 4));
+      } else
+      seam_x(lds_bo, (keep_x_new && !(GWW_MF_ABL & 256)) ? x_out : nullptr, std::false_type{}, 0u);
     } else {
     seam(X, x_out, lds_bo, [] {});
 #if GWW_MF_NORM
@@ -1050,6 +1081,15 @@
         } else if (GWW_MF_XSTNT) __builtin_nontemporal_store(y, reinterpret_cast<f32x4*>(reinterpret_cast<char*>(y_out) + xoff + (32 * t + 8 * cc) * 4));
         else *reinterpret_cast<f32x4*>(reinterpret_cast<char*>(y_out) + xoff + (32 * t + 8 * cc) * 4) = y;
       }
+    if (float* const lt_out = reinterpret_cast<float*>(q_out)) {
+      const unsigned b = (unsigned)xrow_l / (unsigned)NQ;
+      if ((unsigned)xrow_l - b * (unsigned)NQ == (unsigned)NQ - 1u) {
+        const char* const src = reinterpret_cast<const char*>(y_out) + xoff;
+        char* const lt = reinterpret_cast<char*>(lt_out) + b * (unsigned)(MF_D * 4) + 16u * (unsigned)hh;
+#pragma unroll 1
+        for (int i = 0; i < 4 * MF_OT; ++i) *reinterpret_cast<f32x4*>(lt + 32 * i) = *reinterpret_cast<const f32x4*>(src + 32 * i);
+      }
+    }
   } else if constexpr (FIN) {
     mf_wait_vmcnt<0>();
     float* y_out = reinterpret_cast<float*>(C);
@@ -1136,6 +1176,17 @@
           *reinterpret_cast<f32x4*>(reinterpret_cast<char*>(y_out) + roff[i] + (64 * np + 32 * h2) * 4) = y;
         }
       }
+    if (float* const lt_out = reinterpret_cast<float*>(q_out)) {
+#pragma unroll
+      for (int i = 0; i < 4; ++i) {
+        const unsigned b = (unsigned)grow[i] / (unsigned)NQ;
+        if ((unsigned)grow[i] - b * (unsigned)NQ != (unsigned)NQ - 1u) continue;
+        const char* const src = reinterpret_cast<const char*>(y_out) + roff[i];
+        char* const lt = reinterpret_cast<char*>(lt_out) + b * (unsigned)(MF_D * 4) + 16u * (unsigned)cchunk;
+#pragma unroll 1
+        for (int q = 0; q < 2 * MF_KT; ++q) *reinterpret_cast<f32x4*>(lt + 128 * q) = *reinterpret_cast<const f32x4*>(src + 128 * q);
+      }
+    }
   } else if constexpr (!QKV) {
     mf_wait_vmcnt<0>();
 #pragma unroll
@@ -1161,7 +1212,14 @@
     }
   } else {
     if constexpr (XACC) {
-      seam_x(lds_b2, x_next);
+      if constexpr (XOUT) {
+        unsigned lo = lane_off;
+        asm volatile("" : "+v"(lo));
+        const long g = m_base + (long)((lo >> 4) & 31u);
+        const unsigned gc = (unsigned)(g < M ? g : M - 1);
+        seam_x(lds_b2, x_next, std::true_type{}, (gc >> 5) * (unsigned)(32 * MF_D * 4) + 16u * (gc & 31u) + (lo & 512u));
+      } else
+      seam_x(lds_b2, x_next, std::false_type{}, 0u);
     } else if constexpr (!LNQ) {
       seam(x_out, x_next, lds_b2, [] {});
 #if GWW_MF_NORM
@@ -1518,6 +1576,8 @@
 }
 
 bool mlp_fused_supported(int d, int F) { return d == MF_D && F > 0 && F % 128 == 0 && F <= MF_FMAX; }
+constexpr bool MF_XL_BUILT = GWW_MF_XACC && GWW_MF_NORM && GWW_MF_SCHED && !GWW_MF_XLDS;
+bool mlp_fused_x_native_supported() { return MF_XL_BUILT; }
 
 int launch_mlp_fused(const MlpFusedArgs& a, hipStream_t s) {
   const char* who = a.who;
@@ -1525,6 +1585,12 @@
   const bool op = a.ctx != nullptr, lnq = !A, fin = a.y != nullptr, qkv = a.qkv_out != nullptr, x0 = a.x0 != nullptr;
   GWW_REQUIRE(!(a.ctx && a.delta) && op == (a.bo != nullptr), "%s: a pending delta, or ctx with the out_proj bias", who);
   GWW_REQUIRE(!fin || (op && !qkv && !a.C && a.lnf_w && a.lnf_b), "%s: the final LayerNorm takes ctx, bo, lnf_w, lnf_b and no other output", who);
+  GWW_REQUIRE(!a.last_token || (fin && a.T > 0 && a.M % a.T == 0 && (((uintptr_t)a.last_token) & 15) == 0 && a.last_token != a.y),
+              "%s: last_token comes with y, T rows per segment and M %% T == 0", who);
+  const int xl = (a.x_native_in ? 1 : 0) | (a.x_native_out ? 2 : 0);
+  GWW_REQUIRE(!xl || (MF_XL_BUILT && op && !a.keep_x_new && !x0 && (!a.x_native_out || (qkv && !a.x_next))),
+              "%s: the accumulator-order residual stream runs between ctx blocks that keep no x_new, in place", who);
+  GWW_REQUIRE(!xl || (long)x_native_bytes(a.M) < (1L << 32), "%s: M = %ld rows exceed the 32-bit offsets of the accumulator-order stream", who, a.M);
   GWW_REQUIRE(!lnq || (!a.x_new && !a.ln_u && !a.ln_cb && !a.b2 && !a.C && a.F == 0), "%s: LayerNorm 1 + q / k / v alone takes no block operand", who);
   GWW_REQUIRE(fin || qkv || (!lnq && a.C), "%s: no output", who);
   GWW_REQUIRE(!x0 || (!a.x_new && !a.keep_x_new && (lnq || (op && qkv))), "%s: x0 runs LN1 + q / k / v alone or ctx + block + q / k / v, without x_new", who);
@@ -1555,8 +1621,20 @@
     hipLaunchKernelGGL(kernel, dim3((unsigned)panels), dim3(MF_THREADS), 0, s, a.x, (const unsigned short*)A, a.x_new, a.ln_u, a.ln_cb,
                        (const unsigned short*)a.Wt, a.b2, fin ? reinterpret_cast<unsigned short*>(a.y) : (unsigned short*)a.C, a.M, a.F,
                        stagger, fin ? a.lnf_w : qkv ? a.qkv_u : nullptr, fin ? a.lnf_b : qkv ? a.qkv_cb : nullptr,
-                       (unsigned short*)a.qkv_out, qkv ? a.NQ : 0, x_next, a.bo, a.keep_x_new ? 1 : 0, z);
+                       fin ? reinterpret_cast<unsigned short*>(a.last_token) : (unsigned short*)a.qkv_out,
+                       fin ? (a.last_token ? a.T : 0) : qkv ? a.NQ : 0, x_next, a.bo, a.keep_x_new ? 1 : 0, z);
   };
+  if constexpr (MF_XL_BUILT) {
+    if (xl) {
+      const int mode = fin ? 3 : 1;
+      if (mode == 1 && !x0 && xl == 2) launch(k_mlp_fused<1, true, false, 2>, MfNoX0{});
+      else if (mode == 1 && xl == 3) launch(k_mlp_fused<1, true, false, 3>, MfNoX0{});
+      else if (mode == 3 && xl == 1) launch(k_mlp_fused<3, true, false, 1>, MfNoX0{});
+      else return fail(GWW_ERR_ARG, "%s: no such instantiation of k_mlp_fused", who);
+      GWW_LAUNCH_CHECK();
+      return GWW_OK;
+    }
+  }
   switch ((lnq ? 2 : fin ? 3 : qkv ? 1 : 0) | (op ? 4 : 0) | (x0 ? 8 : 0)) {
     case 5: launch(k_mlp_fused<1, true>, MfNoX0{}); break;
     case 1: launch(k_mlp_fused<1, false>, MfNoX0{}); break;
diff --git a/gw_whisper_amd/encoder.py b/gw_whisper_amd/encoder.py
--- a/gw_whisper_amd/encoder.py
+++ b/gw_whisper_amd/encoder.py
@@ -403,6 +403,9 @@
     def set_stem_shortcut(self, on: bool = True):
         check(lib().gww_encoder_set_stem_shortcut(self._ensure_handle(), int(on)), "gww_encoder_set_stem_shortcut")
 
+    def set_x_native(self, on: bool = True):
+        check(lib().gww_encoder_set_x_native(self._ensure_handle(), int(on)), "gww_encoder_set_x_native")
+
     def stem_shortcut_flags(self, batch: int) -> tuple:
         if self._ws is None:
             raise _lib.GwwError("stem_shortcut_flags: no forward has run yet")
diff --git a/include/gww.h b/include/gww.h
--- a/include/gww.h
+++ b/include/gww.h
@@ -79,6 +79,10 @@
 
 int gww_encoder_set_stem_shortcut(gww_encoder* enc, int on);
 int gww_encoder_stem_shortcut_flags(const gww_encoder* enc, int batch, int precision, const void* workspace, int* flags);
+
+int gww_encoder_set_x_native(gww_encoder* enc, int on);
+size_t gww_x_native_offset(long row, int col, long M);
+size_t gww_x_native_bytes(long M);
 
 int gww_encoder_trace_enable(gww_encoder* enc, int on);
 int gww_encoder_trace_read(gww_encoder* enc, float* ms, int* counts);
```
